# laoreja/HPLFlowNet

Hardware: AMD Instinct MI355X
Metric: point-pairs/sec + EPE3D, N=8192 FlyingThings3D, 1/2/4/8 MI355X (higher is better)
Workload: dtype f32 (wide layers: fp32 operands as scaled fp16 pairs, 3 partial products, fp32 accumulate); 1 GPU; full HPLFlowNet inference (7 levels, 19.3M params, random init), FT3D-like synthetic pair, N=8192, bs=1 per GPU; num_points=8192, step_includes_lattice_build=True, forward_streams=3, lattices_under_construction=3, exact_fallback_launches=0, lattice_launches_per_pair=34

## Files before the change

### hplflownet_amd/_lib.py

```python
import ctypes
import os

import torch

_HERE = os.path.dirname(os.path.abspath(__file__))
LIB_PATH = os.path.join(_HERE, 'libhplbcl.so')

c_i64, c_i32, c_f32, c_vp = ctypes.c_int64, ctypes.c_int32, ctypes.c_float, ctypes.c_void_p


class HplError(RuntimeError):
    pass


class RelayoutJob(ctypes.Structure):
    _fields_ = [('W', ctypes.c_void_p), ('base', ctypes.c_int64), ('sr', ctypes.c_int64), ('sq', ctypes.c_int64),
                ('sf', ctypes.c_int64), ('R', ctypes.c_int32), ('Q', ctypes.c_int32), ('F', ctypes.c_int32),
                ('mirror', ctypes.c_int32), ('ldw', ctypes.c_int64)]


class Split3Job(ctypes.Structure):
    _fields_ = [('Wt', ctypes.c_void_p), ('dst', ctypes.c_void_p), ('k_rows', ctypes.c_int64), ('ldw', ctypes.c_int64),
                ('plane_stride', ctypes.c_int64), ('amax', ctypes.c_void_p), ('planes', ctypes.c_int32), ('pad_', ctypes.c_int32)]

# ... 52 lines not shown
class Buf(ctypes.Structure):
    _fields_ = [('rows_sym', c_i32), ('cols', c_i32)]


class Weight(ctypes.Structure):
    _fields_ = [('Wt', c_vp), ('ldw', c_i64), ('rows', c_i64), ('Wt3', c_vp), ('wt3_plane_stride', c_i64),
                ('w_amax', c_vp), ('wt3_planes', c_i32), ('pad_', c_i32)]


class Op(ctypes.Structure):
    _fields_ = [('kind', c_i32), ('tag', c_i32), ('a', Ref), ('out', Ref), ('res', Ref), ('m_sym', c_i32),
                ('res_mod_sym', c_i32), ('level', c_i32), ('table', c_i32), ('order', c_i32), ('F', c_i32), ('C', c_i32),
                ('N', c_i32), ('weight', c_i32), ('bias', c_i32), ('act', c_i32), ('slope', c_f32), ('use_norm', c_i32),
                ('reg_stride_sym', c_i32), ('ext', c_i32), ('cond', c_i32), ('cond_level', c_i32), ('out2', Ref),
                ('rows2_sym', c_i32), ('b', Ref), ('flags', c_i32), ('aux', c_i32)]


class LevelTables(ctypes.Structure):
    _fields_ = [('n0', c_i64), ('n1', c_i64), ('H0', c_i64), ('H1', c_i64), ('emg_pair', c_vp),
                ('csr_ptr', c_vp), ('csr_pt', c_vp), ('csr_w', c_vp), ('csr_norm', c_vp), ('bary0', c_vp), ('off0', c_vp),
                ('blur', c_vp), ('blur_stride', c_i64), ('blur_perm', c_vp), ('up_perm', c_vp), ('n_up_groups', c_i32),
                ('up_group_cut', c_i32 * 5), ('up_group_perm', c_vp * 4), ('corr1', c_vp), ('corr1_stride', c_i64),
                ('corr1_perm', c_vp), ('corr2', c_vp), ('tile_bm', c_i32), ('group_tile_bm', c_i32),
                ('blur_perm_tidx', c_vp), ('blur_perm_tmask', c_vp), ('up_perm_tidx', c_vp), ('up_perm_tmask', c_vp),
                ('up_group_tidx', c_vp * 4), ('up_group_tmask', c_vp * 4), ('corr1_perm_tidx', c_vp),
                ('corr1_perm_tmask', c_vp), ('bary1', c_vp), ('off1', c_vp), ('up_tap_m', c_vp), ('up_tap_row', c_vp),
                ('up_tap_ptr', c_vp), ('up_tap_max', c_i64)]


class LatticeSpec(ctypes.Structure):
    _fields_ = [('n_levels', c_i32), ('scale', c_f32 * 8), ('bcn_radius', c_i32 * 8), ('corr_filter_radius', c_i32 * 8),
                ('corr_corr_radius', c_i32 * 8), ('next_divisor', c_f32 * 8), ('wide_up', c_i32 * 8), ('n_groups', c_i32),
                ('group_cut', c_i32 * 5), ('groups_min_sparsity', c_f32), ('perm_min_rows', c_i64), ('groups_min_rows', c_i64),
                ('group_tile_bm', c_i32),
                ('fused', c_i32)]


_SIGNATURES = {
    'hpl_version': (ctypes.c_int, []),
    'hpl_last_error': (ctypes.c_char_p, []),
    'hpl_device_info': (ctypes.c_int, [ctypes.c_int, ctypes.POINTER(ctypes.c_int), ctypes.POINTER(ctypes.c_int),
                                       ctypes.c_char_p, ctypes.c_int]),
    'hpl_index_narrow': (ctypes.c_int, [c_vp, c_vp, c_i64, c_vp]),
    'hpl_corr2_permute': (ctypes.c_int, [c_vp, c_vp, ctypes.c_int, ctypes.c_int, c_i64, c_vp]),
    'hpl_corr2_permute32': (ctypes.c_int, [c_vp, c_vp, ctypes.c_int, ctypes.c_int, c_i64, c_vp]),
    'hpl_csr_build': (ctypes.c_int, [c_vp, c_vp, c_i64, c_i64, c_i64, c_vp, c_vp, c_vp, c_vp, c_vp, c_vp]),
    'hpl_csr_build_pair': (ctypes.c_int, [c_vp, c_vp, c_i64, c_i64, c_vp, c_vp, c_i64, c_i64, c_vp, c_vp, c_vp, c_vp,
                                          c_vp, c_vp]),
    'hpl_splat': (ctypes.c_int, [c_vp, c_i64, ctypes.c_int, c_vp, c_vp, c_vp, c_vp, c_i64, c_vp, c_i64, c_vp]),
    'hpl_slice': (ctypes.c_int, [c_vp, c_i64, ctypes.c_int, c_vp, c_vp, c_i64, c_vp, c_vp, c_vp, c_i64, c_vp]),
    'hpl_splat_add': (ctypes.c_int, [c_vp, c_i64, ctypes.c_int, c_vp, c_vp, c_vp, c_vp, c_i64, c_vp, c_i64, c_vp]),
    'hpl_slice_add': (ctypes.c_int, [c_vp, c_i64, ctypes.c_int, c_vp, c_vp, c_i64, c_vp, c_vp, c_vp, c_i64, c_vp]),
    'hpl_weight_unlayout_batch': (ctypes.c_int, [c_vp, ctypes.c_int, c_vp, c_i64, c_vp, c_vp]),
    'hpl_psum': (ctypes.c_int, [c_vp, c_i64, c_i64, c_i64, ctypes.c_int, c_vp, c_i64, ctypes.c_int, c_vp]),
    'hpl_regroup': (ctypes.c_int, [c_vp, c_i64, c_i64, ctypes.c_int, ctypes.c_int, c_vp, c_i64, ctypes.c_int, c_vp]),
    'hpl_epe3d': (ctypes.c_int, [c_vp, c_vp, c_i64, c_vp, c_vp, c_vp]),
    'hpl_adam_flat': (ctypes.c_int, [c_vp, c_vp, c_vp, c_vp, c_i64, ctypes.c_double, ctypes.c_double, ctypes.c_double, ctypes.c_double,
                                     c_i64, c_vp]),
    'hpl_gather_sum': (ctypes.c_int, [c_vp, c_i64, c_vp, c_i64, c_i64, ctypes.c_int, ctypes.c_int, ctypes.c_int, c_vp, c_vp, c_i64, c_i64,
                                      ctypes.c_int, c_f32, c_vp, c_i64, c_vp]),
    'hpl_table_invert': (ctypes.c_int, [c_vp, c_i64, ctypes.c_int, c_i64, ctypes.c_int, c_i64, c_vp, c_vp]),
    'hpl_weight_relayout': (ctypes.c_int, [c_vp, c_i64, ctypes.c_int, ctypes.c_int, ctypes.c_int, c_i64, c_i64,
                                           c_i64, c_vp, c_vp, c_i64, c_i64, c_vp]),
    'hpl_weight_relayout_batch': (ctypes.c_int, [c_vp, ctypes.c_int, c_vp, c_i64, c_vp, c_vp]),
    'hpl_weight_fold': (ctypes.c_int, [c_vp, ctypes.c_int, ctypes.c_int, ctypes.c_int, ctypes.c_int, ctypes.c_int, c_vp, ctypes.c_int,
                                       c_vp, c_vp, ctypes.c_int, c_vp, c_i64, c_vp, c_vp, c_vp]),
    'hpl_weight_split3': (ctypes.c_int, [c_vp, c_i64, c_i64, c_vp, c_i64, c_vp]),
    'hpl_weight_split3_batch': (ctypes.c_int, [c_vp, ctypes.c_int, c_i64, ctypes.c_int, c_vp]),
    'hpl_weight_split2h': (ctypes.c_int, [c_vp, c_i64, c_i64, c_vp, c_i64, c_vp, c_vp]),
    'hpl_amax': (ctypes.c_int, [c_vp, c_i64, c_i64, c_i32, c_vp, c_vp]),
    'hpl_amax_rows': (ctypes.c_int, [c_vp, c_i64, c_i64, c_i32, c_vp, c_vp, c_vp]),
    'hpl_gconv_wgrad_scaled': (ctypes.c_int, [c_vp, c_i64, c_i64, c_vp, c_i64, c_i64, c_i64, ctypes.c_int, ctypes.c_int,
                                              c_vp, c_i64, ctypes.c_int, c_vp, c_i64, c_vp, c_vp, c_vp, c_i64, c_vp, c_vp, c_vp, c_vp]),
    'hpl_weight_unlayout': (ctypes.c_int, [c_vp, c_i64, ctypes.c_int, ctypes.c_int, ctypes.c_int, c_vp, c_i64,
                                           c_i64, c_i64, c_i64, ctypes.c_int, c_vp]),
    'hpl_tap_order_scratch_ints': (c_i64, [c_i64]),
    'hpl_tap_order': (ctypes.c_int, [c_vp, c_i64, ctypes.c_int, c_i64, c_vp, c_vp, c_vp]),
    'hpl_tile_index': (ctypes.c_int, [c_vp, c_i64, ctypes.c_int, c_i64, c_vp, ctypes.c_int, c_vp, c_vp, c_vp]),
    'hpl_gconv_forward': (ctypes.c_int, [ctypes.POINTER(GConvDesc), c_vp]),
    'hpl_gconv_forward_naive': (ctypes.c_int, [ctypes.POINTER(GConvDesc), c_vp]),
    'hpl_gconv_wgrad': (ctypes.c_int, [c_vp, c_i64, c_i64, c_vp, c_i64, c_i64, c_i64, ctypes.c_int, ctypes.c_int,
                                       c_vp, c_i64, ctypes.c_int, c_vp, c_i64, c_vp, c_vp, c_vp, c_i64, c_vp, c_vp]),
    'hpl_gconv_launch_info': (ctypes.c_int, [ctypes.POINTER(GConvDesc), ctypes.POINTER(GConvInfo)]),
    'hpl_wgrad_launch_info': (ctypes.c_int, [c_vp, c_i64, c_i64, c_vp, c_i64, c_i64, c_i64, ctypes.c_int, ctypes.c_int,
                                             c_vp, c_i64, ctypes.c_int, c_vp, c_i64, c_vp, c_vp, c_vp, c_i64, c_vp, c_vp, c_vp,
                                             ctypes.POINTER(WGradInfo)]),
    'hpl_tap_lists': (ctypes.c_int, [c_vp, c_i64, ctypes.c_int, c_i64, c_vp, c_vp, c_vp, c_vp, c_vp]),
    'hpl_colsum': (ctypes.c_int, [c_vp, c_i64, c_i64, ctypes.c_int, c_vp, c_vp]),
    'hpl_leaky_bwd': (ctypes.c_int, [c_vp, c_i64, c_vp, c_i64, c_f32, c_vp, c_i64, c_i64, ctypes.c_int, c_vp]),
    'hpl_leaky_bwd_amax': (ctypes.c_int, [c_vp, c_i64, c_vp, c_i64, c_f32, c_vp, c_i64, c_i64, ctypes.c_int, c_vp, c_vp]),
    'hpl_transpose': (ctypes.c_int, [c_vp, c_i64, c_vp, c_i64, c_i64, c_i64, c_vp]),
    'hpl_table_symmetric': (ctypes.c_int, [c_vp, c_i64, ctypes.c_int, c_i64, c_vp, c_vp]),
    'hpl_lattice_keys': (ctypes.c_int, [c_vp, c_i64, c_f32, c_vp, c_vp, c_vp, c_i64, c_vp]),
    'hpl_lattice_keys_pair': (ctypes.c_int, [c_vp, c_vp, c_vp, c_vp, c_i64, c_i64, c_f32, c_i64, c_i64, c_f32, c_vp, c_vp,
                                             c_vp, c_vp, c_vp, c_vp, c_i64, c_vp]),
    'hpl_lattice_workspace_bytes': (c_i64, [c_i64, c_i64]),
    'hpl_lattice_hash': (ctypes.c_int, [c_vp, c_i64, c_vp, c_i64, c_vp, c_vp, c_vp, c_vp, c_vp, c_vp, c_i64, c_vp]),
    'hpl_lattice_neighbors': (ctypes.c_int, [c_vp, c_i64, c_i64, c_vp, c_vp, c_i64, c_i64, ctypes.c_int,
                                             ctypes.c_int, ctypes.c_int, c_vp, c_vp, c_i64, c_i64, c_vp, c_vp, c_vp]),
    'hpl_lattice_next_points': (ctypes.c_int, [c_vp, c_i64, c_i64, c_f32, c_vp, c_vp]),
    'hpl_lattice_create': (c_vp, [ctypes.POINTER(LatticeSpec)]),
    'hpl_lattice_destroy': (None, [c_vp]),
    'hpl_lattice_arena_bytes': (c_i64, [c_vp, c_i64, c_i64]),
    'hpl_lattice_set_bounds': (ctypes.c_int, [c_vp, ctypes.POINTER(c_i64)]),
    'hpl_lattice_stats': (ctypes.c_int, [c_vp, ctypes.POINTER(c_i32)]),
    'hpl_lattice_begin': (ctypes.c_int, [c_vp, c_vp, c_vp, c_i64, c_i64, c_vp, c_i64, c_vp]),
    'hpl_lattice_begin_batch': (ctypes.c_int, [c_vp, c_vp, c_vp, c_i64, c_i64, c_i64, c_vp, c_i64, c_vp]),
    'hpl_lattice_arena_bytes_batch': (c_i64, [c_vp, c_i64, c_i64, c_i64]),
    'hpl_lattice_begin_ragged': (ctypes.c_int, [c_vp, c_vp, c_vp, c_i64, ctypes.POINTER(c_i64), ctypes.POINTER(c_i64), c_vp, c_i64,
                                                c_vp]),
    'hpl_lattice_arena_bytes_ragged': (c_i64, [c_vp, c_i64, ctypes.POINTER(c_i64), ctypes.POINTER(c_i64)]),
    'hpl_lattice_pair_counts': (ctypes.c_int, [c_vp, ctypes.POINTER(c_i64)]),
    'hpl_lattice_ready': (ctypes.c_int, [c_vp]),
    'hpl_lattice_advance': (ctypes.c_int, [c_vp, ctypes.POINTER(ctypes.c_int)]),
    'hpl_lattice_tables': (ctypes.POINTER(LevelTables), [c_vp]),
    'hpl_lattice_extras': (ctypes.c_int, [c_vp, ctypes.POINTER(c_vp), ctypes.POINTER(c_i64)]),
    'hpl_lattice_query_info': (ctypes.c_int, [c_vp, ctypes.POINTER(QueryInfo)]),
    'hpl_lattice_query': (ctypes.c_int, [ctypes.POINTER(QueryInfo), c_vp, c_i64, ctypes.POINTER(c_i64), ctypes.c_int, c_vp, c_vp, c_vp,
                                         c_vp]),
    'hpl_knn_interp': (ctypes.c_int, [c_vp, c_i64, c_vp, ctypes.c_int, c_vp, c_i64, ctypes.c_int, c_f32, ctypes.c_int,
                                      ctypes.POINTER(c_i64), ctypes.POINTER(c_i64), c_vp, c_vp, c_vp, c_vp, c_vp]),
    'hpl_rigid_fit_workspace_bytes': (c_i64, [ctypes.c_int, c_i64]),
    'hpl_rigid_fit': (ctypes.c_int, [c_vp, c_i64, c_vp, c_i64, c_i64, c_vp, ctypes.c_int, ctypes.POINTER(c_i64), ctypes.c_int,
                                     c_f32, c_vp, c_vp, c_vp, c_vp, c_vp, c_i64, c_vp]),
    'hpl_motion_segment_workspace_bytes': (c_i64, [ctypes.c_int, c_i64]),
    'hpl_motion_segment': (ctypes.c_int, [c_vp, c_i64, c_vp, c_i64, c_i64, c_vp, ctypes.c_int, ctypes.POINTER(c_i64), c_f32, c_f32,
                                          c_f32, ctypes.c_int, ctypes.c_int, c_vp, c_vp, c_vp, c_vp, c_vp, c_i64, c_vp]),
    'hpl_selfsup_loss_workspace_bytes': (c_i64, [ctypes.c_int, c_i64, c_i64, ctypes.c_int]),
    'hpl_selfsup_loss': (ctypes.c_int, [c_vp, c_i64, c_vp, c_i64, c_i64, c_vp, c_i64, ctypes.c_int, ctypes.POINTER(c_i64),
                                        ctypes.POINTER(c_i64), ctypes.c_int, c_f32, c_f32, c_vp, c_vp, c_vp, c_vp, c_vp, c_vp,
                                        c_i64, c_vp]),
    'hpl_ground_fit_workspace_bytes': (c_i64, [ctypes.c_int, c_i64, ctypes.c_int]),
    'hpl_ground_fit': (ctypes.c_int, [c_vp, c_i64, ctypes.c_int, ctypes.POINTER(c_i64), ctypes.POINTER(c_f32), c_f32, ctypes.c_int,
                                      c_f32, ctypes.c_int, c_f32, ctypes.c_uint64, ctypes.c_uint64, c_vp, c_vp, c_vp, c_vp, c_vp,
                                      c_vp, c_vp, c_i64, c_vp]),
    'hpl_voxel_downsample_workspace_bytes': (c_i64, [ctypes.c_int, c_i64, ctypes.c_int]),
    'hpl_voxel_downsample': (ctypes.c_int, [c_vp, c_i64, c_vp, c_i64, ctypes.c_int, ctypes.c_int, ctypes.POINTER(c_i64), c_f32,
                                            ctypes.POINTER(c_f32), ctypes.c_int, c_vp, c_i64, c_vp, c_i64, c_vp, c_vp, c_vp,
                                            c_vp, c_vp, c_i64, c_vp]),
    'hpl_frames_workspace_bytes': (c_i64, [ctypes.c_int, c_i64]),
    'hpl_frames_from_kitti': (ctypes.c_int, [c_vp, c_vp, c_vp, ctypes.c_int, ctypes.POINTER(ctypes.c_int32),
                                             ctypes.POINTER(ctypes.c_int32), ctypes.POINTER(c_i64), ctypes.POINTER(c_f32), c_f32,
                                             c_vp, c_i64, c_vp, c_i64, c_vp, c_vp, c_vp, c_i64, c_vp]),
    'hpl_frames_from_ft3d': (ctypes.c_int, [c_vp, c_vp, c_vp, c_vp, c_vp, ctypes.c_int, ctypes.POINTER(ctypes.c_int32),
                                            ctypes.POINTER(ctypes.c_int32), ctypes.POINTER(c_i64), c_f32, c_f32, c_f32,
                                            ctypes.c_int, c_f32, c_vp, c_i64, c_vp, c_i64, c_vp, c_vp, c_vp, c_i64, c_vp]),
    'hpl_png_unfilter': (ctypes.c_int, [c_vp, c_i64, c_i64, ctypes.c_int]),
    'hpl_icp_workspace_bytes': (c_i64, [ctypes.c_int, c_i64, c_i64]),
    'hpl_icp': (ctypes.c_int, [c_vp, c_i64, c_vp, c_i64, c_vp, c_vp, ctypes.c_int, ctypes.POINTER(c_i64), ctypes.POINTER(c_i64),
                               ctypes.c_int, c_f32, c_f32, c_f32, c_f32, c_vp, c_vp, c_vp, c_vp, c_vp, c_vp, c_i64, c_vp]),
    'hpl_plan_create': (c_vp, [ctypes.POINTER(Op), ctypes.c_int, ctypes.POINTER(Buf), ctypes.c_int,
                               ctypes.POINTER(Weight), ctypes.c_int, ctypes.POINTER(c_vp), ctypes.c_int]),
    'hpl_plan_destroy': (None, [c_vp]),
    'hpl_plan_workspace_bytes': (c_i64, [c_vp, ctypes.POINTER(LevelTables), ctypes.c_int]),
    'hpl_plan_run': (ctypes.c_int, [c_vp, ctypes.POINTER(LevelTables), ctypes.c_int, c_vp, c_vp, c_vp, c_vp, c_i64, c_vp]),
    'hpl_plan_run_range': (ctypes.c_int, [c_vp, ctypes.POINTER(LevelTables), ctypes.c_int, c_vp, c_vp, c_vp, c_vp, c_vp, c_vp, c_i64,
                                          c_vp, c_vp, ctypes.c_int, ctypes.c_int, ctypes.c_int]),
    'hpl_plan_run_range_loss': (ctypes.c_int, [c_vp, ctypes.POINTER(LevelTables), ctypes.c_int, c_vp, c_vp, c_vp, c_vp, c_vp, c_vp, c_i64,
                                               c_vp, c_vp, ctypes.c_int, ctypes.c_int, ctypes.c_int, ctypes.c_int, ctypes.c_int,
                                               ctypes.POINTER(c_i64), c_vp, ctypes.c_int, c_vp]),
    'hpl_plan_run_batch': (ctypes.c_int, [c_vp, ctypes.POINTER(LevelTables), ctypes.c_int, ctypes.c_int, c_vp, c_vp, c_vp, c_vp, c_i64,
                                          c_vp]),
    'hpl_plan_batch_extra_bytes': (c_i64, [ctypes.POINTER(LevelTables), ctypes.c_int]),
    'hpl_batch_stage': (ctypes.c_int, [ctypes.c_int, c_i64, c_i64, c_vp, c_vp, c_vp, c_vp, c_vp, c_vp, c_vp]),
    'hpl_ragged_stage': (ctypes.c_int, [ctypes.c_int, ctypes.POINTER(c_vp), ctypes.POINTER(c_i64), ctypes.POINTER(c_i64),
                                        ctypes.POINTER(c_vp), ctypes.POINTER(c_i64), ctypes.POINTER(c_i64), ctypes.POINTER(c_vp),
# ... 84 lines not shown
```

### hplflownet_amd/csrc/executor.hip

```cpp
#include "common.h"
#include "gconv_common.h"
#include <stdlib.h>

#include <algorithm>
#include <new>
#include <vector>

using namespace hpl;

namespace {

constexpr int64_t SPLITK_ELEMS = 8 << 20;
constexpr int64_t SPLITK_WS_BYTES = 64ll << 20;
constexpr int AMAX_SLOTS = 4096;
constexpr int64_t HEAD_BYTES = SPLITK_WS_BYTES + AMAX_SLOTS * 8;
constexpr int MAX_SYMS = HPL_SYM_LEVEL0 + 8 * HPL_MAX_LEVELS;

__global__ void k_copy_cols(const float *__restrict__ src, int64_t lds, float *__restrict__ dst, int64_t ldd,
                            int64_t rows, int cols) {
    const int64_t total = rows * cols;
    int64_t i = (int64_t)blockIdx.x * blockDim.x + threadIdx.x;
    const int64_t stride = (int64_t)gridDim.x * blockDim.x;
    for (; i < total; i += stride) {
        const int64_t r = i / cols;
        const int c = (int)(i - r * cols);
        dst[r * ldd + c] = src[r * lds + c];
    }
}

__global__ void k_copy_cols4(const float4 *__restrict__ src, int64_t lds4, float4 *__restrict__ dst, int64_t ldd4,
                             int64_t rows, int cols4) {
    const int64_t total = rows * cols4;
    int64_t i = (int64_t)blockIdx.x * blockDim.x + threadIdx.x;
    const int64_t stride = (int64_t)gridDim.x * blockDim.x;
    for (; i < total; i += stride) {
        const int64_t r = i / cols4;
        const int c = (int)(i - r * cols4);
        dst[r * ldd4 + c] = src[r * lds4 + c];
    }
}

constexpr int EMG_JOBS = 24;
struct EmgJobs {
    const float4 *src[EMG_JOBS];
    float *dst[EMG_JOBS];
    int64_t ldd[EMG_JOBS];
    int64_t rows[EMG_JOBS];
    int ones[EMG_JOBS];
    int n;
};
__global__ void k_copy_emg_batch(const EmgJobs j) {
    const int job = blockIdx.y;
    const float4 *src = j.src[job];
    float *dst = j.dst[job];
    const int64_t ldd = j.ldd[job], rows = j.rows[job];
    const bool ones = j.ones[job] != 0;
    const bool vec = (ldd % 4 == 0) && ((reinterpret_cast<uintptr_t>(dst) & 15) == 0);
    for (int64_t r = (int64_t)blockIdx.x * blockDim.x + threadIdx.x; r < rows; r += (int64_t)gridDim.x * blockDim.x) {
        const float4 v = src[r];
        float *d = dst + r * ldd;
        if (vec) *reinterpret_cast<float4 *>(d) = v;
        else { d[0] = v.x; d[1] = v.y; d[2] = v.z; d[3] = v.w; }
        if (!ones) continue;
        if (vec) *reinterpret_cast<float4 *>(d + 4) = make_float4(1.f, 0.f, 0.f, 0.f);
        else { d[4] = 1.f; d[5] = 0.f; d[6] = 0.f; d[7] = 0.f; }
    }
}

inline int range_guard_mode() {
    static const int m = [] { const char *e = getenv("HPL_RANGE_GUARD"); return e ? atoi(e) : 1; }();
    return m;
}
inline bool range_guard() { return range_guard_mode() != 0; }

struct View {
    float *p;
    int64_t ld;
    int64_t rows;
    int cols;
};

}

struct hpl_plan {
    std::vector<hpl_op> ops;
    std::vector<hpl_buf> bufs;
    std::vector<hpl_weight> weights;
    std::vector<const float *> biases;
    int profile_tag = -1;
    bool hoist_emg = true;
    int64_t *clock_probe = nullptr;
    std::vector<hipEvent_t> pool;
    size_t pool_used = 0;
    std::vector<float *> base;
    std::vector<int64_t> rows;
    const hpl_relayout_job *ul_jobs = nullptr;
    const int64_t *ul_prefix = nullptr;
    const float *ul_src = nullptr;
    std::vector<int32_t> ul_first;
    std::vector<int64_t> ul_offset;
    std::vector<hipEvent_t> fence;
    size_t fence_used = 0;
    struct AmaxEnt { int buf; int64_t row_off, rows; int col_off, cols; const float *slot; bool guarded; };
    std::vector<AmaxEnt> amax;
    int amax_used = 0;
    int32_t *guard_trips = nullptr;
    std::vector<int64_t> lay_sym, lay_off;
    int64_t lay_total = 0;
};

namespace {

int resolve_syms(const hpl_level_tables *lv, int n_levels, int64_t *sym) {
    HPL_REQUIRE(lv && n_levels >= 1 && n_levels <= HPL_MAX_LEVELS, "hpl_plan: 1 .. %d lattice levels expected, got %d",
                HPL_MAX_LEVELS, n_levels);
    for (int i = 0; i < MAX_SYMS; ++i) sym[i] = 0;
    sym[HPL_SYM_N0] = lv[0].n0;
    sym[HPL_SYM_N1] = lv[0].n1;
    sym[HPL_SYM_NP] = lv[0].n0 + lv[0].n1;
    for (int L = 0; L < n_levels; ++L) {
        int64_t *s = sym + HPL_SYM_LEVEL0 + 8 * L;
        HPL_REQUIRE(lv[L].n0 > 0 && lv[L].n1 > 0 && lv[L].H0 > 0 && lv[L].H1 > 0, "hpl_plan: empty lattice level %d", L);
        HPL_REQUIRE(L == 0 || (lv[L].n0 == lv[L - 1].H0 && lv[L].n1 == lv[L - 1].H1),
                    "hpl_plan: level %d has %lld / %lld input points, level %d has %lld / %lld vertices", L,
                    (long long)lv[L].n0, (long long)lv[L].n1, L - 1, (long long)lv[L - 1].H0, (long long)lv[L - 1].H1);
        s[HPL_SYM_H0] = lv[L].H0;
        s[HPL_SYM_H1] = lv[L].H1;
        s[HPL_SYM_HP] = lv[L].H0 + lv[L].H1;
        s[HPL_SYM_FH0] = 15 * lv[L].H0;
        s[HPL_SYM_IN0] = lv[L].n0;
        s[HPL_SYM_INP] = lv[L].n0 + lv[L].n1;
        s[HPL_SYM_FH1] = 15 * lv[L].H1;
    }
    return HPL_OK;
}

inline int64_t symv(const int64_t *sym, int id) { return id < 0 ? 0 : sym[id]; }

inline int64_t buf_bytes(int64_t rows, int cols) { return (rows * cols * 4 + 255) / 256 * 256; }

struct Runner {
    hpl_plan &pl;
    const hpl_level_tables *lv;
    int n_levels;
    const int64_t *sym;
    const float *pc[2];
    float *out;
    float *splitk;
    hipStream_t s;
    hplStream hs;
    const float *sf = nullptr;
    float *loss = nullptr;
    int loss_kind = HPL_LOSS_ROWS;
    int batch = 1, loss_stride = 1;
    const float *pair_loss = nullptr;
    const float *dflow = nullptr;
    hipStream_t main_s = nullptr, side_s = nullptr;
    bool side_busy = false;
    float *amax_base = nullptr;
    const float *cur_a_amax = nullptr, *cur_b_amax = nullptr;
    float *cur_y_amax = nullptr;
    bool cur_y_guarded = false;

    int amax_of(const hpl_ref &r, const View &v, int64_t rows, int cols, const float *&slot, bool guard) {
        const int64_t off = r.buf >= 0 ? symv(sym, r.row_off_sym) : 0;
        guard = guard && range_guard() && range_guard_mode() != 3;
        for (const auto &e : pl.amax)
            if (e.buf == r.buf && e.row_off == off && e.rows == rows && e.col_off == r.col_off && e.cols == cols && (e.guarded || !guard)) { slot = e.slot; return HPL_OK; }
        HPL_REQUIRE(pl.amax_used < AMAX_SLOTS, "hpl_plan_run: more than %d operand reductions in one run", AMAX_SLOTS);
        float *dst = amax_base + 2 * pl.amax_used++;
        const int rc = hpl_gc::amax_launch(v.p, v.ld, rows, cols, dst, main_s, guard ? reinterpret_cast<unsigned *>(dst + 1) : nullptr);
        if (rc) return rc;
        if (r.buf >= 0) pl.amax.push_back({r.buf, off, rows, r.col_off, cols, dst, guard});
        slot = dst;
        return HPL_OK;
    }
    void amax_forget(const hpl_ref &r) {
        if (r.buf < 0) return;
        for (size_t i = 0; i < pl.amax.size();) {
            const auto &e = pl.amax[i];
            if (e.buf == r.buf && e.col_off < r.col_off + r.cols && r.col_off < e.col_off + e.cols) { pl.amax[i] = pl.amax.back(); pl.amax.pop_back(); }
            else ++i;
        }
    }
    void amax_produced(const hpl_op &op) {
        if (!cur_y_amax || op.out.buf < 0) return;
        pl.amax.push_back({op.out.buf, symv(sym, op.out.row_off_sym), symv(sym, op.m_sym), op.out.col_off, op.N, cur_y_amax, cur_y_guarded});
        cur_y_amax = nullptr;
    }
    static bool guarded(const hpl_op &op) { return range_guard() && !(op.flags & HPL_FLAG_NOGUARD); }
    float *amax_slot() { return pl.amax_used < AMAX_SLOTS ? amax_base + 2 * pl.amax_used++ : nullptr; }
    int prepare_amax(const hpl_op &op, bool side) {
        cur_a_amax = cur_b_amax = nullptr;
        cur_y_amax = nullptr;
        cur_y_guarded = false;
        if (hpl_gc::split_planes() != 2) return HPL_OK;
        View A, B;
        int rc;
        if (op.kind == HPL_OP_LEAKY_BWD) {
            if (!side && op.out.buf >= 0 && op.N >= 128 && symv(sym, op.m_sym) >= 1024) cur_y_amax = amax_slot();
            return HPL_OK;
        }
        if (op.kind == HPL_OP_GCONV) {
            if (op.weight < 0 || op.weight >= (int)pl.weights.size() || pl.weights[op.weight].wt3_planes != 2 || !pl.weights[op.weight].Wt3) return HPL_OK;
            const int64_t M = symv(sym, op.m_sym);
            if ((op.flags & HPL_FLAG_SCATTER) || !hpl_gc::split3_maybe(M, op.C, op.F > 15 ? 15 : op.F, op.N)) return HPL_OK;
            if ((rc = view(op.a, A, "gconv input"))) return rc;
            if ((rc = amax_of(op.a, A, A.rows, op.C, cur_a_amax, guarded(op)))) return rc;
            if (!side && op.out.buf >= 0 && op.N >= 128 && !(op.flags & HPL_FLAG_NOYAMAX)) cur_y_amax = amax_slot();
            return HPL_OK;
        }
        if (op.kind == HPL_OP_WGRAD) {
            const int64_t M = symv(sym, op.m_sym);
            const bool taps = (op.flags & HPL_FLAG_TAPS) && op.table == HPL_TBL_BLUR0;
            if (!(op.N >= 256 && op.C >= 128 && M >= 8192 && (taps || (op.F == 1 && op.table == HPL_TBL_NONE)))) return HPL_OK;
            if ((rc = view(op.a, A, "wgrad input")) || (rc = view(op.b, B, "wgrad output gradient"))) return rc;
            if ((rc = amax_of(op.a, A, A.rows, op.C, cur_a_amax, false))) return rc;
            return amax_of(op.b, B, M, op.N, cur_b_amax, false);
        }
        return HPL_OK;
    }

    hipEvent_t fence_event() {
        if (pl.fence_used == pl.fence.size()) {
            hipEvent_t e;
            if (hipEventCreateWithFlags(&e, hipEventDisableTiming) != hipSuccess) return nullptr;
            pl.fence.push_back(e);
        }
        return pl.fence[pl.fence_used++];
    }
    int to_side() {
        hipEvent_t e = fence_event();
        HPL_REQUIRE(e, "hpl_plan_run_range: hipEventCreate failed");
        if (hipEventRecord(e, main_s) != hipSuccess || hipStreamWaitEvent(side_s, e, 0) != hipSuccess) { set_error("hpl_plan_run_range: fence"); return HPL_EHIP; }
        s = side_s; hs = reinterpret_cast<hplStream>(side_s);
        side_busy = true;
        return HPL_OK;
    }
    void to_main() { s = main_s; hs = reinterpret_cast<hplStream>(main_s); }
    int join() {
        if (!side_busy) return HPL_OK;
        hipEvent_t e = fence_event();
        HPL_REQUIRE(e, "hpl_plan_run_range: hipEventCreate failed");
        if (hipEventRecord(e, side_s) != hipSuccess || hipStreamWaitEvent(main_s, e, 0) != hipSuccess) { set_error("hpl_plan_run_range: join"); return HPL_EHIP; }
        side_busy = false;
        return HPL_OK;
    }

    int view(const hpl_ref &r, View &v, const char *what) const {
        if (r.buf == HPL_BUF_OUT) {
            v.p = out + r.col_off;
            v.ld = 3;
            v.rows = sym[HPL_SYM_N0];
            v.cols = r.cols;
            HPL_REQUIRE(r.col_off + r.cols <= 3, "hpl_plan_run: %s exceeds the [N][3] output", what);
            return HPL_OK;
        }
        HPL_REQUIRE(r.buf >= 0 && r.buf < (int)pl.bufs.size(), "hpl_plan_run: %s refers to buffer %d", what, r.buf);
        const int64_t off = symv(sym, r.row_off_sym);
        const int64_t have = pl.rows[r.buf] - off;
        v.rows = r.rows_sym < 0 ? have : sym[r.rows_sym];
        HPL_REQUIRE(off >= 0 && v.rows >= 0 && v.rows <= have && r.col_off >= 0 &&
                        r.col_off + r.cols <= pl.bufs[r.buf].cols,
                    "hpl_plan_run: %s outside buffer %d (%lld x %d): rows %lld + %lld, columns %d + %d", what, r.buf,
                    (long long)pl.rows[r.buf], pl.bufs[r.buf].cols, (long long)off, (long long)v.rows, r.col_off, r.cols);
        HPL_REQUIRE(pl.base[r.buf], "hpl_plan_run: %s refers to buffer %d, which no active op of the program uses", what, r.buf);
        v.ld = pl.bufs[r.buf].cols;
        v.p = pl.base[r.buf] + off * v.ld + r.col_off;
        v.cols = r.cols;
        return HPL_OK;
    }

    void bracket(bool on, bool stop) {
// ... 27 lines not shown
        }
        HPL_REQUIRE(op.weight >= 0 && op.weight < (int)pl.weights.size(), "hpl_plan_run: weight image %d", op.weight);
        HPL_REQUIRE(op.level >= 0 && op.level < n_levels, "hpl_plan_run: op uses lattice level %d of %d", op.level, n_levels);
        const hpl_level_tables &t = lv[op.level];
        const hpl_weight &w = pl.weights[op.weight];
        const int64_t M = symv(sym, op.m_sym);
        const int32_t *nbr = nullptr, *perm = nullptr, *tidx = nullptr, *tmask = nullptr;
        int64_t stride = 0, reg = 0;
        int ngroups = 0;
        switch (op.table) {
        case HPL_TBL_NONE: break;
        case HPL_TBL_BLUR_PAIR:
            nbr = t.blur; stride = t.blur_stride;
            if (op.order != HPL_ORD_NONE) { perm = t.blur_perm; tidx = t.blur_perm_tidx; tmask = t.blur_perm_tmask; }
            break;
        case HPL_TBL_BLUR0:
            nbr = t.blur; stride = t.blur_stride;
            if (op.order == HPL_ORD_GROUPS && t.n_up_groups >= 2) ngroups = t.n_up_groups;
            else if (op.order != HPL_ORD_NONE) { perm = t.up_perm; tidx = t.up_perm_tidx; tmask = t.up_perm_tmask; }
            break;
        case HPL_TBL_CORR1:
            nbr = t.corr1; stride = t.corr1_stride;
            if (op.order != HPL_ORD_NONE) { perm = t.corr1_perm; tidx = t.corr1_perm_tidx; tmask = t.corr1_perm_tmask; }
            break;
        case HPL_TBL_CORR2: nbr = t.corr2; stride = 15 * t.H0; break;
        case HPL_TBL_REGULAR: reg = symv(sym, op.reg_stride_sym); break;
        default: HPL_REQUIRE(false, "hpl_plan_run: gconv with table kind %d", op.table);
        }
        HPL_REQUIRE(op.table == HPL_TBL_NONE || op.table == HPL_TBL_REGULAR || nbr, "hpl_plan_run: level %d lacks table %d",
                    op.level, op.table);
        HPL_REQUIRE(op.table != HPL_TBL_REGULAR || (reg > 0 && (op.F - 1) * reg + M <= A.rows),
                    "hpl_plan_run: regular stride %lld x %d taps outside the %lld input rows", (long long)reg, op.F,
                    (long long)A.rows);
        const bool accum = (op.flags & HPL_FLAG_ACCUM) != 0, scatter = (op.flags & HPL_FLAG_SCATTER) != 0;
        HPL_REQUIRE(!(accum && has_res) && !(scatter && (has_out2 || ngroups >= 2 || !t.corr2 || op.aux <= 0 || op.N % op.aux)),
                    "hpl_plan_run: accumulate / scatter flags on an op they do not fit");
        HPL_REQUIRE(A.cols >= op.C && (scatter || (Y.cols >= op.N && Y.rows >= M)), "hpl_plan_run: gconv shapes (C=%d of %d, N=%d of %d)",
                    op.C, A.cols, op.N, Y.cols);
        HPL_REQUIRE(!scatter || (Y.cols >= op.aux && Y.rows >= t.H1), "hpl_plan_run: scatter target too small");
        const bool prof = pl.profile_tag >= 0 && op.tag == pl.profile_tag;
        auto pass = [&](int f0, int F, const int32_t *row_perm, bool first, bool last, const int32_t *ti,
                        const int32_t *tm) -> int {
            hpl_gconv_desc d = {};
            d.A = A.p + (reg ? (int64_t)f0 * reg * A.ld : 0);
            d.lda = A.ld;
            d.rows_a = A.rows - (reg ? (int64_t)f0 * reg : 0);
            d.nbr = nbr ? nbr + (int64_t)f0 * stride : nullptr;
            d.nbr_stride = stride;
            d.reg_stride = reg;
            d.M = M; d.C = op.C; d.F = F;
            const int64_t wrows = w.rows - (int64_t)f0 * op.C;
            d.Wt = w.Wt + (int64_t)f0 * op.C * w.ldw;
            d.ldw = w.ldw;
            d.N = op.N;
            d.w_rows = (int32_t)imin(wrows, cdiv((int64_t)F * op.C, 32) * 32);
            d.act = last ? op.act : HPL_ACT_NONE;
            d.slope = op.slope;
            d.bias = (first && op.bias >= 0) ? pl.biases[op.bias] : nullptr;
            if (first) {
                if (has_res) { d.res = R.p; d.ldres = R.ld; d.res_mod = op.res_mod_sym >= 0 ? sym[op.res_mod_sym] : R.rows; }
                else if (accum && !scatter) { d.res = Y.p; d.ldres = Y.ld; d.res_mod = M; }
            } else {
                d.res = Y.p; d.ldres = Y.ld; d.res_mod = M;
            }
            d.Y = Y.p; d.ldy = Y.ld;
            if (last && has_out2) { d.Y2 = Y2.p; d.ldy2 = Y2.ld; d.rows2 = rows2; }
            if (last && cur_y_amax && !scatter) {
                d.y_amax = cur_y_amax;
                if (guarded(op) && range_guard_mode() < 3) { d.y_guard = reinterpret_cast<uint32_t *>(cur_y_amax + 1); cur_y_guarded = true; }
            }
            d.row_perm = row_perm;
            if (row_perm && ti && tm) { d.tile_idx = ti; d.tile_mask = tm; d.tile_bm = ngroups >= 2 ? t.group_tile_bm : t.tile_bm; }
            if (w.Wt3 && ((int64_t)f0 * op.C) % 8 == 0 && (w.wt3_planes != 2 || cur_a_amax)) {
                d.Wt3 = static_cast<const char *>(w.Wt3) + (int64_t)f0 * op.C / 8 * w.ldw * 16;
                d.wt3_plane_stride = w.wt3_plane_stride;
                d.wt3_planes = w.wt3_planes;
                d.a_amax = cur_a_amax; d.w_amax = w.w_amax;
                if (cur_a_amax && guarded(op) && range_guard_mode() != 2) { d.a_guard = reinterpret_cast<const uint32_t *>(cur_a_amax + 1); d.guard_trips = pl.guard_trips; }
            }
            if (prof) d.clock_probe = pl.clock_probe;
            if (scatter) { d.scat = t.corr2; d.scat_stride = 15 * t.H0; d.scat_c = op.aux; }
            else
            if (M * op.N <= SPLITK_ELEMS) { d.ws = splitk; d.ws_bytes = SPLITK_WS_BYTES; }
            bracket(prof, false);
            const int r = hpl_gconv_forward(&d, hs);
            bracket(prof, true);
            return r;
        };
        if (ngroups >= 2) {
            for (int g = 0; g < ngroups; ++g) {
                rc = pass(t.up_group_cut[g], t.up_group_cut[g + 1] - t.up_group_cut[g], t.up_group_perm[g], g == 0,
                          g == ngroups - 1, t.up_group_tidx[g], t.up_group_tmask[g]);
                if (rc) return rc;
            }
            return HPL_OK;
        }
        if ((nbr || reg) && op.F > 15) {
            for (int f0 = 0; f0 < op.F; f0 += 15) {
                rc = pass(f0, (int)imin(15, op.F - f0), nullptr, f0 == 0, f0 + 15 >= op.F, nullptr, nullptr);
                if (rc) return rc;
            }
            return HPL_OK;
        }
        return pass(0, op.F, perm, true, true, tidx, tmask);
    }

    int run_op(const hpl_op &op) {
        const bool prof = pl.profile_tag >= 0 && op.tag == pl.profile_tag && op.kind != HPL_OP_GCONV;
        int rc = HPL_OK;
        View A, Y;
        switch (op.kind) {
        case HPL_OP_GCONV: return gconv(op);
        case HPL_OP_SPLAT: {
            if ((rc = view(op.a, A, "splat input")) || (rc = view(op.out, Y, "splat output"))) return rc;
            HPL_REQUIRE(op.level >= 0 && op.level < n_levels, "hpl_plan_run: splat at level %d", op.level);
            const hpl_level_tables &t = lv[op.level];
            const int64_t H = symv(sym, op.m_sym);
            HPL_REQUIRE(op.table == HPL_TBL_CSR_PAIR || op.table == HPL_TBL_CSR_C0, "hpl_plan_run: splat table kind %d", op.table);
            HPL_REQUIRE(H == (op.table == HPL_TBL_CSR_PAIR ? t.H0 + t.H1 : t.H0) && Y.rows >= H && Y.cols >= op.C &&
                            A.cols >= op.C && A.rows >= (op.table == HPL_TBL_CSR_PAIR ? t.n0 + t.n1 : t.n0),
                        "hpl_plan_run: splat shapes at level %d", op.level);
            bracket(prof, false);
            rc = ((op.flags & HPL_FLAG_ACCUM) ? hpl_splat_add : hpl_splat)(A.p, A.ld, op.C, t.csr_ptr, t.csr_pt, t.csr_w,
                                                                         op.use_norm ? t.csr_norm : nullptr, H, Y.p, Y.ld, hs);
            bracket(prof, true);
            return rc;
        }
        case HPL_OP_SLICE: {
            if ((rc = view(op.a, A, "slice input")) || (rc = view(op.out, Y, "slice output"))) return rc;
            HPL_REQUIRE(op.level >= 0 && op.level < n_levels && op.table == HPL_TBL_CLOUD0, "hpl_plan_run: slice at level %d", op.level);
            const hpl_level_tables &t = lv[op.level];
            const int64_t N = symv(sym, op.m_sym);
            HPL_REQUIRE(N == t.n0 && A.rows >= t.H0 && A.cols >= op.C && Y.cols >= op.C && Y.rows >= N,
                        "hpl_plan_run: slice shapes at level %d", op.level);
            bracket(prof, false);
            rc = hpl_slice(A.p, A.ld, op.C, t.bary0, t.off0, N, nullptr, op.bias >= 0 ? pl.biases[op.bias] : nullptr, Y.p,
                           Y.ld, hs);
            bracket(prof, true);
            return rc;
        }
        case HPL_OP_COPY: {
            if ((rc = view(op.out, Y, "copy output"))) return rc;
            const int64_t rows = symv(sym, op.m_sym);
            const float *src;
            int64_t lds;
            if (op.a.buf == -1) {
                HPL_REQUIRE(op.level >= 0 && op.level < n_levels && (op.C == 4 || op.C == 8), "hpl_plan_run: emg copy at level %d", op.level);
                src = lv[op.level].emg_pair;
                lds = 4;
                HPL_REQUIRE(rows <= lv[op.level].n0 + lv[op.level].n1, "hpl_plan_run: emg copy of %lld rows", (long long)rows);
                if (op.C == 8) {
                    HPL_REQUIRE(!(op.flags & HPL_FLAG_ACCUM) && Y.rows >= rows && Y.cols >= 8, "hpl_plan_run: emg copy output too small");
                    if (rows == 0) return HPL_OK;
                    EmgJobs jobs;
                    jobs.src[0] = reinterpret_cast<const float4 *>(src);
                    jobs.dst[0] = Y.p; jobs.ldd[0] = Y.ld; jobs.rows[0] = rows; jobs.ones[0] = 1;
                    jobs.n = 1;
                    k_copy_emg_batch<<<dim3((unsigned)imin(cdiv(rows, 256), 64), 1), 256, 0, s>>>(jobs);
                    HPL_CHECK_LAUNCH("hpl_plan_run (copy)");
                    return HPL_OK;
                }
            } else {
                if ((rc = view(op.a, A, "copy input"))) return rc;
                HPL_REQUIRE(A.rows >= rows && A.cols >= op.C, "hpl_plan_run: copy input too small");
                src = A.p;
                lds = A.ld;
            }
            HPL_REQUIRE(Y.rows >= rows && Y.cols >= op.C, "hpl_plan_run: copy output too small");
// ... 130 lines not shown
            return hpl_gather_sum(A.p, A.ld, t.corr2, 15 * t.H0, M, op.F, op.N, op.N, bias, has_res ? R.p : nullptr, has_res ? R.ld : 0,
                                  has_res ? (op.res_mod_sym >= 0 ? sym[op.res_mod_sym] : R.rows) : 0, op.act, op.slope, Y.p, Y.ld, hs);
        }
        case HPL_OP_INVERT: {
            if ((rc = view(op.out, Y, "inverse table"))) return rc;
            HPL_REQUIRE(op.level >= 0 && op.level < n_levels && lv[op.level].corr2, "hpl_plan_run: invert at level %d", op.level);
            const hpl_level_tables &t = lv[op.level];
            HPL_REQUIRE(Y.ld == Y.cols && Y.rows * Y.cols >= 225 * t.H1, "hpl_plan_run: inverse table buffer too small");
            return hpl_table_invert(t.corr2, 15 * t.H0, 15, t.H0, 15, t.H1, reinterpret_cast<int32_t *>(Y.p), hs);
        }
        default: HPL_REQUIRE(false, "hpl_plan_run: unknown op kind %d", op.kind);
        }
        return HPL_OK;
    }
};

}

extern "C" hpl_plan *hpl_plan_create(const hpl_op *ops, int n_ops, const hpl_buf *bufs, int n_bufs,
                                     const hpl_weight *weights, int n_weights, const float *const *biases,
                                     int n_biases) {
    if (!ops || n_ops <= 0 || !bufs || n_bufs <= 0 || n_weights < 0 || n_biases < 0) {
        set_error("hpl_plan_create: bad arguments");
        return nullptr;
    }
    hpl_plan *p = new (std::nothrow) hpl_plan();
    if (!p) return nullptr;
    p->ops.assign(ops, ops + n_ops);
    p->bufs.assign(bufs, bufs + n_bufs);
    if (n_weights) p->weights.assign(weights, weights + n_weights);
    if (n_biases) p->biases.assign(biases, biases + n_biases);
    auto overlaps = [](const hpl_ref &a, const hpl_ref &b) {
        return a.buf >= 0 && a.buf == b.buf && a.col_off < b.col_off + b.cols && b.col_off < a.col_off + a.cols;
    };
    for (int i = 0; i < n_ops && p->hoist_emg; ++i) {
        if (!(ops[i].kind == HPL_OP_COPY && ops[i].a.buf == -1)) continue;
        for (int j = 0; j < n_ops; ++j)
            if (j != i && (overlaps(ops[i].out, ops[j].out) || (ops[j].kind == HPL_OP_GCONV && overlaps(ops[i].out, ops[j].out2)))) {
                const bool exclusive = ops[i].cond != HPL_COND_ALWAYS && ops[j].cond != HPL_COND_ALWAYS &&
                                       ops[i].cond != ops[j].cond && ops[i].cond_level == ops[j].cond_level;
                if (!exclusive) p->hoist_emg = false;
            }
    }
    for (const hpl_buf &b : p->bufs)
        if (b.cols <= 0 || b.rows_sym < 0 || b.rows_sym >= MAX_SYMS) {
            set_error("hpl_plan_create: bad buffer (rows symbol %d, %d columns)", b.rows_sym, b.cols);
            delete p;
            return nullptr;
        }
    return p;
}

extern "C" void hpl_plan_destroy(hpl_plan *plan) {
    if (!plan) return;
    for (hipEvent_t e : plan->pool) (void)hipEventDestroy(e);
    for (hipEvent_t e : plan->fence) (void)hipEventDestroy(e);
    if (plan->guard_trips) (void)hipFree(plan->guard_trips);
    delete plan;
}

namespace {
int64_t plan_layout(hpl_plan &pl, const hpl_level_tables *lv, int n_levels, const int64_t *sym) {
    if (pl.lay_sym.size() == (size_t)MAX_SYMS && std::equal(pl.lay_sym.begin(), pl.lay_sym.end(), sym)) return pl.lay_total;
    const int nb = (int)pl.bufs.size(), nops = (int)pl.ops.size();
    std::vector<int> first(nb, nops + 1), last(nb, -1);
    auto touch = [&](const hpl_ref &r, int at, bool to_end) {
        if (r.buf < 0 || r.buf >= nb) return;
        first[r.buf] = std::min(first[r.buf], at);
        last[r.buf] = std::max(last[r.buf], to_end ? nops : at);
    };
    for (int i = 0; i < nops; ++i) {
        const hpl_op &op = pl.ops[i];
        if (op.cond != HPL_COND_ALWAYS) {
            if (op.cond_level < 0 || op.cond_level >= n_levels) continue;
            const bool shrink = lv[op.cond_level].n0 < lv[op.cond_level].H0;
            if ((op.cond == HPL_COND_SHRINK) != shrink) continue;
        }
        const bool emg = op.kind == HPL_OP_COPY && op.a.buf == -1 && pl.hoist_emg;
        const bool side = (op.flags & HPL_FLAG_SIDE) != 0;
        const int at = emg ? 0 : i;
        touch(op.a, at, side); touch(op.b, at, side); touch(op.res, at, side);
        touch(op.out, at, false); touch(op.out2, at, false);
    }
    std::vector<int> order;
    for (int b = 0; b < nb; ++b) if (last[b] >= 0) order.push_back(b);
    std::vector<int64_t> size(nb, 0);
    for (int b : order) size[b] = buf_bytes(sym[pl.bufs[b].rows_sym], pl.bufs[b].cols);
    std::stable_sort(order.begin(), order.end(), [&](int x, int y) { return first[x] != first[y] ? first[x] < first[y] : size[x] > size[y]; });
    pl.lay_off.assign(nb, -1);
    int64_t total = HEAD_BYTES;
    std::vector<std::pair<int64_t, int64_t>> busy;
    std::vector<int> placed;
    for (int b : order) {
        busy.clear();
        for (int q : placed)
            if (first[q] <= last[b] && first[b] <= last[q] && size[q] > 0) busy.emplace_back(pl.lay_off[q], pl.lay_off[q] + size[q]);
        std::sort(busy.begin(), busy.end());
        int64_t at = HEAD_BYTES;
        for (const auto &iv : busy) {
            if (iv.first - at >= size[b]) break;
            at = std::max(at, iv.second);
        }
        pl.lay_off[b] = at;
        total = std::max(total, at + size[b]);
        placed.push_back(b);
    }
    pl.lay_sym.assign(sym, sym + MAX_SYMS);
    pl.lay_total = total + 256;
    return pl.lay_total;
}
}

extern "C" int64_t hpl_plan_workspace_bytes(const hpl_plan *plan, const hpl_level_tables *levels, int n_levels) {
    int64_t sym[MAX_SYMS];
    if (!plan || resolve_syms(levels, n_levels, sym) != HPL_OK) return -1;
    return plan_layout(*const_cast<hpl_plan *>(plan), levels, n_levels, sym);
}

extern "C" int hpl_plan_run(hpl_plan *plan, const hpl_level_tables *levels, int n_levels, const float *pc1,
                            const float *pc2, float *out, void *workspace, int64_t workspace_bytes, hplStream stream) {
    HPL_REQUIRE(plan, "hpl_plan_run: null argument");
    return hpl_plan_run_range(plan, levels, n_levels, pc1, pc2, nullptr, out, nullptr, workspace, workspace_bytes, stream, nullptr, 0,
                              (int)plan->ops.size(), 1);
}

extern "C" int hpl_plan_set_unlayout(hpl_plan *plan, const hpl_relayout_job *jobs, const int64_t *prefix, const float *src,
                                     const int32_t *bucket_first, const int64_t *bucket_offset, int n_buckets) {
    HPL_REQUIRE(plan && jobs && prefix && src && bucket_first && bucket_offset && n_buckets > 0, "hpl_plan_set_unlayout: bad arguments");
    plan->ul_jobs = jobs; plan->ul_prefix = prefix; plan->ul_src = src;
    plan->ul_first.assign(bucket_first, bucket_first + n_buckets + 1);
    plan->ul_offset.assign(bucket_offset, bucket_offset + n_buckets + 1);
    return HPL_OK;
}

extern "C" int hpl_plan_run_range(hpl_plan *plan, const hpl_level_tables *levels, int n_levels, const float *pc1, const float *pc2,
                                  const float *sf, float *out, float *loss, void *workspace, int64_t workspace_bytes, hplStream stream,
                                  hplStream side_stream, int op_begin, int op_end, int join) {
    return hpl_plan_run_range_loss(plan, levels, n_levels, pc1, pc2, sf, out, loss, workspace, workspace_bytes, stream, side_stream,
                                   op_begin, op_end, join, HPL_LOSS_ROWS, 1, nullptr, nullptr, 1, nullptr);
}

extern "C" int hpl_plan_run_range_loss(hpl_plan *plan, const hpl_level_tables *levels, int n_levels, const float *pc1, const float *pc2,
                                       const float *sf, float *out, float *loss, void *workspace, int64_t workspace_bytes,
                                       hplStream stream, hplStream side_stream, int op_begin, int op_end, int join, int loss_kind,
                                       int batch, const int64_t *prefix, float *pair_loss, int loss_stride, const float *dflow) {
    HPL_REQUIRE(plan && pc1 && pc2 && out && workspace, "hpl_plan_run: null argument");
    HPL_REQUIRE(loss_kind == HPL_LOSS_ROWS || loss_kind == HPL_LOSS_GRAD,
                "hpl_plan_run_range_loss: loss kind %d", loss_kind);
    if (loss_kind != HPL_LOSS_ROWS) {
        HPL_REQUIRE(batch >= 1 && batch <= 64 && prefix && loss_stride >= 1,
                    "hpl_plan_run_range_loss: loss kind %d over %d pairs (1 .. 64) needs their prefix and a loss stride >= 1 (%d)", loss_kind,
                    batch, loss_stride);
        HPL_REQUIRE(levels && prefix[0] == 0 && prefix[batch] == levels[0].n0,
                    "hpl_plan_run_range_loss: the prefix runs from %lld to %lld, the lattice has %lld points", (long long)prefix[0],
                    (long long)prefix[batch], levels ? (long long)levels[0].n0 : -1ll);
    }
    HPL_REQUIRE(op_begin >= 0 && op_begin <= op_end && op_end <= (int)plan->ops.size(), "hpl_plan_run_range: ops [%d, %d) of %d", op_begin,
                op_end, (int)plan->ops.size());
    int64_t sym[MAX_SYMS];
    int rc = resolve_syms(levels, n_levels, sym);
    if (rc) return rc;
    char *w = reinterpret_cast<char *>((reinterpret_cast<uintptr_t>(workspace) + 255) / 256 * 256);
    char *const end = reinterpret_cast<char *>(workspace) + workspace_bytes;
    const int64_t need = plan_layout(*plan, levels, n_levels, sym);
    HPL_REQUIRE(w + need - 256 <= end, "hpl_plan_run: workspace of %lld bytes is too small (hpl_plan_workspace_bytes: %lld)",
                (long long)workspace_bytes, (long long)need);
    plan->base.resize(plan->bufs.size());
    plan->rows.resize(plan->bufs.size());
    for (size_t i = 0; i < plan->bufs.size(); ++i) {
        plan->rows[i] = sym[plan->bufs[i].rows_sym];
        plan->base[i] = plan->lay_off[i] >= 0 ? reinterpret_cast<float *>(w + plan->lay_off[i]) : nullptr;
    }
    float *splitk = reinterpret_cast<float *>(w);
    Runner r{*plan, levels, n_levels, sym, {pc1, pc2}, out, splitk, to_stream(stream), stream};
    r.sf = sf; r.loss = loss;
    r.loss_kind = loss_kind; r.batch = batch; r.loss_stride = loss_stride;
    r.pair_loss = pair_loss; r.dflow = dflow;
    r.main_s = to_stream(stream);
    r.side_s = side_stream ? to_stream(side_stream) : nullptr;
    r.amax_base = reinterpret_cast<float *>(w + SPLITK_WS_BYTES);
    plan->fence_used = 0;
    if (!plan->guard_trips && hpl_gc::split_planes() == 2) {
        if (hipMalloc(reinterpret_cast<void **>(&plan->guard_trips), 4) != hipSuccess || hipMemsetAsync(plan->guard_trips, 0, 4, r.main_s) != hipSuccess) {
            set_error("hpl_plan_run: allocating the range-guard counter failed");
            return HPL_EHIP;
        }
    }
    if (op_begin == 0) {
        plan->amax.clear();
        plan->amax_used = 0;
        if (hpl_gc::split_planes() == 2 && hipMemsetAsync(r.amax_base, 0, AMAX_SLOTS * 8, r.main_s) != hipSuccess) { set_error("hpl_plan_run: hipMemsetAsync failed"); return HPL_EHIP; }
    }
    auto active = [&](const hpl_op &op, bool &run) -> int {
        run = true;
        if (op.cond != HPL_COND_ALWAYS) {
            HPL_REQUIRE(op.cond_level >= 0 && op.cond_level < n_levels, "hpl_plan_run: condition on level %d", op.cond_level);
            const bool shrink = levels[op.cond_level].n0 < levels[op.cond_level].H0;
            run = (op.cond == HPL_COND_SHRINK) == shrink;
        }
        return HPL_OK;
    };
    auto is_emg = [](const hpl_op &op) { return op.kind == HPL_OP_COPY && op.a.buf == -1; };
    constexpr int batch_emg = 1;
    const bool hoist = batch_emg && plan->hoist_emg;
    if (hoist && op_begin == 0) {
        EmgJobs jobs;
        jobs.n = 0;
        int64_t most = 0;
        auto flush = [&]() {
            if (!jobs.n) return;
            dim3 grid((unsigned)imin(cdiv(most, 256), 64), (unsigned)jobs.n);
            k_copy_emg_batch<<<grid, 256, 0, r.s>>>(jobs);
            jobs.n = 0;
            most = 0;
        };
        for (const hpl_op &op : plan->ops) {
            if (!is_emg(op)) continue;
            bool run;
            if ((rc = active(op, run))) return rc;
            if (!run) continue;
            View Y;
            if ((rc = r.view(op.out, Y, "copy output"))) return rc;
            const int64_t rows = symv(sym, op.m_sym);
            HPL_REQUIRE(op.level >= 0 && op.level < n_levels && (op.C == 4 || op.C == 8) && Y.cols >= op.C && Y.rows >= rows &&
                            rows <= levels[op.level].n0 + levels[op.level].n1,
                        "hpl_plan_run: emg copy of %lld rows at level %d", (long long)rows, op.level);
            if (rows == 0) continue;
            jobs.src[jobs.n] = reinterpret_cast<const float4 *>(levels[op.level].emg_pair);
            jobs.dst[jobs.n] = Y.p;
            jobs.ldd[jobs.n] = Y.ld;
            jobs.rows[jobs.n] = rows;
            jobs.ones[jobs.n] = op.C == 8;
            most = most > rows ? most : rows;
            if (++jobs.n == EMG_JOBS) flush();
        }
        flush();
        HPL_CHECK_LAUNCH("hpl_plan_run (emg copies)");
    }
    for (int i = op_begin; i < op_end; ++i) {
        const hpl_op &op = plan->ops[i];
        if (hoist && is_emg(op)) continue;
        bool run;
        if ((rc = active(op, run))) return rc;
        if (!run) continue;
        const bool side = r.side_s && (op.flags & HPL_FLAG_SIDE);
        if ((rc = r.prepare_amax(op, side))) return rc;
        r.amax_forget(op.out);
        r.amax_forget(op.out2);
        if (side) { if ((rc = r.to_side())) return rc; }
        else if (op.kind == HPL_OP_UNLAYOUT && (rc = r.join())) return rc;
        rc = r.run_op(op);
        if (side) r.to_main();
        if (rc) return rc;
        r.amax_produced(op);
    }
    if (!join) return HPL_OK;
    r.side_busy = r.side_s != nullptr;
    return r.join();
}

extern "C" int hpl_plan_guard_trips(hpl_plan *plan, int64_t *count) {
    HPL_REQUIRE(plan && count, "hpl_plan_guard_trips: null argument");
    *count = 0;
    if (!plan->guard_trips) return HPL_OK;
    int32_t v = 0;
    if (hipMemcpy(&v, plan->guard_trips, 4, hipMemcpyDeviceToHost) != hipSuccess) { set_error("hpl_plan_guard_trips: read-back failed"); return HPL_EHIP; }
    *count = v;
    return HPL_OK;
}

extern "C" int hpl_plan_profile(hpl_plan *plan, int tag) {
    HPL_REQUIRE(plan, "hpl_plan_profile: null plan");
    plan->profile_tag = tag;
    return HPL_OK;
}

extern "C" int hpl_plan_clock_probe(hpl_plan *plan, int64_t *clock_probe) {
    HPL_REQUIRE(plan, "hpl_plan_clock_probe: null plan");
    plan->clock_probe = clock_probe;
    return HPL_OK;
}

extern "C" int hpl_plan_profile_read(hpl_plan *plan, int *launches, float *total_ms) {
    HPL_REQUIRE(plan && launches && total_ms, "hpl_plan_profile_read: null argument");
    *launches = 0;
    *total_ms = 0.f;
    for (size_t i = 0; i + 1 < plan->pool_used; i += 2) {
        if (hipEventSynchronize(plan->pool[i + 1]) != hipSuccess) { set_error("hpl_plan_profile_read: event wait failed"); return HPL_EHIP; }
        float ms = 0.f;
        if (hipEventElapsedTime(&ms, plan->pool[i], plan->pool[i + 1]) == hipSuccess) { *total_ms += ms; ++*launches; }
    }
    plan->pool_used = 0;
    return HPL_OK;
}
```

### hplflownet_amd/csrc/gconv.hip

```cpp
#include "common.h"
#include "gconv_common.h"
#include <cstdlib>
#include <cmath>
#include <cstring>
#include <string>

#include <stdlib.h>
#include <type_traits>

using namespace hpl;
using namespace hpl_gc;



namespace {

template <int BM, int BN, int WGM, int WGN, bool AVEC, int F_LDS, bool COMPACT = false>
__global__ void __launch_bounds__(64 * WGM * WGN, COMPACT ? 6 : 1) k_gconv(const GParams p) {
    constexpr int NT = 64 * WGM * WGN;
    constexpr int WTM = BM / WGM, WTN = BN / WGN;
    constexpr int TM = WTM / 32, TN = WTN / 32;
    constexpr int LDA_S = COMPACT ? BM + 1 : BM + 2;
    constexpr int LDB_S = BN;
    constexpr int A_ROWS_PER_PASS = NT / 8;
// ... 436 lines not shown
        if (p.act == HPL_ACT_LEAKY) {
            acc.x = acc.x > 0.f ? acc.x : p.slope * acc.x;
            acc.y = acc.y > 0.f ? acc.y : p.slope * acc.y;
            acc.z = acc.z > 0.f ? acc.z : p.slope * acc.z;
            acc.w = acc.w > 0.f ? acc.w : p.slope * acc.w;
        }
        *reinterpret_cast<float4 *>(p.Y + (int64_t)m * p.ldy + n) = acc;
        if (p.Y2 && m < (unsigned)p.rows2) *reinterpret_cast<float4 *>(p.Y2 + (int64_t)m * p.ldy2 + n) = acc;
    }
}

__global__ void k_gconv_naive(const GParams p) {
    const int64_t total = p.M * p.N;
    int64_t i = (int64_t)blockIdx.x * blockDim.x + threadIdx.x;
    const int64_t stride = (int64_t)gridDim.x * blockDim.x;
    for (; i < total; i += stride) {
        const int64_t m = i / p.N;
        const int n = (int)(i - m * p.N);
        float acc = 0.f;
        for (int f = 0; f < p.F; ++f) {
            const int64_t row = src_row(p, f, m);
            if (row < 0) continue;
            const float *a = p.A + row * p.lda;
            const float *w = p.Wt + (int64_t)f * p.C * p.ldw + n;
            for (int c = 0; c < p.C; ++c) acc = fmaf(a[c], w[(int64_t)c * p.ldw], acc);
        }
        float v = acc + (p.bias ? p.bias[n] : 0.f);
        if (p.res) v += p.res[(m % p.res_mod) * p.ldres + n];
        if (p.act == HPL_ACT_LEAKY) v = v > 0.f ? v : p.slope * v;
        if (p.scat) {
            const int k = n / p.scat_c, c = n - k * p.scat_c;
            const int32_t tgt = p.scat[(int64_t)k * p.scat_stride + m];
            if (tgt >= 0) atomicAdd(p.Y + (int64_t)tgt * p.ldy + c, v);
        } else {
            p.Y[m * p.ldy + n] = v;
            if (p.Y2 && m < p.rows2) p.Y2[m * p.ldy2 + n] = v;
        }
    }
}

}

int hpl_gc::fill_params(const hpl_gconv_desc *d, GParams &p, const char *who) {
    HPL_REQUIRE(d, "%s: null descriptor", who);
    HPL_REQUIRE(d->A && d->Wt && d->Y, "%s: null A / Wt / Y", who);
    HPL_REQUIRE(d->M >= 0 && d->C > 0 && d->F > 0 && d->N > 0, "%s: bad sizes M=%lld C=%d F=%d N=%d", who,
                (long long)d->M, d->C, d->F, d->N);
    HPL_REQUIRE(d->F <= 15, "%s: F=%d taps (radius > 1) not supported by the LDS-staged index table", who, d->F);
    HPL_REQUIRE(d->rows_a > 0 && d->rows_a < (int64_t)INT32_MAX, "%s: rows_a out of range", who);
    HPL_REQUIRE((int64_t)d->F * d->C <= 32768, "%s: contraction length F*C = %lld > 32768 (slice list in LDS)", who,
                (long long)d->F * d->C);
    HPL_REQUIRE(d->lda >= d->C, "%s: lda %lld < C %d", who, (long long)d->lda, d->C);
    HPL_REQUIRE(d->ldw >= d->N && d->ldw % 4 == 0 && aligned16(d->Wt), "%s: ldw must be a multiple of 4 >= N and Wt 16-byte aligned", who);
    HPL_REQUIRE(d->nbr || d->F == 1 || d->reg_stride > 0, "%s: F > 1 needs a neighbour table or reg_stride", who);
    HPL_REQUIRE(!d->res || (d->res_mod > 0 && d->ldres >= d->N), "%s: bad residual description", who);
    HPL_REQUIRE(!d->scat || d->scat_c > 0, "%s: bad scatter description", who);
    HPL_REQUIRE(d->scat || d->ldy >= d->N, "%s: ldy %lld < N %d", who, (long long)d->ldy, d->N);
    HPL_REQUIRE(d->act == HPL_ACT_NONE || d->act == HPL_ACT_LEAKY, "%s: unknown activation %d", who, d->act);
    p.A = d->A; p.lda = d->lda; p.rows_a = d->rows_a;
    p.nbr = d->nbr; p.nbr_stride = d->nbr_stride; p.reg_stride = d->reg_stride;
    p.M = d->M; p.C = d->C; p.F = d->F; p.K = d->F * d->C;
    p.Wt = d->Wt; p.ldw = d->ldw; p.N = d->N; p.act = d->act; p.slope = d->slope;
    p.bias = d->bias; p.res = d->res; p.ldres = d->ldres; p.res_mod = d->res_mod;
    p.Y = d->Y; p.ldy = d->ldy;
    p.Y2 = d->Y2; p.ldy2 = d->ldy2; p.rows2 = d->Y2 ? d->rows2 : 0;
    HPL_REQUIRE(!d->Y2 || (!d->scat && d->ldy2 >= d->N && d->rows2 >= 0), "%s: bad second destination", who);
    p.scat = d->scat; p.scat_stride = d->scat_stride; p.scat_c = d->scat_c;
    p.row_perm = d->row_perm;
    p.tile_idx = (d->tile_idx && d->tile_mask && d->row_perm) ? d->tile_idx : nullptr;
    p.tile_mask = d->tile_mask;
    p.tile_bm = d->tile_bm;
    p.clock_probe = reinterpret_cast<long long *>(d->clock_probe);
    p.perm_chunk = 4;
    p.ws = d->ws; p.ws_bytes = d->ws ? d->ws_bytes : 0; p.splits = 1; p.partial = nullptr;
    p.Wt3 = d->Wt3; p.w3_plane_stride = d->wt3_plane_stride;
    p.planes = d->wt3_planes == 2 ? 2 : 3; p.a_amax = d->a_amax; p.w_amax = d->w_amax;
    HPL_REQUIRE(!d->Wt3 || d->wt3_planes == 0 || d->wt3_planes == 2 || d->wt3_planes == 3, "%s: wt3_planes = %d", who, d->wt3_planes);
    if (p.planes == 2 && !(p.a_amax && p.w_amax)) p.Wt3 = nullptr;
    p.y_amax = d->y_amax; p.y_amax_done = 0;
    p.a_guard = d->a_guard; p.y_guard = d->y_guard; p.guard_trips = d->guard_trips; p.guard_partials = 0;
    HPL_REQUIRE(!(d->y_amax && d->scat), "%s: y_amax with a scatter epilogue", who);
    p.col_share = 0; p.col_rows = 0;
    p.tiles_m = p.tiles_n = 0;
    p.a_bytes = ((d->rows_a - 1) * d->lda + d->C) * 4;
    const int64_t w_rows = d->w_rows ? (int64_t)d->w_rows : cdiv(p.K, 32) * 32;
    HPL_REQUIRE(w_rows >= p.K, "%s: w_rows=%lld < F*C=%d", who, (long long)w_rows, p.K);
    p.w_bytes = imin(w_rows, cdiv(p.K, 32) * 32) * d->ldw * 4;
    HPL_REQUIRE(p.a_bytes < (int64_t)INT32_MAX && p.w_bytes < (int64_t)INT32_MAX,
                "%s: A or Wt spans >= 2 GiB (32-bit buffer offsets)", who);
    return HPL_OK;
}

namespace {
void plan_cfg(GParams &p, hpl_gconv_info &o, int BM, int BN, int WGM, int WGN) {
    const bool avec = o.avec != 0;
    o.family = HPL_FAMILY_FP32;
    o.bm = BM; o.bn = BN; o.threads = 64 * WGM * WGN;
    p.tiles_m = (int)cdiv(p.M, BM);
    p.tiles_n = (int)cdiv(p.N, BN);
    if (p.tile_bm != BM || p.F == 1) p.tile_idx = nullptr;
    p.splits = 1;
    const int tiles = p.tiles_m * p.tiles_n;
    const int nk = (p.K + BK - 1) / BK;
    if (p.ws && !p.scat && tiles <= 128 && nk >= 8) {
        int sp = (int)imin(imin(16, nk / 4), imax(1, 512 / tiles));
        while (sp > 1 && (int64_t)sp * p.M * p.N * 4 > p.ws_bytes) --sp;
        p.splits = sp;
        p.partial = p.ws;
    } else if (p.ws && !p.scat && nk >= 32) {
        constexpr int mid = 1;
        const int WG_PER_CU = 16 / (WGM * WGN);
        const double slots = 256.0 * WG_PER_CU;
        if (mid && tiles < 6 * slots) {
            double best = 0.0;
            int best_sp = 1;
            for (int sp = 1; sp <= 16 && sp * 8 <= nk; ++sp) {
                if (sp > 1 && (int64_t)sp * p.M * p.N * 4 > p.ws_bytes) break;
                const double rounds = tiles * sp / slots;
                const double eff = rounds / std::ceil(rounds);
                const double cost = sp == 1 ? 0.0 : 100.0 * sp / (double)p.K;
                const double score = eff * (1.0 - cost);
                if (score > best * 1.03) { best = score; best_sp = sp; }
            }
            if (best_sp > 1) { p.splits = best_sp; p.partial = p.ws; }
        }
    }
    int grid = tiles * p.splits;
    {
        const int64_t lim = (int64_t)0x7fffffff;
        static const int epi = getenv("HPL_GCONV_EPILOGUE") ? atoi(getenv("HPL_GCONV_EPILOGUE")) : 1;
        p.epi_fast = (epi && !p.scat && p.M < (1 << 24) && p.M * (p.splits > 1 ? p.N : p.ldy) * 4 < lim && p.ldy * 4 < (1 << 24) &&
                      (!p.res || (p.res_mod > 0 && p.res_mod < (1 << 24) && imin(p.res_mod, p.M) * p.ldres * 4 < lim && p.ldres * 4 < (1 << 24))) &&
                      (!p.Y2 || (p.rows2 * p.ldy2 * 4 < lim && p.ldy2 * 4 < (1 << 24)))) ? 1 : 0;
    }
    p.col_share = 0; p.col_rows = 0;
    constexpr int col_order = 1;
    if (col_order && p.row_perm && p.splits == 1) {
        int g = 8, b = p.tiles_n % 8;
        while (b) { const int t = g % b; g = b; b = t; }
        p.col_share = 8 / g;
        p.col_rows = p.col_share == 1 ? p.tiles_m : (int)cdiv(p.tiles_m, COL_CHUNK * p.col_share) * COL_CHUNK;
        grid = p.tiles_n * p.col_share * p.col_rows;
    }
    o.f_lds = p.F == 1 ? 1 : 15;
    o.compact = 0;
    if (BM == 64 && BN == 128 && WGM == 2 && WGN == 4) {
        if (avec && p.F > 1 && p.F <= 8 && nk <= 512 && p.splits == 1) {
            o.f_lds = 8;
            o.compact = 1;
        }
    }
    o.splits = p.splits;
    o.guard_sets = 1;
    o.col_share = p.col_share; o.col_rows = p.col_rows;
    o.tile_tables = p.tile_idx ? 1 : 0;
    o.epi_fast = p.epi_fast;
    o.tiles_m = p.tiles_m; o.tiles_n = p.tiles_n;
    o.grid = grid;
}

template <int BM, int BN, int WGM, int WGN>
void launch_cfg(const GParams &p, const hpl_gconv_info &o, hipStream_t s) {
    const int grid = (int)o.grid;
    if constexpr (BM == 64 && BN == 128 && WGM == 2 && WGN == 4) {
        if (o.compact) {
            k_gconv<BM, BN, WGM, WGN, true, 8, true><<<grid, 64 * WGM * WGN, 0, s>>>(p);
            return;
        }
    }
    if (o.f_lds == 1) {
        if (o.avec) k_gconv<BM, BN, WGM, WGN, true, 1><<<grid, 64 * WGM * WGN, 0, s>>>(p);
        else k_gconv<BM, BN, WGM, WGN, false, 1><<<grid, 64 * WGM * WGN, 0, s>>>(p);
    } else {
        if (o.avec) k_gconv<BM, BN, WGM, WGN, true, 15><<<grid, 64 * WGM * WGN, 0, s>>>(p);
        else k_gconv<BM, BN, WGM, WGN, false, 15><<<grid, 64 * WGM * WGN, 0, s>>>(p);
    }
}

int plan_finish(const GParams &p) {
    if (p.splits <= 1) return HPL_FINISH_NONE;
    const bool vec = p.N % 4 == 0 && p.ldy % 4 == 0 && aligned16(p.Y) && aligned16(p.partial) && (!p.bias || aligned16(p.bias)) &&
                     (!p.res || (p.ldres % 4 == 0 && aligned16(p.res))) && (!p.Y2 || (p.ldy2 % 4 == 0 && aligned16(p.Y2))) &&
                     p.M * p.N < (int64_t)0x7fffffff && p.res_mod < (int64_t)0x7fffffff;
    return vec ? HPL_FINISH_VEC4 : HPL_FINISH_SCALAR;
}

void launch_finish(const GParams &p, const hpl_gconv_info &o, hipStream_t s) {
    if (o.finish == HPL_FINISH_VEC4) {
        const int g = (int)imin(cdiv(p.M * (p.N / 4), 256), 2048);
        k_gconv_finish4<<<g, 256, 0, s>>>(p);
    } else {
        const int g = (int)imin(cdiv(p.M * p.N, 256), 2048);
        k_gconv_finish<<<g, 256, 0, s>>>(p);
    }
}

void plan_forward(GParams &p, hpl_gconv_info &o) {
    memset(&o, 0, sizeof(o));
    o.avec = ((p.C % 4 == 0) && (p.lda % 4 == 0) && aligned16(p.A)) ? 1 : 0;
    if (o.avec && p.Wt3 && plan_split3(p, o)) {
        o.finish = plan_finish(p);
        return;
    }
    const int64_t t128 = cdiv(p.M, 128), t64 = cdiv(p.M, 64);
    const int nsel = p.N;
    if (nsel > 64) {
        const int64_t tn = cdiv(p.N, 128);
        if (t64 * tn >= 512) plan_cfg(p, o, 64, 128, 2, 4);
        else plan_cfg(p, o, 64, 64, 2, 2);
    } else if (nsel > 32) {
        plan_cfg(p, o, 64, 64, 2, 2);
    } else {
        if (t128 >= 512) plan_cfg(p, o, 128, 32, 4, 1);
        else plan_cfg(p, o, 64, 32, 2, 1);
    }
    o.finish = plan_finish(p);
}
}

extern "C" int hpl_gconv_launch_info(const hpl_gconv_desc *d, hpl_gconv_info *info) {
    HPL_REQUIRE(info, "hpl_gconv_launch_info: null info");
    memset(info, 0, sizeof(*info));
    GParams p;
    int rc = fill_params(d, p, "hpl_gconv_forward");
    if (rc != HPL_OK) return rc;
    if (p.M == 0) return HPL_OK;
    plan_forward(p, *info);
    return HPL_OK;
}

extern "C" int hpl_gconv_forward(const hpl_gconv_desc *d, hplStream stream) {
    GParams p;
    int rc = fill_params(d, p, "hpl_gconv_forward");
    if (rc != HPL_OK) return rc;
    if (p.M == 0) return HPL_OK;
    hipStream_t s = to_stream(stream);
    hpl_gconv_info o;
    plan_forward(p, o);
    if (o.family != HPL_FAMILY_FP32) {
        launch_split3(p, o, s);
        if (o.finish != HPL_FINISH_NONE) launch_finish(p, o, s);
        HPL_CHECK_LAUNCH("hpl_gconv_forward");
        if (p.y_amax && !p.y_amax_done) return amax_launch(p.Y, p.ldy, p.M, p.N, p.y_amax, s, p.y_guard);
        return HPL_OK;
    }
    if (o.bm == 128) launch_cfg<128, 32, 4, 1>(p, o, s);
    else if (o.bn == 128) launch_cfg<64, 128, 2, 4>(p, o, s);
    else if (o.bn == 64) launch_cfg<64, 64, 2, 2>(p, o, s);
    else launch_cfg<64, 32, 2, 1>(p, o, s);
    if (o.finish != HPL_FINISH_NONE) launch_finish(p, o, s);
    HPL_CHECK_LAUNCH("hpl_gconv_forward");
    if (p.y_amax) return amax_launch(p.Y, p.ldy, p.M, p.N, p.y_amax, s, p.y_guard);
    return HPL_OK;
}

namespace {
__global__ void __launch_bounds__(256) k_tile_index(const int32_t *__restrict__ nbr, int64_t stride, int F, int64_t M,
                                                    const int32_t *__restrict__ perm, int BM, int32_t *__restrict__ tile_idx,
                                                    int32_t *__restrict__ tile_mask) {
    __shared__ int masks[8];
    const int t = threadIdx.x;
    if (t < 8) masks[t] = 0;
    __syncthreads();
    const int64_t tile = blockIdx.x, m0 = tile * BM;
    int32_t *out = tile_idx + tile * F * BM;
    const int r = t % BM;
    const int64_t m = m0 + r;
    const int v = (m < M) ? (perm ? perm[m] : (int)m) : -1;
    int mybits = 0;
    for (int f = t / BM; f < F; f += 256 / BM) {
        const int row = (v >= 0) ? nbr[(int64_t)f * stride + v] : -1;
        out[f * BM + r] = row;
        mybits |= (row >= 0) ? (1 << f) : 0;
    }
#pragma unroll
    for (int o = 16; o >= 1; o >>= 1) mybits |= __shfl_xor(mybits, o, 64);
    if ((t & 31) == 0 && mybits) {
        atomicOr(&masks[0], mybits);
        atomicOr(&masks[2 + (r >> 5)], mybits);
    }
    __syncthreads();
    if (t < 8) tile_mask[tile * 8 + t] = masks[t];
}
}

namespace {
__global__ void __launch_bounds__(1024) k_tile_rank(int32_t *__restrict__ tile_mask, int tiles) {
    __shared__ int hist[16], base[16], running[16], wcnt[16][16];
    const int t = threadIdx.x, lane = t & 63, wave = t >> 6;
    if (t < 16) { hist[t] = 0; running[t] = 0; }
    __syncthreads();
    for (int j = t; j < tiles; j += 1024) atomicAdd(&hist[__popc(tile_mask[(int64_t)j * 8] & 0x7fff)], 1);
    __syncthreads();
    if (t == 0) {
        int off = 0;
        for (int b = 15; b >= 0; --b) { base[b] = off; off += hist[b]; }
    }
    __syncthreads();
    for (int j0 = 0; j0 < tiles; j0 += 1024) {
        const int j = j0 + t;
        const int c = j < tiles ? __popc(tile_mask[(int64_t)j * 8] & 0x7fff) : -1;
        int mine = 0;
#pragma unroll
        for (int cls = 0; cls < 16; ++cls) {
            const unsigned long long bal = __ballot(c == cls);
            if (c == cls) mine = __popcll(bal & ((1ull << lane) - 1ull));
            if (lane == 0) wcnt[wave][cls] = __popcll(bal);
        }
        __syncthreads();
        if (c >= 0) {
            int before = 0;
            for (int w = 0; w < wave; ++w) before += wcnt[w][c];
            tile_mask[(int64_t)(base[c] + running[c] + before + mine) * 8 + 6] = j;
        }
        __syncthreads();
        if (t < 16) {
            int tot = 0;
            for (int w = 0; w < 16; ++w) tot += wcnt[w][t];
            running[t] += tot;
        }
        __syncthreads();
    }
}
}

extern "C" int hpl_tile_index(const int32_t *nbr, int64_t nbr_stride, int F, int64_t M, const int32_t *row_perm,
                              int BM, int32_t *tile_idx, int32_t *tile_mask, hplStream stream) {
    HPL_REQUIRE(nbr && tile_idx && tile_mask && F >= 1 && F <= 15 && M > 0 && (BM == 64 || BM == 128),
                "hpl_tile_index: bad arguments");
    k_tile_index<<<(int)cdiv(M, BM), 256, 0, to_stream(stream)>>>(nbr, nbr_stride, F, M, row_perm, BM, tile_idx, tile_mask);
    k_tile_rank<<<1, 1024, 0, to_stream(stream)>>>(tile_mask, (int)cdiv(M, BM));
    HPL_CHECK_LAUNCH("hpl_tile_index");
    return HPL_OK;
}

extern "C" int hpl_gconv_forward_naive(const hpl_gconv_desc *d, hplStream stream) {
// ... 706 lines not shown
```

### hplflownet_amd/csrc/gconv3.hip

```cpp
#include "common.h"
#include "gconv_common.h"

#include <stdlib.h>
#include <string>
#include <type_traits>

using namespace hpl;
using namespace hpl_gc;

typedef __bf16 bf16x8 __attribute__((ext_vector_type(8)));
typedef __bf16 bf16x2 __attribute__((ext_vector_type(2)));
typedef _Float16 f16x8 __attribute__((ext_vector_type(8)));
typedef _Float16 f16x2 __attribute__((ext_vector_type(2)));
typedef float float2_t __attribute__((ext_vector_type(2)));
typedef unsigned u32x4 __attribute__((ext_vector_type(4)));
typedef unsigned u32x2 __attribute__((ext_vector_type(2)));


namespace {

__device__ __forceinline__ void split2(float x0, float x1, unsigned &h, unsigned &m, unsigned &l) {
    const float2_t v = {x0, x1};
    h = __builtin_bit_cast(unsigned, __builtin_convertvector(v, bf16x2));
    const float r0 = x0 - __builtin_bit_cast(float, h << 16), r1 = x1 - __builtin_bit_cast(float, h & 0xffff0000u);
    const float2_t rv = {r0, r1};
    m = __builtin_bit_cast(unsigned, __builtin_convertvector(rv, bf16x2));
    const float s0 = r0 - __builtin_bit_cast(float, m << 16), s1 = r1 - __builtin_bit_cast(float, m & 0xffff0000u);
    const float2_t sv = {s0, s1};
    l = __builtin_bit_cast(unsigned, __builtin_convertvector(sv, bf16x2));
}

__device__ __forceinline__ void split2h(float x0, float x1, float s, unsigned &h, unsigned &l) {
    const float2_t v = {x0 * s, x1 * s};
    const f16x2 hh = __builtin_convertvector(v, f16x2);
    h = __builtin_bit_cast(unsigned, hh);
    const float2_t hf = __builtin_convertvector(hh, float2_t);
    const float2_t r = {v.x - hf.x, v.y - hf.y};
    l = __builtin_bit_cast(unsigned, __builtin_convertvector(r, f16x2));
}

__device__ __forceinline__ void split2h_resid(float x0, float x1, float s, unsigned &h, unsigned &l) {
    const float2_t v = {x0 * s, x1 * s};
    const f16x2 hh = __builtin_convertvector(v, f16x2);
    const float2_t hf = __builtin_convertvector(hh, float2_t);
    const float2_t r = {v.x - hf.x, v.y - hf.y};
    const f16x2 ll = __builtin_convertvector(r, f16x2);
    const float2_t lf = __builtin_convertvector(ll, float2_t);
    constexpr float K = (float)(1 << RESID_SHIFT);
    const float2_t r2 = {(r.x - lf.x) * K, (r.y - lf.y) * K};
    const f16x2 h2 = __builtin_convertvector(r2, f16x2);
    h = __builtin_bit_cast(unsigned, h2);
    const float2_t h2f = __builtin_convertvector(h2, float2_t);
    const float2_t q = {r2.x - h2f.x, r2.y - h2f.y};
    l = __builtin_bit_cast(unsigned, __builtin_convertvector(q, f16x2));
}

constexpr int BM3 = 128;

template <int WGN, int F_LDS, int NB, int PL, bool GUARD = false>
__device__ __forceinline__ void gconv3_body(const GParams &p, const unsigned block) {
    static_assert(PL == 2 || PL == 3, "operand planes: 2 (fp16 pairs) or 3 (bf16 triples)");
    static_assert(!GUARD || PL == 2, "the range guard belongs to the fp16-pair form");
    bool tripped = false;
    if constexpr (PL == 2) tripped = guard_tripped(p.a_amax, p.a_guard);
    if constexpr (GUARD) { if (!tripped) return; }
    constexpr int BM = BM3, BN = 64 * WGN, NT = 128 * WGN;
    constexpr int ROWS_PP = NT / 4;
    constexpr int A_PASSES = 2 * BM / ROWS_PP;
    constexpr int HALF_PASSES = A_PASSES / 2;
    constexpr int A_STAGE = PL * 2 * BM * 16;
    constexpr int B_STAGE = PL * 2 * BN * 16;
    constexpr int NA = 3;
    static_assert(NB == 3 || NB == 4, "weight ring of 3 or 4 stages");
    constexpr int ASETS = NB - 1;
    constexpr int B_BASE = NA * A_STAGE;
    constexpr int B_CHUNKS_PER_WAVE = PL;
    constexpr int KLIST = 1024;
    constexpr bool PP = WGN == 4;
    static_assert(A_PASSES == 2 || A_PASSES == 4, "two halves of a slice per thread");
    __shared__ __attribute__((aligned(16))) unsigned char smem[NA * A_STAGE + NB * B_STAGE + ((F_LDS + 1) * BM + BM + 8) * 4 + KLIST * 2];
    int *Is = reinterpret_cast<int *>(smem + NA * A_STAGE + NB * B_STAGE);
    int *Vs = Is + (F_LDS + 1) * BM;
    int *tapmask_s = Vs + BM;
    unsigned short *Ks = reinterpret_cast<unsigned short *>(tapmask_s + 8);

    int tile_m, tile_n;
    tile_coords(p, tile_m, tile_n, block);
    if (tile_m < 0) return;
    const int64_t m0 = (int64_t)tile_m * BM;
    const int n0 = tile_n * BN;
    const int t = threadIdx.x, lane = t & 63;
    const int wave = __builtin_amdgcn_readfirstlane(t >> 6);
    const int wm = wave / WGN, wn = wave % WGN;
    const int li = lane & 31, hi = lane >> 5;

    const bool probe = p.clock_probe && (block & 63) == 0 && t == 0;
    long long probe_c = 0, probe_w = 0;
    if (probe) { probe_c = (long long)__builtin_readcyclecounter(); probe_w = (long long)__builtin_amdgcn_s_memrealtime(); }

    if (p.tile_idx && p.tile_bm == BM) {
        const int32_t *ti = p.tile_idx + (int64_t)tile_m * p.F * BM;
        if (t < 8) tapmask_s[t] = p.tile_mask[(int64_t)tile_m * 8 + t];
        for (int r = t; r < BM; r += NT) {
            const int64_t m = m0 + r;
            Vs[r] = (m < p.M) ? (p.row_perm ? p.row_perm[m] : (int)m) : -1;
        }
        for (int i = t; i < (F_LDS + 1) * BM; i += NT) {
            const int row = (i < p.F * BM) ? ti[i] : -1;
            Is[i] = row >= 0 ? row * (int)(p.lda * 4) : (int)0x80000000;
        }
    } else {
        if (t < 8) tapmask_s[t] = 0;
        for (int r = t; r < BM; r += NT) {
            const int64_t m = m0 + r;
            Vs[r] = (m < p.M) ? (p.row_perm ? p.row_perm[m] : (int)m) : -1;
        }
        __syncthreads();
        int mybits = 0;
        for (int i = t; i < F_LDS * BM; i += NT) {
            const int f = i / BM, r = i - f * BM;
            const int v = Vs[r];
            int row = -1;
            if (v >= 0 && f < p.F) row = p.nbr ? p.nbr[(int64_t)f * p.nbr_stride + v] : (int)((int64_t)f * p.reg_stride + v);
            Is[i] = row >= 0 ? row * (int)(p.lda * 4) : (int)0x80000000;
            mybits |= (row >= 0) ? (1 << f) : 0;
        }
        for (int i = F_LDS * BM + t; i < (F_LDS + 1) * BM; i += NT) Is[i] = (int)0x80000000;
        if (mybits) {
            atomicOr(tapmask_s, mybits);
            atomicOr(tapmask_s + 2 + ((t % BM) >> 5), mybits);
        }
    }
    __syncthreads();
    const int tapmask = __builtin_amdgcn_readfirstlane(tapmask_s[0]);
    const bool blockskip = p.C >= BK;
    int bmask[2];
#pragma unroll
    for (int i = 0; i < 2; ++i) bmask[i] = __builtin_amdgcn_readfirstlane(tapmask_s[2 + wm * 2 + i]);
    const int nk = (p.K + BK - 1) / BK;
    if (wave == 0) {
        int count = 0;
        for (int base = 0; base < nk; base += 64) {
            const int kt = base + lane;
            bool need = false;
            int f_lo = 0;
            if (kt < nk) {
                f_lo = (kt * BK) / p.C;
                const int f_hi = min((kt * BK + BK - 1) / p.C, p.F - 1);
                int bits = 0;
                for (int f = f_lo; f <= f_hi; ++f) bits |= 1 << f;
                need = (tapmask & bits) != 0;
            }
            const unsigned long long bal = __ballot(need);
            if (need) {
                int e = kt;
                e |= (f_lo << 10) | ((blockskip && (kt * BK + BK - 1) / p.C > f_lo && f_lo + 1 < p.F) ? (1 << 14) : 0);
                Ks[count + __popcll(bal & ((1ull << lane) - 1ull))] = (unsigned short)e;
            }
            count += __popcll(bal);
        }
        if (lane == 0) tapmask_s[1] = count;
    }
    __syncthreads();
    int nsl = __builtin_amdgcn_readfirstlane(tapmask_s[1]);
    int split = 0;
    if (p.splits > 1) {
        const int ngrid = p.row_perm && p.col_share > 0 ? p.tiles_n * p.col_share * p.col_rows : p.tiles_m * p.tiles_n;
        split = (int)block / ngrid;
        const int k_lo = (int)((int64_t)nk * split / p.splits), k_hi = (int)((int64_t)nk * (split + 1) / p.splits);
        auto below = [&](int kt) {
            int a = 0, b = nsl;
            while (a < b) {
                const int mid = (a + b) >> 1;
                if ((int)(Ks[mid] & 1023) < kt) a = mid + 1; else b = mid;
            }
            return a;
        };
        const int lo = below(k_lo), hi_e = below(k_hi);
        __syncthreads();
        if (lo > 0) {
            unsigned short mine[KLIST / (128 * WGN) + 1];
            int cnt = 0;
            for (int i = t; i < hi_e - lo; i += NT) mine[cnt++] = Ks[lo + i];
            __syncthreads();
            cnt = 0;
            for (int i = t; i < hi_e - lo; i += NT) Ks[i] = mine[cnt++];
        }
        __syncthreads();
        nsl = hi_e - lo;
    }

    constexpr unsigned OOB = 0x80000000u;
    const int32x4_t rsrc_a = make_rsrc(p.A, (int)p.a_bytes);
    const int k4 = t & 3, arow0 = t >> 2;
    const unsigned w3_bytes = (unsigned)(p.w_bytes / 2);
    __amdgpu_buffer_rsrc_t rsrc_b[PL];
#pragma unroll
    for (int pl = 0; pl < PL; ++pl)
        rsrc_b[pl] = __builtin_amdgcn_make_buffer_rsrc(
            const_cast<unsigned char *>(reinterpret_cast<const unsigned char *>(p.Wt3) + (int64_t)pl * p.w3_plane_stride),
            (short)0, (int)w3_bytes, 0x00020000);
    const unsigned ldw16 = (unsigned)p.ldw * 16u;

    float4_t ra[ASETS][A_PASSES];
    int a_rows[A_PASSES], a_c[A_PASSES];
    auto load_a_rows = [&](int e) {
        const int f0 = (e >> 10) & 15;
        const int c0 = (e & 1023) * BK - f0 * p.C;
#pragma unroll
        for (int i = 0; i < A_PASSES; ++i) {
            int c = c0 + ((i & 1) * 4 + k4) * 4, f = f0;
            const bool wrap = c >= p.C;
            c = wrap ? c - p.C : c;
            f += wrap ? 1 : 0;
            a_rows[i] = Is[f * BM + arow0 + (i >> 1) * ROWS_PP];
            a_c[i] = c;
        }
    };
    auto load_a_issue = [&](auto set_tag) {
        constexpr int SET = decltype(set_tag)::value;
        const int32x4_t rs = rsrc_a;
#pragma unroll
        for (int i = 0; i < A_PASSES; ++i) {
            float4_t &dst = ra[SET][i];
            const unsigned o = (unsigned)a_rows[i] + (unsigned)a_c[i] * 4u;
            asm volatile("buffer_load_dwordx4 %0, %1, %2, 0 offen" : "=v"(dst) : "v"(o), "s"(rs) : "memory");
        }
    };
    auto load_a = [&](auto set_tag, int e) {
        load_a_rows(e);
        load_a_issue(set_tag);
    };
    auto pin = [&](auto set_tag) {
        constexpr int SET = decltype(set_tag)::value;
#pragma unroll
        for (int i = 0; i < A_PASSES; ++i) {
            float4_t &x = ra[SET][i];
            asm volatile("" : "+v"(x));
        }
    };
    auto a_slot = [](int row, int kb) { return row ^ ((((row >> 5) & 3) << 1) ^ (kb << 2)); };
    const int kb_w = (t >> 1) & 1;
    float s_a = 1.f, s_out = 1.f, s_out2 = 1.f;
    if constexpr (PL == 2) {
        s_a = split_scale(p.a_amax[0]);
        s_out = split_unscale(s_a);
        if constexpr (GUARD) s_out *= 1.0f / (float)(1 << RESID_SHIFT);
        s_out2 = split_unscale(split_scale(p.w_amax[0]));
    }
    auto store_a = [&](auto set_tag, int h, int st, int j) {
        constexpr int SET = decltype(set_tag)::value;
        const float4_t v = h ? ra[SET][2 * j + 1] : ra[SET][2 * j];
        const int row = arow0 + j * ROWS_PP;
        unsigned char *base = smem + st * A_STAGE + (kb_w * BM + a_slot(row, kb_w)) * 16 + (t & 1) * 8;
        if constexpr (PL == 2) {
            unsigned h0, l0, h1, l1;
            if constexpr (GUARD) {
                split2h_resid(v.x, v.y, s_a, h0, l0);
                split2h_resid(v.z, v.w, s_a, h1, l1);
            } else {
                split2h(v.x, v.y, s_a, h0, l0);
                split2h(v.z, v.w, s_a, h1, l1);
            }
            *reinterpret_cast<u32x2 *>(base) = u32x2{h0, h1};
            *reinterpret_cast<u32x2 *>(base + 2 * BM * 16) = u32x2{l0, l1};
        } else {
            unsigned h0, m0_, l0, h1, m1, l1;
            split2(v.x, v.y, h0, m0_, l0);
            split2(v.z, v.w, h1, m1, l1);
            *reinterpret_cast<u32x2 *>(base) = u32x2{h0, h1};
            *reinterpret_cast<u32x2 *>(base + 2 * BM * 16) = u32x2{m0_, m1};
            *reinterpret_cast<u32x2 *>(base + 4 * BM * 16) = u32x2{l0, l1};
        }
    };
    const unsigned b_colofs = ((unsigned)(n0 + wn * 64 + lane) < (unsigned)p.ldw) ? (unsigned)(n0 + wn * 64 + lane) * 16u : OOB;
    auto load_b = [&](int kt, int h, int st) {
        const unsigned kbg = (unsigned)(kt * (BK / 8) + h * 2 + wm);
        const unsigned off = kbg * ldw16 + b_colofs;
#pragma unroll
        for (int pl = 0; pl < PL; ++pl)
            __builtin_amdgcn_raw_ptr_buffer_load_lds(
                rsrc_b[pl],
                (__attribute__((address_space(3))) void *)(smem + B_BASE + st * B_STAGE + ((pl * 2 + wm) * BN + wn * 64) * 16),
                16, (int)off, 0, 0, 0);
    };

    floatx16 acc[2][2];
#pragma unroll
    for (int i = 0; i < 2; ++i)
#pragma unroll
        for (int j = 0; j < 2; ++j)
#pragma unroll
            for (int r = 0; r < 16; ++r) acc[i][j][r] = 0.f;

    unsigned a_rofs[2];
#pragma unroll
    for (int i = 0; i < 2; ++i) {
        const int row = wm * 64 + i * 32 + li;
        a_rofs[i] = (unsigned)((hi * BM + (row ^ ((((row >> 5) & 3) << 1) ^ (hi << 2)))) * 16);
    }
    const unsigned b_rofs = (unsigned)(B_BASE + (hi * BN + wn * 64 + li) * 16);

    using S0 = std::integral_constant<int, 0>;
    using S1 = std::integral_constant<int, 1>;
    using T = std::true_type;
    using Fl = std::false_type;
    auto wait_vm_lgkm0 = [](auto n_tag) {
        constexpr int N = decltype(n_tag)::value;
        __builtin_amdgcn_s_waitcnt((N & 0xF) | ((N >> 4) << 14) | (0x7 << 4) | (0x0 << 8));
    };

    using S2 = std::integral_constant<int, 2>;
    if (nsl > 0) {
        int ks_cb = 0;
        int ks_reg = (int)Ks[min(lane, KLIST - 1)];
        auto ks_at = [&](int x) { return __builtin_amdgcn_readlane(ks_reg, x - ks_cb); };
        auto ks_advance = [&](int sl) {
            if (sl - ks_cb >= 32) { ks_cb += 32; ks_reg = (int)Ks[min(ks_cb + lane, KLIST - 1)]; }
        };
        auto kt_at = [&](int sl) { return ks_at(sl) & 1023; };
#pragma unroll
        for (int g = 0; g < NB - 1; ++g)
            if (g / 2 < nsl) load_b(kt_at(g / 2), g & 1, g);
        load_a(S0{}, ks_at(0));
        wait_vm_lgkm0(S0{});
        pin(S0{});
#pragma unroll
        for (int j = 0; j < HALF_PASSES; ++j) { store_a(S0{}, 0, 0, j); store_a(S0{}, 1, 1, j); }
        if (nsl > 1) load_a(S1{}, ks_at(1));
        if constexpr (ASETS == 3) { if (nsl > 2) load_a(S2{}, ks_at(2)); }
        wait_vm_lgkm0(S0{});
        asm volatile("s_barrier" ::: "memory");

        if (PP && wm == 1) asm volatile("s_barrier" ::: "memory");

        int sta = 0, stb = 0;
        auto halfstep = [&](int e_cur, int h, auto b_tag, int kt_b, int hb_b, auto w_tag, auto setw_tag, auto l_tag, auto setl_tag,
                            int kt_l, auto inflight_tag) {
            constexpr bool B = decltype(b_tag)::value, W = decltype(w_tag)::value, L = decltype(l_tag)::value;
            const int sta2 = sta >= 1 ? sta - 1 : 2;
            const int stb2 = stb >= 1 ? stb - 1 : NB - 1;
            const unsigned char *sa = smem + sta * A_STAGE;
            const unsigned char *sb = smem + stb * B_STAGE;
            bool need[2];
            {
                const int f_lo = (e_cur >> 10) & 15, two = (e_cur >> 14) & 1;
#pragma unroll
                for (int i = 0; i < 2; ++i)
                    need[i] = !blockskip || (((bmask[i] >> f_lo) | (two ? (bmask[i] >> (f_lo + 1)) : 0)) & 1);
            }
            u32x4 af[PL][2], bf[PL][2];
            constexpr int NQ = PL == 3 ? 6 : 3;
            constexpr int PA[6] = {0, 0, 1, 0, PL == 3 ? 2 : 0, 1};
            constexpr int PB[6] = {0, 1, 0, PL == 3 ? 2 : 0, 0, 1};
            auto mfma = [&](const u32x4 &a, const u32x4 &b, floatx16 &c) {
                if constexpr (PL == 3)
                    c = __builtin_amdgcn_mfma_f32_32x32x16_bf16(__builtin_bit_cast(bf16x8, b), __builtin_bit_cast(bf16x8, a), c, 0, 0, 0);
                else
                    c = __builtin_amdgcn_mfma_f32_32x32x16_f16(__builtin_bit_cast(f16x8, b), __builtin_bit_cast(f16x8, a), c, 0, 0, 0);
            };
            if constexpr (PP) {
#pragma unroll
                for (int pl = 0; pl < PL; ++pl)
#pragma unroll
                    for (int i = 0; i < 2; ++i) {
                        af[pl][i] = *reinterpret_cast<const u32x4 *>(sa + a_rofs[i] + pl * 2 * BM * 16);
                        bf[pl][i] = *reinterpret_cast<const u32x4 *>(sb + b_rofs + pl * 2 * BN * 16 + i * 32 * 16);
                    }
                wait_vm_lgkm0(inflight_tag);
                __builtin_amdgcn_sched_barrier(0);
                asm volatile("s_barrier" ::: "memory");
                __builtin_amdgcn_sched_barrier(0);
                auto others = [&]() {
                    if constexpr (B) load_b(kt_b, hb_b, stb2);
                    if constexpr (L) { load_a_issue(setl_tag); load_a_rows(kt_l); }
                    if constexpr (W) {
                        if (h == 0) pin(setw_tag);
#pragma unroll
                        for (int j = 0; j < HALF_PASSES; ++j) store_a(setw_tag, h, sta2, j);
                    }
                };
                if (need[0] || need[1]) {
#pragma unroll
                    for (int q = 0; q < NQ; ++q)
#pragma unroll
                        for (int i = 0; i < 2; ++i)
#pragma unroll
                            for (int j = 0; j < 2; ++j) mfma(af[PA[q]][i], bf[PB[q]][j], acc[i][j]);
                    others();
#pragma unroll
                    for (int k = 0; k < 4 * NQ; ++k) {
                        __builtin_amdgcn_sched_group_barrier(0x008, 1, 0);
                        __builtin_amdgcn_sched_group_barrier(0x006, 4, 0);
                        if (k % 3 == 0) __builtin_amdgcn_sched_group_barrier(0x020, 1, 0);
                        if (k % 4 == 1) __builtin_amdgcn_sched_group_barrier(0x100, 1, 0);
                        if (k % 4 == 3) __builtin_amdgcn_sched_group_barrier(0x200, 1, 0);
                    }
                } else {
                    others();
                }
                __builtin_amdgcn_sched_barrier(0);
                asm volatile("s_barrier" ::: "memory");
                __builtin_amdgcn_sched_barrier(0);
                sta = sta == 2 ? 0 : sta + 1;
                stb = stb == NB - 1 ? 0 : stb + 1;
                return;
            }
            if (need[0] || need[1]) {
#pragma unroll
                for (int pl = 0; pl < PL; ++pl)
#pragma unroll
                    for (int i = 0; i < 2; ++i) {
                        af[pl][i] = *reinterpret_cast<const u32x4 *>(sa + a_rofs[i] + pl * 2 * BM * 16);
                        bf[pl][i] = *reinterpret_cast<const u32x4 *>(sb + b_rofs + pl * 2 * BN * 16 + i * 32 * 16);
                    }
            }
            if constexpr (B) load_b(kt_b, hb_b, stb2);
            if constexpr (L) load_a_rows(kt_l);
            if constexpr (W) { if (h == 0) pin(setw_tag); }
            auto rest = [&]() {
                if constexpr (L) load_a_issue(setl_tag);
                if constexpr (W) {
#pragma unroll
                    for (int j = 0; j < HALF_PASSES; ++j) store_a(setw_tag, h, sta2, j);
                }
            };
            if (need[0] || need[1]) {
#pragma unroll
                for (int q = 0; q < NQ; ++q)
#pragma unroll
                    for (int i = 0; i < 2; ++i)
#pragma unroll
                        for (int j = 0; j < 2; ++j) mfma(af[PA[q]][i], bf[PB[q]][j], acc[i][j]);
                rest();
#pragma unroll
                for (int k = 0; k < 4 * NQ; ++k) {
                    __builtin_amdgcn_sched_group_barrier(0x008, 1, 0);
                    __builtin_amdgcn_sched_group_barrier(0x006, 4, 0);
                    if (k % 4 == 0) __builtin_amdgcn_sched_group_barrier(0x020, 1, 0);
                    if (k % 4 == 3) __builtin_amdgcn_sched_group_barrier(0x200, 1, 0);
                }
            } else {
                rest();
            }
            wait_vm_lgkm0(inflight_tag);
            asm volatile("s_barrier" ::: "memory");
            sta = sta == 2 ? 0 : sta + 1;
            stb = stb == NB - 1 ? 0 : stb + 1;
        };
        constexpr int NLB = B_CHUNKS_PER_WAVE, NLA = A_PASSES;
        auto slice_steady = [&](int sl, auto u_tag) {
            constexpr int U = decltype(u_tag)::value;
            using SW = std::integral_constant<int, (U + 1) % ASETS>;
            using SL = std::integral_constant<int, U % ASETS>;
            ks_advance(sl);
            const int e = ks_at(sl);
            const int k1 = kt_at(sl + 1), kl = ks_at(sl + ASETS);
            if constexpr (PP) {
                halfstep(e, 0, T{}, k1, 1, T{}, SW{}, T{}, SL{}, ks_at(sl + ASETS + 1), std::integral_constant<int, NLB>{});
                halfstep(e, 1, T{}, kt_at(sl + 2), 0, T{}, SW{}, Fl{}, SL{}, 0, std::integral_constant<int, NLB + NLA>{});
            } else
            if constexpr (NB == 3) {
                halfstep(e, 0, T{}, k1, 0, T{}, SW{}, T{}, SL{}, kl, std::integral_constant<int, NLB + NLA>{});
                halfstep(e, 1, T{}, k1, 1, T{}, SW{}, Fl{}, SL{}, 0, std::integral_constant<int, NLB>{});
            } else {
                halfstep(e, 0, T{}, k1, 1, T{}, SW{}, T{}, SL{}, kl, std::integral_constant<int, 2 * NLB + NLA>{});
                halfstep(e, 1, T{}, kt_at(sl + 2), 0, T{}, SW{}, Fl{}, SL{}, 0, std::integral_constant<int, 2 * NLB + NLA>{});
            }
        };
        auto slice_tail = [&](int sl, auto u_tag) {
            constexpr int U = decltype(u_tag)::value;
            using SW = std::integral_constant<int, (U + 1) % ASETS>;
            using SL = std::integral_constant<int, U % ASETS>;
            using Z = std::integral_constant<int, 0>;
            ks_advance(sl);
            const int e = ks_at(sl);
            const bool w = sl + 1 < nsl, l = sl + ASETS < nsl;
            const int kl = l ? ks_at(sl + ASETS + (PP ? 1 : 0)) : 0;
            {
                const int gb = 2 * sl + NB - 1;
                const bool b = gb / 2 < nsl;
                const int kb = b ? kt_at(gb / 2) : 0;
                if (b && w && l) halfstep(e, 0, T{}, kb, gb & 1, T{}, SW{}, T{}, SL{}, kl, Z{});
                else if (b && w) halfstep(e, 0, T{}, kb, gb & 1, T{}, SW{}, Fl{}, SL{}, 0, Z{});
                else if (w) halfstep(e, 0, Fl{}, 0, 0, T{}, SW{}, Fl{}, SL{}, 0, Z{});
                else if (b) halfstep(e, 0, T{}, kb, gb & 1, Fl{}, SW{}, Fl{}, SL{}, 0, Z{});
                else halfstep(e, 0, Fl{}, 0, 0, Fl{}, SW{}, Fl{}, SL{}, 0, Z{});
            }
            {
                const int gb = 2 * sl + 1 + NB - 1;
                const bool b = gb / 2 < nsl;
                const int kb = b ? kt_at(gb / 2) : 0;
                if (b && w) halfstep(e, 1, T{}, kb, gb & 1, T{}, SW{}, Fl{}, SL{}, 0, Z{});
                else if (w) halfstep(e, 1, Fl{}, 0, 0, T{}, SW{}, Fl{}, SL{}, 0, Z{});
                else if (b) halfstep(e, 1, T{}, kb, gb & 1, Fl{}, SW{}, Fl{}, SL{}, 0, Z{});
                else halfstep(e, 1, Fl{}, 0, 0, Fl{}, SW{}, Fl{}, SL{}, 0, Z{});
            }
        };
        if constexpr (PP) load_a_rows(ks_at(ASETS));
        int sl = 0;
        for (; sl + 2 * ASETS < nsl; sl += ASETS) {
            slice_steady(sl, S0{});
            slice_steady(sl + 1, S1{});
            if constexpr (ASETS == 3) slice_steady(sl + 2, S2{});
        }
        for (; sl < nsl; sl += ASETS) {
            slice_tail(sl, S0{});
            if (sl + 1 < nsl) slice_tail(sl + 1, S1{});
            if constexpr (ASETS == 3) { if (sl + 2 < nsl) slice_tail(sl + 2, S2{}); }
        }
        if (PP && wm == 0) asm volatile("s_barrier" ::: "memory");
    }
    if constexpr (PL == 2) {
#pragma unroll
        for (int i = 0; i < 2; ++i)
#pragma unroll
            for (int j = 0; j < 2; ++j)
#pragma unroll
                for (int r = 0; r < 16; ++r) acc[i][j][r] = acc[i][j][r] * s_out * s_out2;
    }
    if constexpr (GUARD) {
        if (p.guard_trips && t == 0 && tile_m == 0 && tile_n == 0 && split == 0) atomicAdd(p.guard_trips, 1);
    }
    const bool defer = !GUARD && tripped;

    typedef int int32x4v __attribute__((ext_vector_type(4)));
    const bool fast_epi = p.epi_fast != 0;
    if (fast_epi) {
        const __amdgpu_buffer_rsrc_t rs_y = __builtin_amdgcn_make_buffer_rsrc(
            p.splits > 1 ? (void *)(p.partial + (int64_t)split * p.M * p.N) : (void *)p.Y, (short)0, 0x7fffffff, 0x00020000);
        const __amdgpu_buffer_rsrc_t rs_r = __builtin_amdgcn_make_buffer_rsrc(
            p.res ? (void *)const_cast<float *>(p.res) : (void *)p.Y, (short)0, p.res ? 0x7fffffff : 0, 0x00020000);
        const __amdgpu_buffer_rsrc_t rs_y2 = __builtin_amdgcn_make_buffer_rsrc(
            p.Y2 ? (void *)p.Y2 : (void *)p.Y, (short)0, (p.Y2 && p.splits <= 1) ? 0x7fffffff : 0, 0x00020000);
        const unsigned ldy_b = (unsigned)(p.splits > 1 ? p.N : p.ldy) * 4u, ldr_b = (unsigned)p.ldres * 4u, ldy2_b = (unsigned)p.ldy2 * 4u;
        const bool plain = p.splits <= 1;
        unsigned ymax = 0;
        unsigned gmin = 0xffffffffu;
        const bool want_guard = p.y_guard && p.y_amax && plain && !defer;
        const bool res_wrap = p.res && p.res_mod < p.M;
        const float res_inv = res_wrap ? 1.0f / (float)p.res_mod : 0.f;
        const bool has_res = p.res != nullptr && plain;
        const bool has_y2 = p.Y2 != nullptr && plain && !defer;
        int mrow[2];
        unsigned yrow[2], rrow[2], y2row[2];
#pragma unroll
        for (int i = 0; i < 2; ++i) {
            const int m = Vs[wm * 64 + i * 32 + li];
            mrow[i] = m;
            int rr = m;
            if (res_wrap) {
                const int q = (int)((float)rr * res_inv);
                rr -= (int)__umul24((unsigned)q, (unsigned)p.res_mod);
                rr = rr < 0 ? rr + (int)p.res_mod : (rr >= (int)p.res_mod ? rr - (int)p.res_mod : rr);
            }
            yrow[i] = __umul24((unsigned)m, ldy_b);
            rrow[i] = __umul24((unsigned)rr, ldr_b);
            y2row[i] = __umul24((unsigned)m, ldy2_b);
        }
        auto at = [&](int m, unsigned row_b, int n) { return (m >= 0 && n < p.N) ? row_b + (unsigned)n * 4u : OOB; };
        auto col_of = [&](int j, int q) { return n0 + wn * 64 + j * 32 + 8 * q + 4 * hi; };
        u32x4 rv[2][2][4];
        if (has_res) {
#pragma unroll
            for (int i = 0; i < 2; ++i)
#pragma unroll
                for (int j = 0; j < 2; ++j)
#pragma unroll
                    for (int q = 0; q < 4; ++q)
                        rv[i][j][q] = __builtin_amdgcn_raw_buffer_load_b128(rs_r, (int)at(mrow[i], rrow[i], col_of(j, q)), 0, 0);
        }
#pragma unroll
        for (int i = 0; i < 2; ++i) {
            unsigned rowmax = 0;
#pragma unroll
            for (int j = 0; j < 2; ++j)
#pragma unroll
                for (int q = 0; q < 4; ++q) {
                    const int n = col_of(j, q);
                    float4_t bs = {0.f, 0.f, 0.f, 0.f};
                    if (p.bias && plain && n < p.N) bs = *reinterpret_cast<const float4_t *>(p.bias + n);
                    float v[4] = {acc[i][j][4 * q + 0], acc[i][j][4 * q + 1], acc[i][j][4 * q + 2], acc[i][j][4 * q + 3]};
// ... 1 lines not shown
                    const unsigned rr4[4] = {rv[i][j][q].x, rv[i][j][q].y, rv[i][j][q].z, rv[i][j][q].w};
                    u32x4 o;
                    unsigned ob[4];
                    const bool live = mrow[i] >= 0 && n < p.N;
#pragma unroll
                    for (int c = 0; c < 4; ++c) {
                        float x = v[c];
                        if (plain) {
                            x = x + bb[c];
                            if (has_res) x += __builtin_bit_cast(float, rr4[c]);
                            if (p.act == HPL_ACT_LEAKY && !defer) x = x > 0.f ? x : p.slope * x;
                        }
                        ob[c] = __builtin_bit_cast(unsigned, x);
                        const unsigned av = live ? (ob[c] & 0x7fffffffu) : 0u;
                        ymax = max(ymax, av);
                        rowmax = max(rowmax, av);
                    }
                    o.x = ob[0]; o.y = ob[1]; o.z = ob[2]; o.w = ob[3];
                    __builtin_amdgcn_raw_buffer_store_b128(o, rs_y, (int)at(mrow[i], yrow[i], n), 0, 0);
                    if (has_y2) __builtin_amdgcn_raw_buffer_store_b128(o, rs_y2, (int)at(mrow[i] < (int)p.rows2 ? mrow[i] : -1, y2row[i], n), 0, 0);
                }
            if (want_guard) {
                rowmax = max(rowmax, (unsigned)__shfl_xor((int)rowmax, 32));
                gmin = rowmax ? min(gmin, rowmax) : gmin;
            }
        }
        if (p.y_amax && plain && !defer) {
#pragma unroll
            for (int o = 32; o > 0; o >>= 1) ymax = max(ymax, (unsigned)__shfl_xor((int)ymax, o));
            unsigned inv = 0u;
            if (want_guard) {
                inv = gmin == 0xffffffffu ? 0u : ~gmin;
#pragma unroll
                for (int o = 16; o > 0; o >>= 1) inv = max(inv, (unsigned)__shfl_xor((int)inv, o));
            }
            __syncthreads();
            unsigned *red = reinterpret_cast<unsigned *>(smem);
            if (lane == 0) { red[2 * wave] = ymax; red[2 * wave + 1] = inv; }
            __syncthreads();
            if (t == 0) {
#pragma unroll
                for (int w = 1; w < NT / 64; ++w) { ymax = max(ymax, red[2 * w]); inv = max(inv, red[2 * w + 1]); }
                amax_publish(reinterpret_cast<unsigned *>(p.y_amax), ymax);
                if (want_guard) amax_publish(p.y_guard, inv);
            }
        }
    } else
#pragma unroll
    for (int i = 0; i < 2; ++i)
#pragma unroll
        for (int j = 0; j < 2; ++j) {
            const int64_t m = Vs[wm * 64 + i * 32 + li];
            if (m < 0) continue;
            const int res_mod = (int)p.res_mod;
#pragma unroll
            for (int r = 0; r < 16; ++r) {
                const int n = n0 + wn * 64 + j * 32 + (r & 3) + 8 * (r >> 2) + 4 * hi;
                if (n >= p.N) continue;
                const float bsv = p.bias ? p.bias[n] : 0.f;
                if (p.splits > 1) {
                    p.partial[((int64_t)split * p.M + m) * p.N + n] = acc[i][j][r];
                    continue;
                }
                float v = acc[i][j][r] + bsv;
                if (p.res) v += p.res[(int64_t)((int)m < res_mod ? (int)m : (int)m % res_mod) * p.ldres + n];
                if (p.act == HPL_ACT_LEAKY && !defer) v = v > 0.f ? v : p.slope * v;
                p.Y[m * p.ldy + n] = v;
                if (p.Y2 && m < p.rows2 && !defer) p.Y2[m * p.ldy2 + n] = v;
            }
        }
    if (probe) {
        atomicAdd(reinterpret_cast<unsigned long long *>(p.clock_probe),
                  (unsigned long long)((long long)__builtin_readcyclecounter() - probe_c));
        atomicAdd(reinterpret_cast<unsigned long long *>(p.clock_probe) + 1,
                  (unsigned long long)((long long)__builtin_amdgcn_s_memrealtime() - probe_w));
    }
}

template <int WGN, int F_LDS, int PL, int NB = 3, bool GUARD = false>
__global__ void __launch_bounds__(128 * WGN, 2) k_gconv3(const GParams p) {
    gconv3_body<WGN, F_LDS, NB, PL, GUARD>(p, blockIdx.x);
}

template <int F_LDS, int NB, int PL, bool GUARD = false>
__global__ void __launch_bounds__(512, 2) k_gconv3w(const GParams p) {
    gconv3_body<4, F_LDS, NB, PL, GUARD>(p, blockIdx.x);
}

__global__ void __launch_bounds__(256) k_weight_split3(const float *__restrict__ Wt, int64_t k_rows, int64_t ldw,
                                                        unsigned char *__restrict__ dst, int64_t plane_stride) {
    const int64_t total = (k_rows / 8) * ldw;
    int64_t i = (int64_t)blockIdx.x * blockDim.x + threadIdx.x;
    const int64_t stride = (int64_t)gridDim.x * blockDim.x;
    for (; i < total; i += stride) {
        const int64_t kb = i / ldw, n = i - kb * ldw;
        float x[8];
#pragma unroll
        for (int j = 0; j < 8; ++j) x[j] = Wt[(kb * 8 + j) * ldw + n];
        u32x4 h, m, l;
        unsigned a, b, c;
        split2(x[0], x[1], a, b, c); h.x = a; m.x = b; l.x = c;
        split2(x[2], x[3], a, b, c); h.y = a; m.y = b; l.y = c;
        split2(x[4], x[5], a, b, c); h.z = a; m.z = b; l.z = c;
        split2(x[6], x[7], a, b, c); h.w = a; m.w = b; l.w = c;
        *reinterpret_cast<u32x4 *>(dst + i * 16) = h;
        *reinterpret_cast<u32x4 *>(dst + plane_stride + i * 16) = m;
        *reinterpret_cast<u32x4 *>(dst + 2 * plane_stride + i * 16) = l;
    }
}

__device__ __forceinline__ void amax_reduce(unsigned v, unsigned *slot) {
#pragma unroll
    for (int o = 32; o > 0; o >>= 1) v = max(v, (unsigned)__shfl_xor((int)v, o));
    __shared__ unsigned part[4];
    if ((threadIdx.x & 63) == 0) part[threadIdx.x >> 6] = v;
    __syncthreads();
    if (threadIdx.x == 0) {
        v = max(max(part[0], part[1]), max(part[2], part[3]));
        amax_publish(slot, v);
    }
}

template <typename V>
__global__ void __launch_bounds__(256) k_amax(const float *__restrict__ X, int64_t ld, int64_t rows, int colsv, int tpr_log, unsigned *__restrict__ slot) {
    constexpr int VW = sizeof(V) / 4;
    const int tpr = 1 << tpr_log, c0 = threadIdx.x & (tpr - 1), rpb = 256 >> tpr_log;
    unsigned v = 0;
    auto fold = [&](const V &x) {
        const unsigned *e = reinterpret_cast<const unsigned *>(&x);
#pragma unroll
        for (int u = 0; u < VW; ++u) v = max(v, e[u] & 0x7fffffffu);
    };
    const int64_t rstep = (int64_t)gridDim.x * rpb;
    int64_t r = (int64_t)blockIdx.x * rpb + (threadIdx.x >> tpr_log);
    for (; r + 3 * rstep < rows; r += 4 * rstep) {
        const float *p0 = X + r * ld, *p1 = p0 + rstep * ld, *p2 = p1 + rstep * ld, *p3 = p2 + rstep * ld;
        for (int c = c0; c < colsv; c += tpr) {
            const V a = *reinterpret_cast<const V *>(p0 + (int64_t)c * VW), b = *reinterpret_cast<const V *>(p1 + (int64_t)c * VW);
            const V d = *reinterpret_cast<const V *>(p2 + (int64_t)c * VW), f = *reinterpret_cast<const V *>(p3 + (int64_t)c * VW);
            fold(a); fold(b); fold(d); fold(f);
        }
    }
    for (; r < rows; r += rstep) {
        const float *p0 = X + r * ld;
        for (int c = c0; c < colsv; c += tpr) fold(*reinterpret_cast<const V *>(p0 + (int64_t)c * VW));
    }
    amax_reduce(v, slot);
}

template <typename V>
__global__ void __launch_bounds__(256) k_amax_rows(const float *__restrict__ X, int64_t ld, int64_t rows, int colsv, int tpr_log,
                                                   unsigned *__restrict__ slot, unsigned *__restrict__ guard) {
    constexpr int VW = sizeof(V) / 4;
    const int tpr = 1 << tpr_log, c0 = threadIdx.x & (tpr - 1), rpb = 256 >> tpr_log;
    unsigned v = 0, ginv = 0;
    auto fold = [&](unsigned &m, const V &x) {
        const unsigned *e = reinterpret_cast<const unsigned *>(&x);
#pragma unroll
        for (int u = 0; u < VW; ++u) m = max(m, e[u] & 0x7fffffffu);
    };
    auto row_done = [&](unsigned m) {
        for (int o = tpr >> 1; o > 0; o >>= 1) m = max(m, (unsigned)__shfl_xor((int)m, o));
        v = max(v, m);
        ginv = m ? max(ginv, ~m) : ginv;
    };
    const int64_t rstep = (int64_t)gridDim.x * rpb;
    for (int64_t r = (int64_t)blockIdx.x * rpb + (threadIdx.x >> tpr_log); r < rows; r += 4 * rstep) {
        const int64_t r1 = r + rstep < rows ? r + rstep : r, r2 = r + 2 * rstep < rows ? r + 2 * rstep : r, r3 = r + 3 * rstep < rows ? r + 3 * rstep : r;
        const float *p0 = X + r * ld, *p1 = X + r1 * ld, *p2 = X + r2 * ld, *p3 = X + r3 * ld;
        unsigned m0 = 0, m1 = 0, m2 = 0, m3 = 0;
        for (int c = c0; c < colsv; c += tpr) {
            const V a = *reinterpret_cast<const V *>(p0 + (int64_t)c * VW), b = *reinterpret_cast<const V *>(p1 + (int64_t)c * VW);
            const V d = *reinterpret_cast<const V *>(p2 + (int64_t)c * VW), f = *reinterpret_cast<const V *>(p3 + (int64_t)c * VW);
            fold(m0, a); fold(m1, b); fold(m2, d); fold(m3, f);
        }
        row_done(m0); row_done(m1); row_done(m2); row_done(m3);
    }
#pragma unroll
    for (int o = 32; o > 0; o >>= 1) ginv = max(ginv, (unsigned)__shfl_xor((int)ginv, o));
    __shared__ unsigned gpart[4];
    if ((threadIdx.x & 63) == 0) gpart[threadIdx.x >> 6] = ginv;
    amax_reduce(v, slot);
    if (threadIdx.x == 0) amax_publish(guard, max(max(gpart[0], gpart[1]), max(gpart[2], gpart[3])));
}

__global__ void k_amax_clear(const hpl_split3_job *__restrict__ jobs, int njobs) {
    for (int j = threadIdx.x; j < njobs; j += blockDim.x)
        if (jobs[j].planes == 2 && jobs[j].amax) *jobs[j].amax = 0.f;
}

__global__ void __launch_bounds__(256) k_amax_batch(const hpl_split3_job *__restrict__ jobs) {
    const hpl_split3_job jb = jobs[blockIdx.y];
    unsigned v = 0;
    if (jb.planes == 2) {
        const int64_t total4 = jb.k_rows * jb.ldw / 4;
        const uint4 *X = reinterpret_cast<const uint4 *>(jb.Wt);
        for (int64_t i = (int64_t)blockIdx.x * 256 + threadIdx.x; i < total4; i += (int64_t)gridDim.x * 256) {
            const uint4 x = X[i];
            v = max(max(v, x.x & 0x7fffffffu), max(max(x.y & 0x7fffffffu, x.z & 0x7fffffffu), x.w & 0x7fffffffu));
        }
    }
    amax_reduce(v, reinterpret_cast<unsigned *>(jb.amax ? jb.amax : const_cast<float *>(jb.Wt)));
}

__device__ __forceinline__ void split2h_store(const float *x, float sc, unsigned char *dst, int64_t plane_stride, int64_t i) {
    u32x4 h, l;
    unsigned a, b;
    split2h(x[0], x[1], sc, a, b); h.x = a; l.x = b;
    split2h(x[2], x[3], sc, a, b); h.y = a; l.y = b;
    split2h(x[4], x[5], sc, a, b); h.z = a; l.z = b;
    split2h(x[6], x[7], sc, a, b); h.w = a; l.w = b;
    *reinterpret_cast<u32x4 *>(dst + i * 16) = h;
    *reinterpret_cast<u32x4 *>(dst + plane_stride + i * 16) = l;
}

__global__ void __launch_bounds__(256) k_weight_split2h(const float *__restrict__ Wt, int64_t k_rows, int64_t ldw,
                                                         unsigned char *__restrict__ dst, int64_t plane_stride,
                                                         const float *__restrict__ amax) {
    const float sc = split_scale(amax[0]);
    const int64_t total = (k_rows / 8) * ldw;
    for (int64_t i = (int64_t)blockIdx.x * 256 + threadIdx.x; i < total; i += (int64_t)gridDim.x * 256) {
        const int64_t kb = i / ldw, n = i - kb * ldw;
        float x[8];
#pragma unroll
        for (int j = 0; j < 8; ++j) x[j] = Wt[(kb * 8 + j) * ldw + n];
        split2h_store(x, sc, dst, plane_stride, i);
    }
}

}

__global__ void __launch_bounds__(256) k_weight_split3_batch(const hpl_split3_job *__restrict__ jobs) {
    const hpl_split3_job jb = jobs[blockIdx.y];
    const float *Wt = jb.Wt;
    unsigned char *dst = reinterpret_cast<unsigned char *>(jb.dst);
    const int64_t ldw = jb.ldw, total = (jb.k_rows / 8) * ldw;
    const float sc = jb.planes == 2 ? split_scale(jb.amax[0]) : 1.f;
    for (int64_t i = (int64_t)blockIdx.x * 256 + threadIdx.x; i < total; i += (int64_t)gridDim.x * 256) {
        const int64_t kb = i / ldw, n = i - kb * ldw;
        float x[8];
#pragma unroll
        for (int j = 0; j < 8; ++j) x[j] = Wt[(kb * 8 + j) * ldw + n];
        if (jb.planes == 2) { split2h_store(x, sc, dst, jb.plane_stride, i); continue; }
        u32x4 h, m, l;
        unsigned a, b, c;
        split2(x[0], x[1], a, b, c); h.x = a; m.x = b; l.x = c;
        split2(x[2], x[3], a, b, c); h.y = a; m.y = b; l.y = c;
        split2(x[4], x[5], a, b, c); h.z = a; m.z = b; l.z = c;
        split2(x[6], x[7], a, b, c); h.w = a; m.w = b; l.w = c;
        *reinterpret_cast<u32x4 *>(dst + i * 16) = h;
        *reinterpret_cast<u32x4 *>(dst + jb.plane_stride + i * 16) = m;
        *reinterpret_cast<u32x4 *>(dst + 2 * jb.plane_stride + i * 16) = l;
    }
}

extern "C" int hpl_weight_split3_batch(const hpl_split3_job *jobs, int njobs, int64_t max_elems, int any_pairs, hplStream stream) {
    HPL_REQUIRE(jobs && njobs > 0 && njobs <= 65535 && max_elems > 0, "hpl_weight_split3_batch: bad arguments");
    if (any_pairs) {
        k_amax_clear<<<1, 256, 0, to_stream(stream)>>>(jobs, njobs);
        dim3 ga((unsigned)imin(cdiv(max_elems / 4, 256), 256), (unsigned)njobs);
        k_amax_batch<<<ga, 256, 0, to_stream(stream)>>>(jobs);
    }
    dim3 grid((unsigned)imin(cdiv(max_elems / 8, 256), 2048), (unsigned)njobs);
    k_weight_split3_batch<<<grid, 256, 0, to_stream(stream)>>>(jobs);
    HPL_CHECK_LAUNCH("hpl_weight_split3_batch");
    return HPL_OK;
}

int hpl_gc::amax_launch(const float *X, int64_t ld, int64_t rows, int cols, float *slot, hipStream_t s, unsigned *guard) {
    if (rows <= 0) return HPL_OK;
    const bool vec = cols % 4 == 0 && ld % 4 == 0 && aligned16(X);
    int cv = vec ? cols / 4 : cols;
    int64_t nrows = rows;
    if (guard) {
        int tl = 0;
        while ((1 << tl) < cv && tl < 6) ++tl;
        const int rpb = 256 >> tl;
        const int grid = (int)imax(1, imin(cdiv(nrows, (int64_t)rpb * 4), 1024));
        if (vec) k_amax_rows<float4><<<grid, 256, 0, s>>>(X, ld, nrows, cv, tl, reinterpret_cast<unsigned *>(slot), guard);
        else k_amax_rows<float><<<grid, 256, 0, s>>>(X, ld, nrows, cv, tl, reinterpret_cast<unsigned *>(slot), guard);
        HPL_CHECK_LAUNCH("hpl_amax_rows");
        return HPL_OK;
    }
    if (ld == cols && (int64_t)rows * cv >= 256) {
        const int64_t total = rows * cv;
        int w = 256;
        while (total % w) w >>= 1;
        if (w >= 64) { cv = w; nrows = total / w; ld = (int64_t)w * (vec ? 4 : 1); }
    }
    int tpr_log = 0;
    while ((1 << tpr_log) < cv && tpr_log < 8) ++tpr_log;
    const int rpb = 256 >> tpr_log;
    const int grid = (int)imax(1, imin(cdiv(nrows, (int64_t)rpb * 4), 1024));
    if (vec) k_amax<float4><<<grid, 256, 0, s>>>(X, ld, nrows, cv, tpr_log, reinterpret_cast<unsigned *>(slot));
    else k_amax<float><<<grid, 256, 0, s>>>(X, ld, nrows, cv, tpr_log, reinterpret_cast<unsigned *>(slot));
    HPL_CHECK_LAUNCH("hpl_amax");
    return HPL_OK;
}

extern "C" int hpl_amax(const float *X, int64_t ld, int64_t rows, int32_t cols, float *slot, hplStream stream) {
    HPL_REQUIRE(X && slot && rows >= 0 && cols > 0 && ld >= cols, "hpl_amax: bad arguments (rows=%lld cols=%d ld=%lld)", (long long)rows, cols, (long long)ld);
    hipStream_t s = to_stream(stream);
    if (hipMemsetAsync(slot, 0, 4, s) != hipSuccess) { set_error("hpl_amax: hipMemsetAsync failed"); return HPL_EHIP; }
    return amax_launch(X, ld, rows, cols, slot, s);
}

extern "C" int hpl_amax_rows(const float *X, int64_t ld, int64_t rows, int32_t cols, float *slot, uint32_t *guard, hplStream stream) {
    HPL_REQUIRE(X && slot && guard && rows >= 0 && cols > 0 && ld >= cols, "hpl_amax_rows: bad arguments (rows=%lld cols=%d ld=%lld)", (long long)rows, cols, (long long)ld);
    hipStream_t s = to_stream(stream);
    if (hipMemsetAsync(slot, 0, 4, s) != hipSuccess || hipMemsetAsync(guard, 0, 4, s) != hipSuccess) { set_error("hpl_amax_rows: hipMemsetAsync failed"); return HPL_EHIP; }
    return amax_launch(X, ld, rows, cols, slot, s, guard);
}

extern "C" int hpl_weight_split2h(const float *Wt, int64_t k_rows, int64_t ldw, void *dst, int64_t plane_stride, float *amax,
                                  hplStream stream) {
    HPL_REQUIRE(Wt && dst && amax && k_rows > 0 && k_rows % 8 == 0 && ldw > 0 && plane_stride >= k_rows * ldw * 2 &&
                    plane_stride % 16 == 0 && aligned16(dst),
                "hpl_weight_split2h: bad arguments (k_rows=%lld ldw=%lld)", (long long)k_rows, (long long)ldw);
    const int rc = hpl_amax(Wt, ldw, k_rows, (int32_t)ldw, amax, stream);
    if (rc) return rc;
    const int grid = (int)imin(cdiv(k_rows / 8 * ldw, 256), 16384);
    k_weight_split2h<<<grid, 256, 0, to_stream(stream)>>>(Wt, k_rows, ldw, reinterpret_cast<unsigned char *>(dst), plane_stride, amax);
    HPL_CHECK_LAUNCH("hpl_weight_split2h");
    return HPL_OK;
}

extern "C" int hpl_weight_split3(const float *Wt, int64_t k_rows, int64_t ldw, void *dst, int64_t plane_stride,
                                 hplStream stream) {
    HPL_REQUIRE(Wt && dst && k_rows > 0 && k_rows % 8 == 0 && ldw > 0 && plane_stride >= k_rows * ldw * 2 &&
                    plane_stride % 16 == 0 && aligned16(dst),
                "hpl_weight_split3: bad arguments (k_rows=%lld ldw=%lld)", (long long)k_rows, (long long)ldw);
    const int grid = (int)imin(cdiv(k_rows / 8 * ldw, 256), 16384);
    k_weight_split3<<<grid, 256, 0, to_stream(stream)>>>(Wt, k_rows, ldw, reinterpret_cast<unsigned char *>(dst), plane_stride);
    HPL_CHECK_LAUNCH("hpl_weight_split3");
    return HPL_OK;
}

bool hpl_gc::split3_enabled() { return split_planes() != 0; }

int hpl_gc::split_planes() {
    static const int planes = [] {
        const char *m = getenv("HPL_MATH");
        if (m && std::string(m) == "f32") return 0;
        if (m && std::string(m) == "bf16x3") return 3;
        return 2;
    }();
    return planes;
}

bool hpl_gc::plan_split3(GParams &p, hpl_gconv_info &o) {
    if (!split3_enabled() || p.scat || p.C < 32 || p.K > 32768) return false;
    if (p.F > 15 || (p.w_bytes / (p.ldw * 4)) % 8 != 0) return false;
    constexpr int min_rows = 8192;
    constexpr int min_rows_stencil = 16384;
    constexpr int fill_tiles = 128;
    constexpr int floor_rows = 1024;
    if (p.N < 256 || p.M < floor_rows) return false;
    const int64_t tiles256 = cdiv(p.M, BM3) * cdiv(p.N, 256);
    const bool fills = tiles256 >= fill_tiles;
    if (p.F == 1 && p.M < min_rows && !fills) return false;
    int splitk = 1;
    if (p.F > 1 && p.M < min_rows_stencil && !fills) {
        constexpr int mid_split = 1;
        constexpr int mid_min_rows = 1024;
        if (p.M < mid_min_rows) return false;
        const int64_t tiles = tiles256;
        const int nk_all = (p.K + BK - 1) / BK;
        splitk = (int)imin(imin(8, 256 / imax(1, tiles)), nk_all / 16);
        const int sets = (p.planes == 2 && p.a_guard) ? 2 : 1;
        if (!mid_split || !p.ws || p.scat || splitk < 2 || (int64_t)sets * splitk * p.M * p.N * 4 > p.ws_bytes || p.N % 256 > 0) return false;
    }
    p.tiles_m = (int)cdiv(p.M, BM3);
    constexpr int wide = 256;
    constexpr int pct = 108;
    const bool bn256 = splitk > 1 || (wide == 256 && cdiv(p.N, 256) * 256 * 100 <= cdiv(p.N, 128) * 128 * pct);
    const int BN = bn256 ? 256 : 128;
    p.tiles_n = (int)cdiv(p.N, BN);
    if (p.tile_bm != BM3) p.tile_idx = nullptr;
    p.splits = 1; p.partial = nullptr;
    int grid = p.tiles_m * p.tiles_n;
    p.col_share = 0; p.col_rows = 0;
    if (splitk > 1) {
        p.splits = splitk;
        p.partial = p.ws;
    }
    if (p.row_perm) {
        int g = 8, b = p.tiles_n % 8;
        while (b) { const int tt = g % b; g = b; b = tt; }
        p.col_share = 8 / g;
        p.col_rows = p.col_share == 1 ? p.tiles_m : (int)cdiv(p.tiles_m, COL_CHUNK * p.col_share) * COL_CHUNK;
        grid = p.tiles_n * p.col_share * p.col_rows;
        constexpr int xcd_row_major = 1;
        if (xcd_row_major && p.splits <= 1 && p.tiles_n > 1 && p.tiles_n <= 8) {
            p.col_share = -1;
            p.col_rows = (int)cdiv(p.tiles_m, 8);
            grid = 8 * p.col_rows * p.tiles_n;
        }
    }
    grid *= p.splits;
    {
        const int64_t lim = (int64_t)0x7fffffff;
        const int64_t rows_y = p.M;
        p.epi_fast = (rows_y < (1 << 24) && rows_y * (p.splits > 1 ? p.N : p.ldy) * 4 < lim && p.ldy * 4 < (1 << 24) &&
                      (!p.res || (p.res_mod > 0 && p.res_mod < (1 << 24) && imin(p.res_mod, rows_y) * p.ldres * 4 < lim && p.ldres * 4 < (1 << 24))) &&
                      (!p.Y2 || (p.rows2 * p.ldy2 * 4 < lim && p.ldy2 * 4 < (1 << 24))) &&
                      p.N % 4 == 0 && (p.splits > 1 ? aligned16(p.partial) : (p.ldy % 4 == 0 && aligned16(p.Y))) && (!p.bias || aligned16(p.bias)) &&
                      (!p.res || (p.ldres % 4 == 0 && aligned16(p.res))) && (!p.Y2 || (p.ldy2 % 4 == 0 && aligned16(p.Y2)))) ? 1 : 0;
        static const int epi = getenv("HPL_SPLIT3_EPILOGUE") ? atoi(getenv("HPL_SPLIT3_EPILOGUE")) : 1;
        if (!epi) p.epi_fast = 0;
    }
    p.y_amax_done = (p.y_amax && p.epi_fast && p.splits <= 1) ? 1 : 0;
    o.family = p.planes == 2 ? HPL_FAMILY_PAIRS : HPL_FAMILY_TRIPLES;
    o.bm = BM3; o.bn = BN; o.threads = bn256 ? 512 : 256;
    o.f_lds = p.F == 1 ? 1 : (p.F <= 8 ? 8 : 15);
    o.compact = 0;
    o.splits = p.splits;
    o.guard_sets = (p.planes == 2 && p.a_guard) ? 2 : 1;
    p.guard_partials = (o.guard_sets == 2 && p.splits > 1) ? 1 : 0;
    o.col_share = p.col_share; o.col_rows = p.col_rows;
    o.tile_tables = p.tile_idx ? 1 : 0;
    o.epi_fast = p.epi_fast;
    o.tiles_m = p.tiles_m; o.tiles_n = p.tiles_n;
    o.grid = grid;
    return true;
}

void hpl_gc::launch_split3(const GParams &p, const hpl_gconv_info &o, hipStream_t s) {
    const int grid = (int)o.grid;
    const bool bn256 = o.bn == 256;
    const int fl = o.f_lds;
    if (o.family == HPL_FAMILY_PAIRS) {
        if (bn256) {
            if (fl == 1) k_gconv3w<1, 4, 2><<<grid, 512, 0, s>>>(p);
            else if (fl == 8) k_gconv3w<8, 4, 2><<<grid, 512, 0, s>>>(p);
            else k_gconv3w<15, 4, 2><<<grid, 512, 0, s>>>(p);
        } else {
            if (fl == 1) k_gconv3<2, 1, 2><<<grid, 256, 0, s>>>(p);
            else if (fl == 8) k_gconv3<2, 8, 2><<<grid, 256, 0, s>>>(p);
            else k_gconv3<2, 15, 2><<<grid, 256, 0, s>>>(p);
        }
        if (o.guard_sets == 2) {
            GParams q = p;
            const int ggrid = grid;
            if (o.splits > 1) q.partial = p.partial + (int64_t)o.splits * p.M * p.N;
            else { q.res = p.Y; q.ldres = p.ldy; q.res_mod = p.M; q.bias = nullptr; }
            if (bn256) {
                if (fl == 1) k_gconv3w<1, 4, 2, true><<<ggrid, 512, 0, s>>>(q);
                else if (fl == 8) k_gconv3w<8, 4, 2, true><<<ggrid, 512, 0, s>>>(q);
                else k_gconv3w<15, 4, 2, true><<<ggrid, 512, 0, s>>>(q);
            } else {
                if (fl == 1) k_gconv3<2, 1, 2, 3, true><<<ggrid, 256, 0, s>>>(q);
                else if (fl == 8) k_gconv3<2, 8, 2, 3, true><<<ggrid, 256, 0, s>>>(q);
                else k_gconv3<2, 15, 2, 3, true><<<ggrid, 256, 0, s>>>(q);
            }
        }
    } else if (bn256) {
        if (fl == 1) k_gconv3w<1, 4, 3><<<grid, 512, 0, s>>>(p);
        else if (fl == 8) k_gconv3w<8, 4, 3><<<grid, 512, 0, s>>>(p);
        else k_gconv3w<15, 4, 3><<<grid, 512, 0, s>>>(p);
    } else {
        if (fl == 1) k_gconv3<2, 1, 3><<<grid, 256, 0, s>>>(p);
        else if (fl == 8) k_gconv3<2, 8, 3><<<grid, 256, 0, s>>>(p);
        else k_gconv3<2, 15, 3><<<grid, 256, 0, s>>>(p);
    }
}
```

### hplflownet_amd/csrc/gconv_common.h

```cpp
#pragma once
#include "common.h"

namespace hpl_gc {

typedef float floatx16 __attribute__((ext_vector_type(16)));
typedef int int32x4_t __attribute__((ext_vector_type(4)));
typedef float float4_t __attribute__((ext_vector_type(4)));

__device__ float4_t buffer_load_f32x4(int32x4_t srsrc, int voffset, int soffset, int aux)
    __asm("llvm.amdgcn.raw.buffer.load.v4f32");


__device__ __forceinline__ int32x4_t make_rsrc(const void *base, int bytes) {
    union {
        int32x4_t v;
        struct { const void *p; int range; int cfg; } s;
    } u;
    u.s.p = base;
    u.s.range = bytes;
    u.s.cfg = 0x00020000;
    return u.v;
}

__host__ __device__ __forceinline__ float split_scale(float amax) {
    unsigned bits;
    __builtin_memcpy(&bits, &amax, 4);
    const int e = (int)((bits >> 23) & 0xffu);
    int sb = 268 - e;
    sb = sb < 2 ? 2 : (sb > 252 ? 252 : sb);
    const unsigned sbits = e == 0 ? 0x3f800000u : ((unsigned)sb << 23);
    float s;
    __builtin_memcpy(&s, &sbits, 4);
    return s;
}
__host__ __device__ __forceinline__ float split_unscale(float s) {
    unsigned bits;
    __builtin_memcpy(&bits, &s, 4);
    const unsigned ibits = (254u - ((bits >> 23) & 0xffu)) << 23;
    float r;
    __builtin_memcpy(&r, &ibits, 4);
    return r;
}

constexpr int COL_CHUNK = 4;
constexpr int BK = 32;

struct GParams {
    const float *A; int64_t lda; int64_t rows_a;
    const int32_t *nbr; int64_t nbr_stride; int64_t reg_stride;
    int64_t M; int C; int F; int K;
    const float *Wt; int64_t ldw; int N; int act; float slope;
    const float *bias; const float *res; int64_t ldres; int64_t res_mod;
    float *Y; int64_t ldy;
    const int32_t *scat; int64_t scat_stride; int scat_c;
    int tiles_m; int tiles_n;
    int64_t a_bytes; int64_t w_bytes;
    const int32_t *row_perm;
    const int32_t *tile_idx;
    const int32_t *tile_mask;
    int tile_bm;
    long long *clock_probe;
    int perm_chunk;
    int col_share;
    int col_rows;
    int splits; float *partial;
    float *Y2; int64_t ldy2; int64_t rows2;
    float *ws; int64_t ws_bytes;
    const void *Wt3; int64_t w3_plane_stride;
    int planes;
    const float *a_amax; const float *w_amax;
    float *y_amax; int y_amax_done;
    const unsigned *a_guard; unsigned *y_guard; int *guard_trips;
    int guard_partials;
    int epi_fast;
};

__device__ __forceinline__ int64_t src_row(const GParams &p, int f, int64_t m) {
    if (f >= p.F || m >= p.M) return -1;
    if (p.nbr) return (int64_t)p.nbr[(int64_t)f * p.nbr_stride + m];
    return (int64_t)f * p.reg_stride + m;
}

__device__ __forceinline__ void tile_coords(const GParams &p, int &tm, int &tn, const unsigned block) {
    const int nwg = p.tiles_m * p.tiles_n;
    const int bid = (int)block % nwg;
    const int q = nwg / 8, r = nwg % 8;
    const int xcd = bid % 8, pos = bid / 8;
    const int id = (xcd < r ? xcd * (q + 1) : r * (q + 1) + (xcd - r) * q) + pos;
    if (p.row_perm && p.col_share < 0) {
        const int x2 = (int)block % 8, pos2 = (int)block / 8;
        const int j = pos2 / p.tiles_n;
        tn = pos2 - j * p.tiles_n;
        const int row = j * 8 + x2;
        tm = row < p.tiles_m ? (p.tile_idx ? p.tile_mask[(int64_t)row * 8 + 6] : p.tiles_m - 1 - row) : -1;
        return;
    }
    if (p.row_perm && p.col_share > 0) {
        const int gsz = p.tiles_n * p.col_share * p.col_rows;
        const int q2 = gsz / 8, r2 = gsz % 8;
        const int b2 = p.splits > 1 ? (int)block % gsz : (int)block;
        const int x2 = b2 % 8, pos2 = b2 / 8;
        const int id2 = (x2 < r2 ? x2 * (q2 + 1) : r2 * (q2 + 1) + (x2 - r2) * q2) + pos2;
        const int v = id2 / p.col_rows, pos = id2 - v * p.col_rows;
        tn = v / p.col_share;
        const int sh = v - tn * p.col_share;
        const int row = p.col_share == 1 ? pos : (pos / COL_CHUNK) * COL_CHUNK * p.col_share + sh * COL_CHUNK + pos % COL_CHUNK;
        tm = row < p.tiles_m ? (p.tile_idx ? p.tile_mask[(int64_t)row * 8 + 6] : p.tiles_m - 1 - row) : -1;
        return;
    }
    if (p.row_perm) {
        const int G = p.perm_chunk;
        const int T = p.tiles_m;
        const int nchunks = (T + G - 1) / G;
        auto chunk_rows = [&](int c) { return min(G, T - c * G); };
        auto chunk_of = [&](int x, int r) { return r * 8 + ((r & 1) ? 7 - x : x); };
        int sq = id / p.tiles_n;
        tn = id - sq * p.tiles_n;
        int x = 0;
        for (; x < 8; ++x) {
            int rows_x = 0;
            for (int r = 0; r * 8 < nchunks; ++r) {
                const int c = chunk_of(x, r);
                if (c < nchunks) rows_x += chunk_rows(c);
            }
            if (sq < rows_x) break;
            sq -= rows_x;
        }
        int row = 0;
        for (int r = 0;; ++r) {
            const int c = chunk_of(x, r);
            if (c >= nchunks) continue;
            const int n = chunk_rows(c);
            if (sq < n) { row = c * G + sq; break; }
            sq -= n;
        }
        tm = T - 1 - row;
        return;
    }
    constexpr int BAND = 8;
    const int band_sz = BAND * p.tiles_n;
    const int band = id / band_sz;
    const int in_band = id - band * band_sz;
    const int rows_in_band = min(BAND, p.tiles_m - band * BAND);
    tm = band * BAND + in_band % rows_in_band;
    tn = in_band / rows_in_band;
}
__device__ __forceinline__ void tile_coords(const GParams &p, int &tm, int &tn) { tile_coords(p, tm, tn, blockIdx.x); }


int fill_params(const hpl_gconv_desc *d, GParams &p, const char *who);
bool plan_split3(GParams &p, hpl_gconv_info &o);
void launch_split3(const GParams &p, const hpl_gconv_info &o, hipStream_t s);
bool split3_enabled();
int split_planes();
int amax_launch(const float *X, int64_t ld, int64_t rows, int cols, float *slot, hipStream_t s, unsigned *guard = nullptr);
constexpr int GUARD_GAP = 18;
__device__ __forceinline__ bool guard_tripped(const float *a_amax, const unsigned *a_guard) {
    if (!a_guard || !a_amax) return false;
    unsigned am;
    const float amf = a_amax[0];
    __builtin_memcpy(&am, &amf, 4);
    const unsigned g = a_guard[0];
    const unsigned rmin = g ? ~g : am;
    return (am >> 23) >= (rmin >> 23) + (unsigned)GUARD_GAP && (am >> 23) < 255u;
}
constexpr int RESID_SHIFT = 24;
inline bool split3_maybe(int64_t M, int C, int F, int N) {
    if (!(C >= 32 && N >= 256 && M >= 1024 && F <= 15)) return false;
    const int64_t tiles256 = ((M + 127) / 128) * ((N + 255) / 256);
    if (tiles256 >= 128) return true;
    if (F == 1) return M >= 8192;
    if (M >= 16384) return true;
    const int64_t nk = ((int64_t)F * C + BK - 1) / BK;
    const int64_t by_tiles = 256 / tiles256, by_k = nk / 16;
    return N % 256 == 0 && (by_tiles < by_k ? by_tiles : by_k) >= 2;
}

struct WParams {
    const float *A; int64_t lda; const int32_t *nbr; int64_t nbr_stride; int64_t reg_stride;
    int64_t M; int C; int F; int K;
    const float *dY; int64_t lddy; int N;
    float *dWt; int64_t ldw;
    int tiles_n; int64_t m_per_split;
    const int32_t *tap_m; const int32_t *tap_row; const int32_t *tap_ptr; int c_tiles;
    float *dbias;
    int64_t rows_a;
    const float *a_amax; const float *dy_amax;
};
bool plan_wgrad3(WParams &p, bool tap, int64_t m_len, hpl_wgrad_info &o);
void launch_wgrad3(const WParams &p, const hpl_wgrad_info &o, hipStream_t s);

}
```

### hplflownet_amd/ops.py

```python
import collections
import ctypes
import os

import torch

from . import _lib
from ._lib import GConvDesc, RelayoutJob, check, ptr, stream

ACT_NONE, ACT_LEAKY = 0, 1
LEAKY_RATE = 0.1


def _cl(x, what='activation'):
    if x.dim() != 2 or x.dtype != torch.float32 or not x.is_cuda or (x.shape[1] > 1 and x.stride(1) != 1):
        raise _lib.HplError('%s must be a channel-last 2-D float32 device tensor with unit channel stride, '
                            'got shape %s strides %s dtype %s device %s'
                            % (what, tuple(x.shape), x.stride(), x.dtype, x.device))
    return x


def _ld(x):
    return x.stride(0) if x.shape[0] > 1 else max(x.shape[1], x.stride(0))


# ... 1011 lines not shown

    def __init__(self, W, F, up0, up_w, Wb, bias_a, bias_b, ones_col, own_bias, dense_bias):
        self.src = (W, Wb, bias_a, bias_b, own_bias)
        self.args = (F, up0, up_w, ones_col, dense_bias)
        self.ptrs = self._ptrs()
        self._keep = [None if p is None else p.detach() for p in self.src]
        O = W.shape[0]
        Cout = W.numel() // (O * F) - up_w + Wb.numel() // up_w + (4 if ones_col >= 0 else 0)
        self.weight = torch.empty((O, Cout) + tuple(W.shape[2:]), dtype=torch.float32, device=W.device)
        self.bias = torch.empty((O,), dtype=torch.float32, device=W.device) if dense_bias else None
        self._sig = None
        self._ev = self._stream = None

    def _ptrs(self):
        return tuple(None if p is None else p.data_ptr() for p in self.src)

    def made_of(self, src, args):
        return args == self.args and all(a is b for a, b in zip(src, self.src)) and self._ptrs() == self.ptrs

    def ensure(self):
        sig = (weight_epoch(),) + tuple(None if p is None else p._version for p in self.src)
        if sig != self._sig:
            F, up0, up_w, ones_col, dense_bias = self.args
            W, Wb, ba, bb, own = [None if p is None else p.detach() for p in self.src]
            with torch.no_grad():
                self.weight, self.bias = weight_fold(W, F, up0, up_w, Wb, ba, bb, ones_col, own, dense_bias, out=self.weight,
                                                     out_bias=self.bias)
            if self._sig is not None:
                torch.autograd.graph.increment_version(self.weight)
                if self.bias is not None:
                    torch.autograd.graph.increment_version(self.bias)
            self._sig = sig
            self._ev = torch.cuda.Event()
            self._ev.record()
            self._stream = stream()
        elif self._ev is not None and stream() != self._stream:
            if self._ev.query():
                self._ev = None
            else:
                torch.cuda.current_stream().wait_event(self._ev)
        return self


class SplitW(object):
    __slots__ = ('planes', 'amax', 'P')

    def __init__(self, planes, amax, P):
        self.planes, self.amax, self.P = planes, amax, P

    def rows_from(self, k0, ldw):
        return SplitW(self.planes[:, (k0 // 8) * ldw * 16:], self.amax, self.P)


def weight_split3(Wt, out=None, planes=None):
    k_rows, ldw = Wt.shape
    if k_rows % 8 or not Wt.is_contiguous():
        raise _lib.HplError('weight_split3: image must be contiguous with a multiple of 8 rows, got %s' % (tuple(Wt.shape),))
    P = out.P if out is not None else (planes or SPLIT_PLANES)
    if out is None:
        out = SplitW(torch.empty((P, k_rows // 8 * ldw * 16), dtype=torch.uint8, device=Wt.device),
                     torch.zeros(1, dtype=torch.float32, device=Wt.device) if P == 2 else None, P)
    if P == 2:
        check(_lib.load().hpl_weight_split2h(ptr(Wt), k_rows, ldw, ptr(out.planes), out.planes.stride(0), ptr(out.amax), stream()),
              'hpl_weight_split2h')
    else:
        check(_lib.load().hpl_weight_split3(ptr(Wt), k_rows, ldw, ptr(out.planes), out.planes.stride(0), stream()), 'hpl_weight_split3')
    return out


def amax(X, rows=None, cols=None):
    p_, ld, r, c = _mat(X, 'amax input')
    out = torch.empty(1, dtype=torch.float32, device=X.device)
    check(_lib.load().hpl_amax(p_, ld, r if rows is None else rows, c if cols is None else cols, ptr(out), stream()), 'hpl_amax')
    return out


def amax_rows(X, rows=None, cols=None):
    p_, ld, r, c = _mat(X, 'amax input')
    out = torch.empty(1, dtype=torch.float32, device=X.device)
    guard = torch.empty(1, dtype=torch.int32, device=X.device)
    check(_lib.load().hpl_amax_rows(p_, ld, r if rows is None else rows, c if cols is None else cols, ptr(out), ptr(guard), stream()),
          'hpl_amax_rows')
    return out, guard


def _mat(x, what, dev=True):
    st, sh = x.stride(), x.shape
    if len(st) != 2 or x.dtype is not torch.float32 or (dev and not x.is_cuda) or (st[1] != 1 and sh[1] > 1):
        raise _lib.HplError('%s must be a channel-last 2-D float32 device tensor with unit channel stride, '
                            'got shape %s strides %s dtype %s device %s' % (what, tuple(sh), st, x.dtype, x.device))
    return x.data_ptr(), (st[0] if sh[0] > 1 else max(sh[1], st[0])), sh[0], sh[1]


def _gconv_desc(A, nbr, M, C, F, Wt, N, bias, act, res, res_mod, out, scat, scat_c, slope, row_perm, split_k, reg_stride, tiles,
                out2, rows2, Wt3, y_amax, guard, y_guard, guard_trips, query=False):
    dev = not query
    ptr = _addr if query else _lib.ptr
    keep = None
    d = GConvDesc()
    d.A, d.lda, d.rows_a, a_cols = _mat(A, 'activation', dev)
    if nbr is not None:
        nst, nsh = nbr.stride(), nbr.shape
        if nbr.dtype is not torch.int32 or len(nsh) != 2 or nsh[0] != F or nsh[1] != M or nst[1] != 1:
            raise _lib.HplError('neighbour table must be int32 [F=%d, M=%d] with unit column stride, got %s %s'
                                % (F, M, tuple(nsh), nbr.dtype))
        d.nbr, d.nbr_stride = ptr(nbr), nst[0]
    elif F != 1:
        if reg_stride <= 0 or (F - 1) * reg_stride + M > d.rows_a:
            raise _lib.HplError('F > 1 needs a neighbour table or a regular stride inside A (F=%d stride=%d M=%d '
                                'rows=%d)' % (F, reg_stride, M, d.rows_a))
        d.reg_stride = reg_stride
    d.M, d.C, d.F = M, C, F
    if C > a_cols:
        raise _lib.HplError('C=%d exceeds the %d channels of A' % (C, a_cols))
    wsh = Wt.shape
    if wsh[0] < F * C or wsh[1] < N or not Wt.is_contiguous():
        raise _lib.HplError('Wt %s too small for K=%d N=%d' % (tuple(wsh), F * C, N))
    d.Wt, d.ldw, d.N = ptr(Wt), wsh[1], N
    d.w_rows = min(wsh[0], round_up(F * C, 32))
    d.act, d.slope = act, slope
    if Wt3 is not None:
        if Wt3.P == 3:
            d.Wt3, d.wt3_plane_stride, d.wt3_planes = ptr(Wt3.planes), Wt3.planes.stride(0), 3
        elif scat is None and split3_maybe(M, C, F, N):
            if query:
                d.a_amax = _QUERY_PTR
                if guard:
                    d.a_guard = _QUERY_PTR
            elif guard:
                keep = amax_rows(A, cols=C)
                d.a_amax, d.a_guard = ptr(keep[0]), ptr(keep[1])
                if guard_trips is not None:
                    d.guard_trips = ptr(guard_trips)
            else:
                keep = amax(A, cols=C)
                d.a_amax = ptr(keep)
            d.Wt3, d.wt3_plane_stride, d.wt3_planes = ptr(Wt3.planes), Wt3.planes.stride(0), 2
            d.w_amax = ptr(Wt3.amax)
    if bias is not None:
        d.bias = ptr(bias)
    if res is not None:
        d.res, d.ldres, rrows, _ = _mat(res, 'res', dev)
        d.res_mod = res_mod or rrows
    if scat is not None:
        if out is None:
            raise _lib.HplError('scatter epilogue needs a zero-initialised `out`')
        d.scat, d.scat_stride, d.scat_c = ptr(scat), scat.stride(0), scat_c
    elif out is None and not query:
        out = torch.empty((M, N), dtype=torch.float32, device=A.device)
    if out is None:
        d.Y, d.ldy = _QUERY_PTR, N
    else:
        d.Y, d.ldy, _, _ = _mat(out, 'out', dev)
    if out2 is not None:
        d.Y2, d.ldy2, r2, c2 = _mat(out2, 'out2', dev)
        if scat is not None or rows2 > r2 or c2 < N:
            raise _lib.HplError('second destination: %d rows x %d columns for rows2=%d N=%d' % (r2, c2, rows2, N))
        d.rows2 = rows2
    if y_amax is not None:
        d.y_amax = ptr(y_amax)
        if y_guard is not None:
            d.y_guard = ptr(y_guard)
    if row_perm is not None:
        if row_perm.dtype is not torch.int32 or row_perm.numel() != M or not row_perm.is_contiguous():
            raise _lib.HplError('row_perm must be a contiguous int32 tensor of M=%d entries' % M)
        d.row_perm = ptr(row_perm)
        if tiles is not None:
            d.tile_idx, d.tile_mask, d.tile_bm = ptr(tiles[0]), ptr(tiles[1]), tiles[0].shape[2]
        if CLOCK_PROBE is not None and N > 64 and M >= 16384:
            d.clock_probe = CLOCK_PROBE.data_ptr()
    st = None if query else stream()
    if split_k and scat is None and M * N <= _SPLITK_MAX_ELEMS:
        if query:
            d.ws, d.ws_bytes = _QUERY_PTR, _SPLITK_WS_FLOATS * 4
        else:
            ws = _splitk_workspace(A.device, st)
            d.ws, d.ws_bytes = ws.data_ptr(), ws.numel() * 4
    return d, out, st, keep


def gconv_raw(A, nbr, M, C, F, Wt, N, bias=None, act=ACT_NONE, res=None, res_mod=0, out=None,
              scat=None, scat_c=0, naive=False, slope=LEAKY_RATE, row_perm=None, split_k=True, reg_stride=0, tiles=None,
              out2=None, rows2=0, Wt3=None, y_amax=None, guard=True, y_guard=None, guard_trips=None):
    d, out, st, _keep = _gconv_desc(A, nbr, M, C, F, Wt, N, bias, act, res, res_mod, out, scat, scat_c, slope, row_perm, split_k,
                                    reg_stride, tiles, out2, rows2, Wt3, y_amax, guard, y_guard, guard_trips)
    lib = _lib.load()
    rc = (lib.hpl_gconv_forward_naive if naive else lib.hpl_gconv_forward)(ctypes.byref(d), st)
    if rc != 0:
        check(rc, 'hpl_gconv_forward')
    return out


def _info_dict(info):
    return {name: getattr(info, name) for name, _ in info._fields_ if name != 'pad_'}


def gconv_launch_info(A, nbr, M, C, F, Wt, N, bias=None, act=ACT_NONE, res=None, res_mod=0, out=None,
                      scat=None, scat_c=0, slope=LEAKY_RATE, row_perm=None, split_k=True, reg_stride=0, tiles=None,
                      out2=None, rows2=0, Wt3=None, y_amax=None, guard=True, y_guard=None, guard_trips=None):
    d = _gconv_desc(A, nbr, M, C, F, Wt, N, bias, act, res, res_mod, out, scat, scat_c, slope, row_perm, split_k,
                    reg_stride, tiles, out2, rows2, Wt3, y_amax, guard, y_guard, guard_trips, query=True)[0]
    info = _lib.GConvInfo()
    check(_lib.load().hpl_gconv_launch_info(ctypes.byref(d), ctypes.byref(info)), 'hpl_gconv_launch_info')
    return _info_dict(info)


def _addr(t):
    return None if t is None else t.data_ptr()


_QUERY_PTR = 256

CLOCK_PROBE = None

_SPLITK_MAX_ELEMS = 8 << 20
_SPLITK_WS = {}
_SPLITK_WS_FLOATS = 16 << 20


def _splitk_workspace(device, st):
    key = (device, st)
    ws = _SPLITK_WS.get(key)
    if ws is None:
        ws = _SPLITK_WS[key] = torch.empty(_SPLITK_WS_FLOATS, dtype=torch.float32, device=device)
    return ws


def _wgrad_args(A, nbr, M, C, F, dY, N, taps, want_bias, reg_stride, query=False):
    ptr = _addr if query else _lib.ptr
    if not query:
        A, dY = _cl(A), _cl(dY, 'dY')
    kp, ldw = round_up(F * C, 32), round_up(N, 4)
    if query:
        dWt, gb = None, None
        p_dWt, p_gb = _QUERY_PTR, (_QUERY_PTR + kp * ldw * 4 if want_bias else None)
    else:
        buf = torch.zeros(kp * ldw + (ldw if want_bias else 0), dtype=torch.float32, device=A.device)
        dWt = buf[:kp * ldw].view(kp, ldw)
        gb = buf[kp * ldw:kp * ldw + N] if want_bias else None
        p_dWt, p_gb = ptr(dWt), ptr(gb)
    tl, tr, tp = taps if (taps is not None and nbr is not None) else (None, None, None)
    sa = sd = keep = None
    if SPLIT_PLANES == 2 and SPLIT3 and N >= 256 and C >= 128 and M >= 8192 and (tl is not None or (F == 1 and nbr is None)):
        if query:
            sa = sd = _QUERY_PTR
        else:
            keep = (amax(A, cols=C), amax(dY, rows=M, cols=N))
            sa, sd = ptr(keep[0]), ptr(keep[1])
    return (ptr(A), _ld(A), A.shape[0], ptr(nbr), nbr.stride(0) if nbr is not None else 0,
            reg_stride if nbr is None else 0, M, C, F, ptr(dY), _ld(dY), N, p_dWt, ldw,
            ptr(tl), ptr(tr), ptr(tp), M if tl is not None else 0, p_gb, sa, sd), dWt, gb, keep


def wgrad_raw(A, nbr, M, C, F, dY, N, taps=None, want_bias=False, reg_stride=0):
    args, dWt, gb, _keep = _wgrad_args(A, nbr, M, C, F, dY, N, taps, want_bias, reg_stride)
    check(_lib.load().hpl_gconv_wgrad_scaled(*(args + (stream(),))), 'hpl_gconv_wgrad')
    return (dWt, gb) if want_bias else dWt


def wgrad_launch_info(A, nbr, M, C, F, dY, N, taps=None, want_bias=False, reg_stride=0):
    args = _wgrad_args(A, nbr, M, C, F, dY, N, taps, want_bias, reg_stride, query=True)[0]
    info = _lib.WGradInfo()
    check(_lib.load().hpl_wgrad_launch_info(*(args + (ctypes.byref(info),))), 'hpl_wgrad_launch_info')
    return _info_dict(info)


def colsum(X):
    X = _cl(X)
    out = torch.empty(X.shape[1], dtype=torch.float32, device=X.device)
    check(_lib.load().hpl_colsum(ptr(X), _ld(X), X.shape[0], X.shape[1], ptr(out), stream()), 'hpl_colsum')
    return out


def leaky_bwd(dY, Y, slope=LEAKY_RATE, amax=None):
    dY, Y = _cl(dY, 'dY'), _cl(Y, 'Y')
    dX = torch.empty(tuple(Y.shape), dtype=torch.float32, device=Y.device)
    check(_lib.load().hpl_leaky_bwd_amax(ptr(dY), _ld(dY), ptr(Y), _ld(Y), slope, ptr(dX), _ld(dX), Y.shape[0],
                                         Y.shape[1], ptr(amax), stream()), 'hpl_leaky_bwd')
    return dX


class SplatFn(torch.autograd.Function):

    @staticmethod
    def forward(ctx, feat, cloud, use_norm):
        ctx.cloud, ctx.use_norm = cloud, use_norm
# ... 377 lines not shown
```

### include/hpl_bcl.h

```cpp
#ifndef HPL_BCL_H
#define HPL_BCL_H

#include <stdint.h>

#ifdef __cplusplus
extern "C" {
#endif

#define HPL_OK 0
#define HPL_EINVAL (-1)
#define HPL_EHIP (-2)
#define HPL_ENODEV (-3)

#define HPL_ACT_NONE 0
#define HPL_ACT_LEAKY 1

typedef void *hplStream;

int hpl_version(void);
const char *hpl_last_error(void);
int hpl_device_info(int device, int *cu_count, int *wave_size, char *arch, int arch_len);

int hpl_index_narrow(const int64_t *src, int32_t *dst, int64_t n, hplStream stream);

// ... 54 lines not shown
    int64_t k_rows, ldw, plane_stride;
    float *amax;
    int32_t planes;
    int32_t pad_;
} hpl_split3_job;
int hpl_weight_split3_batch(const hpl_split3_job *jobs , int njobs, int64_t max_elems, int any_pairs,
                            hplStream stream);

int hpl_weight_unlayout(const float *Wt, int64_t ldw, int R, int Q, int F, float *W, int64_t base,
                        int64_t sr, int64_t sq, int64_t sf, int accumulate, hplStream stream);

typedef struct hpl_gconv_desc {
    const float *A;
    int64_t lda;
    int64_t rows_a;
    const int32_t *nbr;
    int64_t nbr_stride;
    int64_t reg_stride;
    int64_t M;
    int32_t C;
    int32_t F;
    const float *Wt;
    int64_t ldw;
    int32_t N;
    int32_t act;
    float slope;
    const float *bias;
    const float *res;
    int64_t ldres;
    int64_t res_mod;
    float *Y;
    int64_t ldy;
    const int32_t *scat;
    int64_t scat_stride;
    int32_t scat_c;
    int32_t w_rows;
    const int32_t *row_perm;
    float *ws;
    int64_t ws_bytes;
    const int32_t *tile_idx;
    const int32_t *tile_mask;
    int32_t tile_bm;
    int64_t *clock_probe;
    float *Y2;
    int64_t ldy2;
    int64_t rows2;
    const void *Wt3;
    int64_t wt3_plane_stride;
    int32_t wt3_planes;
    const float *a_amax;
    const float *w_amax;
    float *y_amax;
    const uint32_t *a_guard;
    uint32_t *y_guard;
    int32_t *guard_trips;
} hpl_gconv_desc;

int hpl_amax(const float *X, int64_t ld, int64_t rows, int32_t cols, float *slot, hplStream stream);
int hpl_amax_rows(const float *X, int64_t ld, int64_t rows, int32_t cols, float *slot, uint32_t *guard, hplStream stream);

int64_t hpl_tap_order_scratch_ints(int64_t M);
int hpl_tap_order(const int32_t *nbr, int64_t nbr_stride, int F, int64_t M, int32_t *perm,
                  int32_t *scratch, hplStream stream);
int hpl_tile_index(const int32_t *nbr, int64_t nbr_stride, int F, int64_t M, const int32_t *row_perm, int BM,
                   int32_t *tile_idx, int32_t *tile_mask, hplStream stream);

int hpl_gconv_forward(const hpl_gconv_desc *desc , hplStream stream);
int hpl_gconv_forward_naive(const hpl_gconv_desc *desc , hplStream stream);

int hpl_gconv_wgrad(const float *A, int64_t lda, int64_t rows_a, const int32_t *nbr,
                    int64_t nbr_stride, int64_t reg_stride, int64_t M, int C, int F,
                    const float *dY, int64_t lddy, int N, float *dWt, int64_t ldw,
                    const int32_t *tap_m, const int32_t *tap_row, const int32_t *tap_ptr,
                    int64_t tap_max, float *dbias, hplStream stream);
int hpl_gconv_wgrad_scaled(const float *A, int64_t lda, int64_t rows_a, const int32_t *nbr,
                           int64_t nbr_stride, int64_t reg_stride, int64_t M, int C, int F,
                           const float *dY, int64_t lddy, int N, float *dWt, int64_t ldw,
                           const int32_t *tap_m, const int32_t *tap_row, const int32_t *tap_ptr,
                           int64_t tap_max, float *dbias, const float *a_amax, const float *dy_amax, hplStream stream);

#define HPL_FAMILY_FP32 0
#define HPL_FAMILY_PAIRS 2
#define HPL_FAMILY_TRIPLES 3
#define HPL_FINISH_NONE 0
#define HPL_FINISH_SCALAR 1
#define HPL_FINISH_VEC4 2
typedef struct hpl_gconv_info {
    int32_t family;
    int32_t bm, bn;
    int32_t threads;
    int32_t avec;
    int32_t f_lds;
    int32_t compact;
    int32_t splits;
    int32_t guard_sets;
    int32_t col_share;
    int32_t col_rows;
    int32_t tile_tables;
    int32_t epi_fast;
    int32_t finish;
    int32_t tiles_m, tiles_n;
    int64_t grid;
} hpl_gconv_info;
int hpl_gconv_launch_info(const hpl_gconv_desc *desc , hpl_gconv_info *info );

#define HPL_WBIAS_NONE 0
#define HPL_WBIAS_KERNEL 1
#define HPL_WBIAS_COLSUM 2
typedef struct hpl_wgrad_info {
    int32_t family;
    int32_t bn;
    int32_t vec;
    int32_t tap;
    int32_t threads;
    int32_t deep;
    int32_t tiles_k, tiles_n;
    int32_t bias;
    int32_t pad_;
    int64_t tiles;
    int64_t splits;
    int64_t m_per_split;
} hpl_wgrad_info;
int hpl_wgrad_launch_info(const float *A, int64_t lda, int64_t rows_a, const int32_t *nbr,
                          int64_t nbr_stride, int64_t reg_stride, int64_t M, int C, int F,
                          const float *dY, int64_t lddy, int N, float *dWt, int64_t ldw,
                          const int32_t *tap_m, const int32_t *tap_row, const int32_t *tap_ptr,
                          int64_t tap_max, float *dbias, const float *a_amax, const float *dy_amax,
                          hpl_wgrad_info *info );

int hpl_colsum(const float *X, int64_t ld, int64_t M, int N, float *out, hplStream stream);
int hpl_leaky_bwd(const float *dY, int64_t lddy, const float *Y, int64_t ldy, float slope,
                  float *dX, int64_t lddx, int64_t M, int N, hplStream stream);
int hpl_leaky_bwd_amax(const float *dY, int64_t lddy, const float *Y, int64_t ldy, float slope,
                       float *dX, int64_t lddx, int64_t M, int N, float *amax, hplStream stream);
int hpl_psum(const float *X, int64_t ldx, int64_t rows, int64_t mod, int N, float *out, int64_t ldo, int accumulate,
             hplStream stream);
int hpl_regroup(const float *G, int64_t ldg, int64_t M, int F, int C, float *out, int64_t ldo, int accumulate,
                hplStream stream);
int hpl_epe3d(const float *pred, const float *sf, int64_t N, float *grad, float *loss, hplStream stream);
int hpl_epe3d_pairs(const float *pred, const float *sf, int batch, int64_t n, float *pair_loss, hplStream stream);
int hpl_pair_grad(const float *dflow, int64_t rows, int batch, const float *pair_loss, int loss_stride, float *grad, float *loss,
                  hplStream stream);
typedef struct hpl_metrics_pair {
    const float *pred;
    const float *gt;
    const float *pc1;
    int64_t n;
    int64_t pred_sc, pred_sp, gt_sc, gt_sp, pc1_sc, pc1_sp;
    float camera[6];
    int32_t has_camera;
    int32_t pad_;
} hpl_metrics_pair;
int hpl_flow_metrics(const hpl_metrics_pair *pairs , int batch, hpl_metrics_pair *stage, double *out,
                     hplStream stream);
typedef struct hpl_transform_params {
    float m[9];
    float shift[3];
    float m2[9];
    float shift2[3];
    double jitter_sigma1, jitter_clip1, jitter_sigma2, jitter_clip2;
    float depth_threshold;
    int32_t no_corr;
    int32_t num_points;
    int32_t allow_less_points;
    int32_t augment;
    int32_t pad_;
    uint64_t seed;
    uint64_t counter;
} hpl_transform_params;
int hpl_transform_pair(const float *pc1, const float *pc2, int64_t M, const hpl_transform_params *params ,
                       const float *jitter1, const float *jitter2, const int32_t *sel1, const int32_t *sel2, int64_t n_sel,
                       float *out_pc1, float *out_pc2, float *out_sf, int64_t capacity, int32_t *counts, void *workspace,
                       int64_t workspace_bytes, hplStream stream);
int64_t hpl_transform_workspace_bytes(int64_t M);
int hpl_transform_capacity(int64_t M, int num_points, int64_t *capacity );
int hpl_philox4x32_10(const uint32_t *counter, const uint32_t *key, uint32_t *out);
int hpl_adam_flat(float *p, const float *g, float *m, float *v, int64_t n, double lr, double beta1, double beta2, double eps,
                  int64_t step, hplStream stream);

int hpl_tap_lists(const int32_t *nbr, int64_t nbr_stride, int F, int64_t M, int32_t *list_m,
                  int32_t *list_row, int32_t *tap_ptr, int32_t *scratch, hplStream stream);

int hpl_table_symmetric(const int32_t *nbr, int64_t nbr_stride, int F, int64_t M, int32_t *flag,
                        hplStream stream);

int hpl_transpose(const float *src, int64_t lds, float *dst, int64_t ldd, int64_t rows_src,
                  int64_t cols_src, hplStream stream);
// ... 320 lines not shown
```

Baseline: 500.8 point-pairs/s.

## Pre-split gconv activations into fp16 pair planes once and reuse across convs

```diff
diff --git a/hplflownet_amd/_lib.py b/hplflownet_amd/_lib.py
--- a/hplflownet_amd/_lib.py
+++ b/hplflownet_amd/_lib.py
@@ -158,6 +158,11 @@
     'hpl_gconv_wgrad': (ctypes.c_int, [c_vp, c_i64, c_i64, c_vp, c_i64, c_i64, c_i64, ctypes.c_int, ctypes.c_int,
                                        c_vp, c_i64, ctypes.c_int, c_vp, c_i64, c_vp, c_vp, c_vp, c_i64, c_vp, c_vp]),
     'hpl_gconv_launch_info': (ctypes.c_int, [ctypes.POINTER(GConvDesc), ctypes.POINTER(GConvInfo)]),
+    'hpl_presplit_ld': (c_i64, [c_i32]),
+    'hpl_presplit_bytes': (c_i64, [c_i64, c_i32]),
+    'hpl_presplit2h': (ctypes.c_int, [c_vp, c_i64, c_i64, c_i32, c_vp, c_vp, c_vp]),
+    'hpl_gconv_forward_presplit': (ctypes.c_int, [ctypes.POINTER(GConvDesc), c_vp, c_i64, c_i64, c_vp]),
+    'hpl_gconv_launch_info_presplit': (ctypes.c_int, [ctypes.POINTER(GConvDesc), c_vp, c_i64, c_i64, ctypes.POINTER(GConvInfo)]),
     'hpl_wgrad_launch_info': (ctypes.c_int, [c_vp, c_i64, c_i64, c_vp, c_i64, c_i64, c_i64, ctypes.c_int, ctypes.c_int,
                                              c_vp, c_i64, ctypes.c_int, c_vp, c_i64, c_vp, c_vp, c_vp, c_i64, c_vp, c_vp, c_vp,
                                              ctypes.POINTER(WGradInfo)]),
diff --git a/hplflownet_amd/csrc/executor.hip b/hplflownet_amd/csrc/executor.hip
--- a/hplflownet_amd/csrc/executor.hip
+++ b/hplflownet_amd/csrc/executor.hip
@@ -104,6 +104,10 @@
     struct AmaxEnt { int buf; int64_t row_off, rows; int col_off, cols; const float *slot; bool guarded; };
     std::vector<AmaxEnt> amax;
     int amax_used = 0;
+    struct PlaneKey { int buf, row_off_sym, rows_sym, col_off, cols; int first, last; };
+    struct PlaneLive { int key; const float *slot; };
+    std::vector<PlaneKey> plane_keys;
+    std::vector<PlaneLive> planes;
     int32_t *guard_trips = nullptr;
     std::vector<int64_t> lay_sym, lay_off;
     int64_t lay_total = 0;
@@ -139,6 +143,18 @@
 
 inline int64_t buf_bytes(int64_t rows, int cols) { return (rows * cols * 4 + 255) / 256 * 256; }
 
+bool planes_candidate(const hpl_plan &pl, const hpl_op &op, const int64_t *sym) {
+    if (hpl_gc::split_planes() != 2 || hpl_gc::presplit_mode() == 0) return false;
+    if (op.kind != HPL_OP_GCONV || op.a.buf < 0 || (op.flags & (HPL_FLAG_SCATTER | HPL_FLAG_NOGUARD | HPL_FLAG_SIDE))) return false;
+    if (op.weight < 0 || op.weight >= (int)pl.weights.size() || pl.weights[op.weight].wt3_planes != 2 || !pl.weights[op.weight].Wt3) return false;
+    const int64_t M = symv(sym, op.m_sym);
+    const int F = op.F > 15 ? 15 : op.F;
+    return hpl_gc::split3_maybe(M, op.C, F, op.N) && hpl_gc::presplit_maybe(M, op.C, F, op.N);
+}
+inline bool same_view(const hpl_plan::PlaneKey &k, const hpl_op &op) {
+    return k.buf == op.a.buf && k.row_off_sym == op.a.row_off_sym && k.rows_sym == op.a.rows_sym && k.col_off == op.a.col_off && k.cols == op.C;
+}
+
 struct Runner {
     hpl_plan &pl;
     const hpl_level_tables *lv;
@@ -157,6 +173,7 @@
     const float *dflow = nullptr;
     hipStream_t main_s = nullptr, side_s = nullptr;
     bool side_busy = false;
+    char *ws_base = nullptr;
     float *amax_base = nullptr;
     const float *cur_a_amax = nullptr, *cur_b_amax = nullptr;
     float *cur_y_amax = nullptr;
@@ -189,6 +206,31 @@
         cur_y_amax = nullptr;
     }
     static bool guarded(const hpl_op &op) { return range_guard() && !(op.flags & HPL_FLAG_NOGUARD); }
+    int planes_of(const hpl_op &op, const View &A, const float *slot, const void *&planes) {
+        planes = nullptr;
+        const int nb = (int)pl.bufs.size();
+        for (int k = 0; k < (int)pl.plane_keys.size(); ++k) {
+            if (!same_view(pl.plane_keys[k], op) || pl.lay_off[nb + k] < 0) continue;
+            planes = ws_base + pl.lay_off[nb + k];
+            for (const auto &e : pl.planes)
+                if (e.key == k && e.slot == slot) return HPL_OK;
+            const int rc = hpl_presplit2h(A.p, A.ld, A.rows, op.C, slot, const_cast<void *>(planes), hs);
+            if (rc) return rc;
+            for (size_t i = 0; i < pl.planes.size();)
+                if (pl.planes[i].key == k) { pl.planes[i] = pl.planes.back(); pl.planes.pop_back(); } else ++i;
+            pl.planes.push_back({k, slot});
+            return HPL_OK;
+        }
+        return HPL_OK;
+    }
+    void planes_forget(const hpl_ref &r) {
+        if (r.buf < 0) return;
+        for (size_t i = 0; i < pl.planes.size();) {
+            const auto &k = pl.plane_keys[pl.planes[i].key];
+            if (k.buf == r.buf && k.col_off < r.col_off + r.cols && r.col_off < k.col_off + k.cols) { pl.planes[i] = pl.planes.back(); pl.planes.pop_back(); }
+            else ++i;
+        }
+    }
     float *amax_slot() { return pl.amax_used < AMAX_SLOTS ? amax_base + 2 * pl.amax_used++ : nullptr; }
     int prepare_amax(const hpl_op &op, bool side) {
         cur_a_amax = cur_b_amax = nullptr;
@@ -382,8 +424,17 @@
             if (scatter) { d.scat = t.corr2; d.scat_stride = 15 * t.H0; d.scat_c = op.aux; }
             else
             if (M * op.N <= SPLITK_ELEMS) { d.ws = splitk; d.ws_bytes = SPLITK_WS_BYTES; }
+            const void *planes = nullptr;
+            const int64_t pld = hpl_presplit_ld(op.C), prow0 = reg ? (int64_t)f0 * reg : 0;
+            if (d.Wt3 && d.wt3_planes == 2 && d.a_amax && s == main_s && (A.rows + 1) * pld < (int64_t)INT32_MAX && planes_candidate(pl, op, sym)) {
+                hpl_gconv_info info;
+                int rp = hpl_gconv_launch_info_presplit(&d, ws_base, pld, A.rows - prow0, &info);
+                if (rp) return rp;
+                if (info.family == HPL_FAMILY_PAIRS_PRESPLIT && (rp = planes_of(op, A, d.a_amax, planes))) return rp;
+            }
             bracket(prof, false);
-            const int r = hpl_gconv_forward(&d, hs);
+            const int r = planes ? hpl_gconv_forward_presplit(&d, static_cast<const char *>(planes) + prow0 * pld, pld, A.rows - prow0, hs)
+                                 : hpl_gconv_forward(&d, hs);
             bracket(prof, true);
             return r;
         };
@@ -680,12 +731,35 @@
         touch(op.a, at, side); touch(op.b, at, side); touch(op.res, at, side);
         touch(op.out, at, false); touch(op.out2, at, false);
     }
+    pl.plane_keys.clear();
+    for (int i = 0; i < nops; ++i) {
+        const hpl_op &op = pl.ops[i];
+        if (op.cond != HPL_COND_ALWAYS) {
+            if (op.cond_level < 0 || op.cond_level >= n_levels) continue;
+            const bool shrink = lv[op.cond_level].n0 < lv[op.cond_level].H0;
+            if ((op.cond == HPL_COND_SHRINK) != shrink) continue;
+        }
+        if (op.a.buf >= nb || !planes_candidate(pl, op, sym)) continue;
+        bool found = false;
+        for (auto &k : pl.plane_keys)
+            if (same_view(k, op)) { k.last = i; found = true; break; }
+        if (!found) pl.plane_keys.push_back({op.a.buf, op.a.row_off_sym, op.a.rows_sym, op.a.col_off, op.C, i, i});
+    }
+    const int np = (int)pl.plane_keys.size();
+    first.resize(nb + np); last.resize(nb + np);
     std::vector<int> order;
     for (int b = 0; b < nb; ++b) if (last[b] >= 0) order.push_back(b);
-    std::vector<int64_t> size(nb, 0);
+    std::vector<int64_t> size(nb + np, 0);
     for (int b : order) size[b] = buf_bytes(sym[pl.bufs[b].rows_sym], pl.bufs[b].cols);
+    for (int k = 0; k < np; ++k) {
+        const auto &key = pl.plane_keys[k];
+        const int64_t rows = key.rows_sym < 0 ? sym[pl.bufs[key.buf].rows_sym] - symv(sym, key.row_off_sym) : sym[key.rows_sym];
+        first[nb + k] = key.first; last[nb + k] = key.last;
+        size[nb + k] = rows > 0 ? (hpl_presplit_bytes(rows, key.cols) + 255) / 256 * 256 : 0;
+        order.push_back(nb + k);
+    }
     std::stable_sort(order.begin(), order.end(), [&](int x, int y) { return first[x] != first[y] ? first[x] < first[y] : size[x] > size[y]; });
-    pl.lay_off.assign(nb, -1);
+    pl.lay_off.assign(nb + np, -1);
     int64_t total = HEAD_BYTES;
     std::vector<std::pair<int64_t, int64_t>> busy;
     std::vector<int> placed;
@@ -777,6 +851,7 @@
     r.main_s = to_stream(stream);
     r.side_s = side_stream ? to_stream(side_stream) : nullptr;
     r.amax_base = reinterpret_cast<float *>(w + SPLITK_WS_BYTES);
+    r.ws_base = w;
     plan->fence_used = 0;
     if (!plan->guard_trips && hpl_gc::split_planes() == 2) {
         if (hipMalloc(reinterpret_cast<void **>(&plan->guard_trips), 4) != hipSuccess || hipMemsetAsync(plan->guard_trips, 0, 4, r.main_s) != hipSuccess) {
@@ -787,6 +862,7 @@
     if (op_begin == 0) {
         plan->amax.clear();
         plan->amax_used = 0;
+        plan->planes.clear();
         if (hpl_gc::split_planes() == 2 && hipMemsetAsync(r.amax_base, 0, AMAX_SLOTS * 8, r.main_s) != hipSuccess) { set_error("hpl_plan_run: hipMemsetAsync failed"); return HPL_EHIP; }
     }
     auto active = [&](const hpl_op &op, bool &run) -> int {
@@ -845,11 +921,15 @@
         if ((rc = r.prepare_amax(op, side))) return rc;
         r.amax_forget(op.out);
         r.amax_forget(op.out2);
+        r.planes_forget(op.out);
+        r.planes_forget(op.out2);
         if (side) { if ((rc = r.to_side())) return rc; }
         else if (op.kind == HPL_OP_UNLAYOUT && (rc = r.join())) return rc;
         rc = r.run_op(op);
         if (side) r.to_main();
         if (rc) return rc;
+        r.planes_forget(op.out);
+        r.planes_forget(op.out2);
         r.amax_produced(op);
     }
     if (!join) return HPL_OK;
diff --git a/hplflownet_amd/csrc/gconv.hip b/hplflownet_amd/csrc/gconv.hip
--- a/hplflownet_amd/csrc/gconv.hip
+++ b/hplflownet_amd/csrc/gconv.hip
@@ -542,6 +542,7 @@
     HPL_REQUIRE(!(d->y_amax && d->scat), "%s: y_amax with a scatter epilogue", who);
     p.col_share = 0; p.col_rows = 0;
     p.tiles_m = p.tiles_n = 0;
+    p.a_planes = nullptr; p.a_pl_ld = 0; p.a_pl_rows = 0; p.presplit = 0;
     p.a_bytes = ((d->rows_a - 1) * d->lda + d->C) * 4;
     const int64_t w_rows = d->w_rows ? (int64_t)d->w_rows : cdiv(p.K, 32) * 32;
     HPL_REQUIRE(w_rows >= p.K, "%s: w_rows=%lld < F*C=%d", who, (long long)w_rows, p.K);
@@ -678,21 +679,32 @@
 }
 }
 
-extern "C" int hpl_gconv_launch_info(const hpl_gconv_desc *d, hpl_gconv_info *info) {
-    HPL_REQUIRE(info, "hpl_gconv_launch_info: null info");
+int hpl_gc::fill_planes(GParams &p, const void *a_planes, int64_t ld_bytes, int64_t rows, const char *who) {
+    if (!a_planes) return HPL_OK;
+    HPL_REQUIRE((reinterpret_cast<uintptr_t>(a_planes) & 127) == 0 && ld_bytes >= presplit_ld(p.C) && ld_bytes % PRESPLIT_UNIT == 0 &&
+                    rows >= p.rows_a && (rows + 1) * ld_bytes < (int64_t)INT32_MAX,
+                "%s: pre-split planes (%lld rows of %lld bytes for %lld x %d of A; 128-byte aligned, below 2 GiB)", who,
+                (long long)rows, (long long)ld_bytes, (long long)p.rows_a, p.C);
+    p.a_planes = a_planes; p.a_pl_ld = ld_bytes; p.a_pl_rows = rows;
+    return HPL_OK;
+}
+
+namespace {
+int gconv_info(const hpl_gconv_desc *d, const void *planes, int64_t ld_bytes, int64_t rows, hpl_gconv_info *info, const char *who) {
+    HPL_REQUIRE(info, "%s: null info", who);
     memset(info, 0, sizeof(*info));
     GParams p;
     int rc = fill_params(d, p, "hpl_gconv_forward");
-    if (rc != HPL_OK) return rc;
+    if (rc != HPL_OK || (rc = fill_planes(p, planes, ld_bytes, rows, who)) != HPL_OK) return rc;
     if (p.M == 0) return HPL_OK;
     plan_forward(p, *info);
     return HPL_OK;
 }
 
-extern "C" int hpl_gconv_forward(const hpl_gconv_desc *d, hplStream stream) {
+int gconv_forward(const hpl_gconv_desc *d, const void *planes, int64_t ld_bytes, int64_t rows, hplStream stream) {
     GParams p;
     int rc = fill_params(d, p, "hpl_gconv_forward");
-    if (rc != HPL_OK) return rc;
+    if (rc != HPL_OK || (rc = fill_planes(p, planes, ld_bytes, rows, "hpl_gconv_forward_presplit")) != HPL_OK) return rc;
     if (p.M == 0) return HPL_OK;
     hipStream_t s = to_stream(stream);
     hpl_gconv_info o;
@@ -712,6 +724,23 @@
     HPL_CHECK_LAUNCH("hpl_gconv_forward");
     if (p.y_amax) return amax_launch(p.Y, p.ldy, p.M, p.N, p.y_amax, s, p.y_guard);
     return HPL_OK;
+}
+}
+
+extern "C" int hpl_gconv_launch_info(const hpl_gconv_desc *d, hpl_gconv_info *info) {
+    return gconv_info(d, nullptr, 0, 0, info, "hpl_gconv_launch_info");
+}
+
+extern "C" int hpl_gconv_launch_info_presplit(const hpl_gconv_desc *d, const void *planes, int64_t ld_bytes, int64_t rows,
+                                              hpl_gconv_info *info) {
+    return gconv_info(d, planes, ld_bytes, rows, info, "hpl_gconv_launch_info_presplit");
+}
+
+extern "C" int hpl_gconv_forward(const hpl_gconv_desc *d, hplStream stream) { return gconv_forward(d, nullptr, 0, 0, stream); }
+
+extern "C" int hpl_gconv_forward_presplit(const hpl_gconv_desc *d, const void *planes, int64_t ld_bytes, int64_t rows,
+                                          hplStream stream) {
+    return gconv_forward(d, planes, ld_bytes, rows, stream);
 }
 
 namespace {
diff --git a/hplflownet_amd/csrc/gconv3.hip b/hplflownet_amd/csrc/gconv3.hip
--- a/hplflownet_amd/csrc/gconv3.hip
+++ b/hplflownet_amd/csrc/gconv3.hip
@@ -57,10 +57,11 @@
 
 constexpr int BM3 = 128;
 
-template <int WGN, int F_LDS, int NB, int PL, bool GUARD = false>
+template <int WGN, int F_LDS, int NB, int PL, bool GUARD = false, int PRE = 0>
 __device__ __forceinline__ void gconv3_body(const GParams &p, const unsigned block) {
     static_assert(PL == 2 || PL == 3, "operand planes: 2 (fp16 pairs) or 3 (bf16 triples)");
     static_assert(!GUARD || PL == 2, "the range guard belongs to the fp16-pair form");
+    static_assert(!PRE || (PL == 2 && !GUARD && WGN == 4 && NB == 4), "pre-split planes: the first launch of the pair form's 8-wave tile");
     bool tripped = false;
     if constexpr (PL == 2) tripped = guard_tripped(p.a_amax, p.a_guard);
     if constexpr (GUARD) { if (!tripped) return; }
@@ -70,7 +71,7 @@
     constexpr int HALF_PASSES = A_PASSES / 2;
     constexpr int A_STAGE = PL * 2 * BM * 16;
     constexpr int B_STAGE = PL * 2 * BN * 16;
-    constexpr int NA = 3;
+    constexpr int NA = PRE ? 4 : 3;
     static_assert(NB == 3 || NB == 4, "weight ring of 3 or 4 stages");
     constexpr int ASETS = NB - 1;
     constexpr int B_BASE = NA * A_STAGE;
@@ -94,6 +95,8 @@
     const int wm = wave / WGN, wn = wave % WGN;
     const int li = lane & 31, hi = lane >> 5;
 
+    const int row_b = PRE ? (int)p.a_pl_ld : (int)(p.lda * 4);
+    const int absent_b = PRE ? (int)(p.a_pl_rows * p.a_pl_ld) : (int)0x80000000;
     const bool probe = p.clock_probe && (block & 63) == 0 && t == 0;
     long long probe_c = 0, probe_w = 0;
     if (probe) { probe_c = (long long)__builtin_readcyclecounter(); probe_w = (long long)__builtin_amdgcn_s_memrealtime(); }
@@ -107,7 +110,7 @@
         }
         for (int i = t; i < (F_LDS + 1) * BM; i += NT) {
             const int row = (i < p.F * BM) ? ti[i] : -1;
-            Is[i] = row >= 0 ? row * (int)(p.lda * 4) : (int)0x80000000;
+            Is[i] = row >= 0 ? row * row_b : absent_b;
         }
     } else {
         if (t < 8) tapmask_s[t] = 0;
@@ -122,10 +125,10 @@
             const int v = Vs[r];
             int row = -1;
             if (v >= 0 && f < p.F) row = p.nbr ? p.nbr[(int64_t)f * p.nbr_stride + v] : (int)((int64_t)f * p.reg_stride + v);
-            Is[i] = row >= 0 ? row * (int)(p.lda * 4) : (int)0x80000000;
+            Is[i] = row >= 0 ? row * row_b : absent_b;
             mybits |= (row >= 0) ? (1 << f) : 0;
         }
-        for (int i = F_LDS * BM + t; i < (F_LDS + 1) * BM; i += NT) Is[i] = (int)0x80000000;
+        for (int i = F_LDS * BM + t; i < (F_LDS + 1) * BM; i += NT) Is[i] = absent_b;
         if (mybits) {
             atomicOr(tapmask_s, mybits);
             atomicOr(tapmask_s + 2 + ((t % BM) >> 5), mybits);
@@ -285,6 +288,47 @@
                 16, (int)off, 0, 0, 0);
     };
 
+    __amdgpu_buffer_rsrc_t rsrc_ap = rsrc_b[0];
+    if constexpr (PRE)
+        rsrc_ap = __builtin_amdgcn_make_buffer_rsrc(const_cast<void *>(p.a_planes), (short)0, (int)((p.a_pl_rows + 1) * p.a_pl_ld), 0x00020000);
+    const int pre_pl = wave & 1, pre_kb = (wave >> 1) & 1;
+    constexpr int PRE_N = PRE == 2 ? 4 : 1;
+    int pre_row[PRE_N];
+#pragma unroll
+    for (int i = 0; i < PRE_N; ++i) {
+        const int slot = wm * 64 + (PRE == 2 ? i * 16 + (lane >> 2) : lane);
+        pre_row[i] = slot ^ ((((slot >> 5) & 3) << 1) ^ (pre_kb << 2));
+    }
+    int pre_off[PRE_N] = {};
+    auto pre_col = [&](int e, int h, int &f) {
+        const int f0 = (e >> 10) & 15;
+        int c = (e & 1023) * BK - f0 * p.C + h * 16 + pre_kb * 8 + (PRE == 2 ? (lane & 3) * 2 : 0);
+        const bool wrap = c >= p.C;
+        f = f0 + (wrap ? 1 : 0);
+        return wrap ? c - p.C : c;
+    };
+    auto pre_index = [&](int e, int h) {
+        int f;
+        (void)pre_col(e, h, f);
+#pragma unroll
+        for (int i = 0; i < PRE_N; ++i) pre_off[i] = Is[f * BM + pre_row[i]];
+    };
+    auto pre_issue = [&](int e, int h, int st) {
+        int f;
+        const int c = pre_col(e, h, f);
+        const unsigned colb = (unsigned)presplit_col_offset(0, 0, c & ~7, pre_pl) + (unsigned)(c & 7) * 2u;
+        unsigned char *dst = smem + st * A_STAGE + ((pre_pl * 2 + pre_kb) * BM + wm * 64) * 16;
+        if constexpr (PRE == 2) {
+#pragma unroll
+            for (int i = 0; i < PRE_N; ++i)
+                __builtin_amdgcn_raw_ptr_buffer_load_lds(rsrc_ap, (__attribute__((address_space(3))) void *)(dst + i * 256), 4,
+                                                         (int)((unsigned)pre_off[i] + colb), 0, 0, 0);
+        } else {
+            __builtin_amdgcn_raw_ptr_buffer_load_lds(rsrc_ap, (__attribute__((address_space(3))) void *)dst, 16,
+                                                     (int)((unsigned)pre_off[0] + colb), 0, 0, 0);
+        }
+    };
+
     floatx16 acc[2][2];
 #pragma unroll
     for (int i = 0; i < 2; ++i)
@@ -322,23 +366,31 @@
 #pragma unroll
         for (int g = 0; g < NB - 1; ++g)
             if (g / 2 < nsl) load_b(kt_at(g / 2), g & 1, g);
-        load_a(S0{}, ks_at(0));
-        wait_vm_lgkm0(S0{});
-        pin(S0{});
-#pragma unroll
-        for (int j = 0; j < HALF_PASSES; ++j) { store_a(S0{}, 0, 0, j); store_a(S0{}, 1, 1, j); }
-        if (nsl > 1) load_a(S1{}, ks_at(1));
-        if constexpr (ASETS == 3) { if (nsl > 2) load_a(S2{}, ks_at(2)); }
+        if constexpr (PRE) {
+#pragma unroll
+            for (int g = 0; g < NB - 1; ++g)
+                if (g / 2 < nsl) { pre_index(ks_at(g / 2), g & 1); pre_issue(ks_at(g / 2), g & 1, g); }
+            if ((NB - 1) / 2 < nsl) pre_index(ks_at((NB - 1) / 2), (NB - 1) & 1);
+        } else {
+            load_a(S0{}, ks_at(0));
+            wait_vm_lgkm0(S0{});
+            pin(S0{});
+#pragma unroll
+            for (int j = 0; j < HALF_PASSES; ++j) { store_a(S0{}, 0, 0, j); store_a(S0{}, 1, 1, j); }
+            if (nsl > 1) load_a(S1{}, ks_at(1));
+            if constexpr (ASETS == 3) { if (nsl > 2) load_a(S2{}, ks_at(2)); }
+        }
         wait_vm_lgkm0(S0{});
         asm volatile("s_barrier" ::: "memory");
 
         if (PP && wm == 1) asm volatile("s_barrier" ::: "memory");
 
         int sta = 0, stb = 0;
-        auto halfstep = [&](int e_cur, int h, auto b_tag, int kt_b, int hb_b, auto w_tag, auto setw_tag, auto l_tag, auto setl_tag,
+        auto halfstep = [&](int e_cur, int h, auto b_tag, int e_b, int hb_b, auto w_tag, auto setw_tag, auto l_tag, auto setl_tag,
                             int kt_l, auto inflight_tag) {
-            constexpr bool B = decltype(b_tag)::value, W = decltype(w_tag)::value, L = decltype(l_tag)::value;
-            const int sta2 = sta >= 1 ? sta - 1 : 2;
+            constexpr bool B = decltype(b_tag)::value, W = decltype(w_tag)::value && !PRE, L = decltype(l_tag)::value && !PRE;
+            const int kt_b = e_b & 1023;
+            const int sta2 = sta >= 1 ? sta - 1 : NA - 1;
             const int stb2 = stb >= 1 ? stb - 1 : NB - 1;
             const unsigned char *sa = smem + sta * A_STAGE;
             const unsigned char *sb = smem + stb * B_STAGE;
@@ -373,6 +425,7 @@
                 __builtin_amdgcn_sched_barrier(0);
                 auto others = [&]() {
                     if constexpr (B) load_b(kt_b, hb_b, stb2);
+                    if constexpr (B && PRE) { pre_issue(e_b, hb_b, sta2); pre_index(kt_l, h); }
                     if constexpr (L) { load_a_issue(setl_tag); load_a_rows(kt_l); }
                     if constexpr (W) {
                         if (h == 0) pin(setw_tag);
@@ -402,7 +455,7 @@
                 __builtin_amdgcn_sched_barrier(0);
                 asm volatile("s_barrier" ::: "memory");
                 __builtin_amdgcn_sched_barrier(0);
-                sta = sta == 2 ? 0 : sta + 1;
+                sta = sta == NA - 1 ? 0 : sta + 1;
                 stb = stb == NB - 1 ? 0 : stb + 1;
                 return;
             }
@@ -455,17 +508,17 @@
             using SL = std::integral_constant<int, U % ASETS>;
             ks_advance(sl);
             const int e = ks_at(sl);
-            const int k1 = kt_at(sl + 1), kl = ks_at(sl + ASETS);
+            const int k1 = ks_at(sl + 1), k2 = ks_at(sl + 2), kl = ks_at(sl + ASETS);
             if constexpr (PP) {
-                halfstep(e, 0, T{}, k1, 1, T{}, SW{}, T{}, SL{}, ks_at(sl + ASETS + 1), std::integral_constant<int, NLB>{});
-                halfstep(e, 1, T{}, kt_at(sl + 2), 0, T{}, SW{}, Fl{}, SL{}, 0, std::integral_constant<int, NLB + NLA>{});
+                halfstep(e, 0, T{}, k1, 1, T{}, SW{}, T{}, SL{}, PRE ? k2 : ks_at(sl + ASETS + 1), std::integral_constant<int, PRE ? NLB + PRE_N : NLB>{});
+                halfstep(e, 1, T{}, k2, 0, T{}, SW{}, Fl{}, SL{}, PRE ? k2 : 0, std::integral_constant<int, PRE ? NLB + PRE_N : NLB + NLA>{});
             } else
             if constexpr (NB == 3) {
                 halfstep(e, 0, T{}, k1, 0, T{}, SW{}, T{}, SL{}, kl, std::integral_constant<int, NLB + NLA>{});
                 halfstep(e, 1, T{}, k1, 1, T{}, SW{}, Fl{}, SL{}, 0, std::integral_constant<int, NLB>{});
             } else {
                 halfstep(e, 0, T{}, k1, 1, T{}, SW{}, T{}, SL{}, kl, std::integral_constant<int, 2 * NLB + NLA>{});
-                halfstep(e, 1, T{}, kt_at(sl + 2), 0, T{}, SW{}, Fl{}, SL{}, 0, std::integral_constant<int, 2 * NLB + NLA>{});
+                halfstep(e, 1, T{}, k2, 0, T{}, SW{}, Fl{}, SL{}, 0, std::integral_constant<int, 2 * NLB + NLA>{});
             }
         };
         auto slice_tail = [&](int sl, auto u_tag) {
@@ -476,28 +529,36 @@
             ks_advance(sl);
             const int e = ks_at(sl);
             const bool w = sl + 1 < nsl, l = sl + ASETS < nsl;
-            const int kl = l ? ks_at(sl + ASETS + (PP ? 1 : 0)) : 0;
+            const int kl = PRE ? (sl + 2 < nsl ? ks_at(sl + 2) : 0) : (l ? ks_at(sl + ASETS + (PP ? 1 : 0)) : 0);
             {
                 const int gb = 2 * sl + NB - 1;
                 const bool b = gb / 2 < nsl;
-                const int kb = b ? kt_at(gb / 2) : 0;
+                const int kb = b ? ks_at(gb / 2) : 0;
+                if constexpr (PRE) {
+                    if (b) halfstep(e, 0, T{}, kb, gb & 1, Fl{}, SW{}, Fl{}, SL{}, kl, Z{});
+                    else halfstep(e, 0, Fl{}, 0, 0, Fl{}, SW{}, Fl{}, SL{}, 0, Z{});
+                } else
                 if (b && w && l) halfstep(e, 0, T{}, kb, gb & 1, T{}, SW{}, T{}, SL{}, kl, Z{});
-                else if (b && w) halfstep(e, 0, T{}, kb, gb & 1, T{}, SW{}, Fl{}, SL{}, 0, Z{});
+                else if (b && w) halfstep(e, 0, T{}, kb, gb & 1, T{}, SW{}, Fl{}, SL{}, kl, Z{});
                 else if (w) halfstep(e, 0, Fl{}, 0, 0, T{}, SW{}, Fl{}, SL{}, 0, Z{});
-                else if (b) halfstep(e, 0, T{}, kb, gb & 1, Fl{}, SW{}, Fl{}, SL{}, 0, Z{});
+                else if (b) halfstep(e, 0, T{}, kb, gb & 1, Fl{}, SW{}, Fl{}, SL{}, kl, Z{});
                 else halfstep(e, 0, Fl{}, 0, 0, Fl{}, SW{}, Fl{}, SL{}, 0, Z{});
             }
             {
                 const int gb = 2 * sl + 1 + NB - 1;
                 const bool b = gb / 2 < nsl;
-                const int kb = b ? kt_at(gb / 2) : 0;
-                if (b && w) halfstep(e, 1, T{}, kb, gb & 1, T{}, SW{}, Fl{}, SL{}, 0, Z{});
+                const int kb = b ? ks_at(gb / 2) : 0;
+                if constexpr (PRE) {
+                    if (b) halfstep(e, 1, T{}, kb, gb & 1, Fl{}, SW{}, Fl{}, SL{}, kl, Z{});
+                    else halfstep(e, 1, Fl{}, 0, 0, Fl{}, SW{}, Fl{}, SL{}, 0, Z{});
+                } else
+                if (b && w) halfstep(e, 1, T{}, kb, gb & 1, T{}, SW{}, Fl{}, SL{}, kl, Z{});
                 else if (w) halfstep(e, 1, Fl{}, 0, 0, T{}, SW{}, Fl{}, SL{}, 0, Z{});
-                else if (b) halfstep(e, 1, T{}, kb, gb & 1, Fl{}, SW{}, Fl{}, SL{}, 0, Z{});
+                else if (b) halfstep(e, 1, T{}, kb, gb & 1, Fl{}, SW{}, Fl{}, SL{}, kl, Z{});
                 else halfstep(e, 1, Fl{}, 0, 0, Fl{}, SW{}, Fl{}, SL{}, 0, Z{});
             }
         };
-        if constexpr (PP) load_a_rows(ks_at(ASETS));
+        if constexpr (PP && !PRE) load_a_rows(ks_at(ASETS));
         int sl = 0;
         for (; sl + 2 * ASETS < nsl; sl += ASETS) {
             slice_steady(sl, S0{});
@@ -665,9 +726,9 @@
     gconv3_body<WGN, F_LDS, NB, PL, GUARD>(p, blockIdx.x);
 }
 
-template <int F_LDS, int NB, int PL, bool GUARD = false>
+template <int F_LDS, int NB, int PL, bool GUARD = false, int PRE = 0>
 __global__ void __launch_bounds__(512, 2) k_gconv3w(const GParams p) {
-    gconv3_body<4, F_LDS, NB, PL, GUARD>(p, blockIdx.x);
+    gconv3_body<4, F_LDS, NB, PL, GUARD, PRE>(p, blockIdx.x);
 }
 
 __global__ void __launch_bounds__(256) k_weight_split3(const float *__restrict__ Wt, int64_t k_rows, int64_t ldw,
@@ -811,6 +872,45 @@
     }
 }
 
+__global__ void __launch_bounds__(256) k_presplit2h(const float *__restrict__ X, int64_t ld, int64_t rows, int c4, int64_t pld,
+                                                    const float *__restrict__ amax, unsigned char *__restrict__ dst) {
+    const float sc = split_scale(amax[0]);
+    const int64_t total = rows * c4;
+    const int64_t step = (int64_t)gridDim.x * 256;
+    for (int64_t i = (int64_t)blockIdx.x * 256 + threadIdx.x; i < total; i += step) {
+        const int64_t r = total < ((int64_t)1 << 32) ? (int64_t)((unsigned)i / (unsigned)c4) : i / c4;
+        const int c = (int)(i - r * c4) * 4;
+        const float4_t v = *reinterpret_cast<const float4_t *>(X + r * ld + c);
+        unsigned h0, l0, h1, l1;
+        split2h(v.x, v.y, sc, h0, l0);
+        split2h(v.z, v.w, sc, h1, l1);
+        unsigned char *d = dst + presplit_col_offset(pld, r, c & ~7, 0) + (c & 4) * 2;
+        *reinterpret_cast<u32x2 *>(d) = u32x2{h0, h1};
+        *reinterpret_cast<u32x2 *>(d + 64) = u32x2{l0, l1};
+    }
+    for (int64_t i = (int64_t)blockIdx.x * 256 + threadIdx.x; i < pld / 16; i += step)
+        *reinterpret_cast<u32x4 *>(dst + rows * pld + i * 16) = u32x4{0u, 0u, 0u, 0u};
+}
+
+}
+
+extern "C" int64_t hpl_presplit_ld(int32_t C) { return C > 0 ? presplit_ld(C) : 0; }
+extern "C" int64_t hpl_presplit_bytes(int64_t rows, int32_t C) { return (rows >= 0 && C > 0) ? presplit_bytes(rows, C) : 0; }
+
+extern "C" int hpl_presplit2h(const float *X, int64_t ld, int64_t rows, int32_t C, const float *amax, void *planes, hplStream stream) {
+    HPL_REQUIRE(X && amax && planes && rows >= 0 && C > 0 && C % 4 == 0 && ld >= C && ld % 4 == 0 && aligned16(X) &&
+                    (reinterpret_cast<uintptr_t>(planes) & 127) == 0,
+                "hpl_presplit2h: bad arguments (rows=%lld C=%d ld=%lld; C and ld multiples of 4, X 16-byte and the planes 128-byte aligned)",
+                (long long)rows, C, (long long)ld);
+    const int grid = (int)imax(1, imin(cdiv(rows * (C / 4), 256 * 4), 1024));
+    k_presplit2h<<<grid, 256, 0, to_stream(stream)>>>(X, ld, rows, C / 4, presplit_ld(C), amax, reinterpret_cast<unsigned char *>(planes));
+    HPL_CHECK_LAUNCH("hpl_presplit2h");
+    return HPL_OK;
+}
+
+int hpl_gc::presplit_mode() {
+    static const int mode = [] { const char *e = getenv("HPL_PRESPLIT"); return e ? (atoi(e) != 0 ? 1 : 0) : -1; }();
+    return mode;
 }
 
 __global__ void __launch_bounds__(256) k_weight_split3_batch(const hpl_split3_job *__restrict__ jobs) {
@@ -929,6 +1029,10 @@
         return 2;
     }();
     return planes;
+}
+
+static bool presplit_class_default(int f_lds, int splits) {
+    return f_lds == 8 && splits <= 1;
 }
 
 bool hpl_gc::plan_split3(GParams &p, hpl_gconv_info &o) {
@@ -998,6 +1102,12 @@
     o.f_lds = p.F == 1 ? 1 : (p.F <= 8 ? 8 : 15);
     o.compact = 0;
     o.splits = p.splits;
+    p.presplit = 0;
+    if (p.planes == 2 && p.a_planes && bn256 && presplit_maybe(p.M, p.C, p.F, p.N) && presplit_mode() != 0 &&
+        (presplit_mode() == 1 || presplit_class_default(o.f_lds, p.splits))) {
+        p.presplit = 1;
+        o.family = HPL_FAMILY_PAIRS_PRESPLIT;
+    }
     o.guard_sets = (p.planes == 2 && p.a_guard) ? 2 : 1;
     p.guard_partials = (o.guard_sets == 2 && p.splits > 1) ? 1 : 0;
     o.col_share = p.col_share; o.col_rows = p.col_rows;
@@ -1012,7 +1122,16 @@
     const int grid = (int)o.grid;
     const bool bn256 = o.bn == 256;
     const int fl = o.f_lds;
-    if (o.family == HPL_FAMILY_PAIRS) {
+    if (o.family == HPL_FAMILY_PAIRS || o.family == HPL_FAMILY_PAIRS_PRESPLIT) {
+        if (o.family == HPL_FAMILY_PAIRS_PRESPLIT && p.C % 8 == 0) {
+            if (fl == 1) k_gconv3w<1, 4, 2, false, 1><<<grid, 512, 0, s>>>(p);
+            else if (fl == 8) k_gconv3w<8, 4, 2, false, 1><<<grid, 512, 0, s>>>(p);
+            else k_gconv3w<15, 4, 2, false, 1><<<grid, 512, 0, s>>>(p);
+        } else if (o.family == HPL_FAMILY_PAIRS_PRESPLIT) {
+            if (fl == 1) k_gconv3w<1, 4, 2, false, 2><<<grid, 512, 0, s>>>(p);
+            else if (fl == 8) k_gconv3w<8, 4, 2, false, 2><<<grid, 512, 0, s>>>(p);
+            else k_gconv3w<15, 4, 2, false, 2><<<grid, 512, 0, s>>>(p);
+        } else
         if (bn256) {
             if (fl == 1) k_gconv3w<1, 4, 2><<<grid, 512, 0, s>>>(p);
             else if (fl == 8) k_gconv3w<8, 4, 2><<<grid, 512, 0, s>>>(p);
diff --git a/hplflownet_amd/csrc/gconv_common.h b/hplflownet_amd/csrc/gconv_common.h
--- a/hplflownet_amd/csrc/gconv_common.h
+++ b/hplflownet_amd/csrc/gconv_common.h
@@ -1,5 +1,6 @@
 #pragma once
 #include "common.h"
+#include "presplit_layout.h"
 
 namespace hpl_gc {
 
@@ -73,6 +74,8 @@
     const unsigned *a_guard; unsigned *y_guard; int *guard_trips;
     int guard_partials;
     int epi_fast;
+    const void *a_planes; int64_t a_pl_ld; int64_t a_pl_rows;
+    int presplit;
 };
 
 __device__ __forceinline__ int64_t src_row(const GParams &p, int f, int64_t m) {
@@ -149,6 +152,12 @@
 
 
 int fill_params(const hpl_gconv_desc *d, GParams &p, const char *who);
+int fill_planes(GParams &p, const void *a_planes, int64_t ld_bytes, int64_t rows, const char *who);
+int presplit_mode();
+inline bool presplit_maybe(int64_t M, int C, int F, int N) {
+    (void)M; (void)F;
+    return C % 4 == 0 && N > 128;
+}
 bool plan_split3(GParams &p, hpl_gconv_info &o);
 void launch_split3(const GParams &p, const hpl_gconv_info &o, hipStream_t s);
 bool split3_enabled();
diff --git a/hplflownet_amd/csrc/presplit_layout.h b/hplflownet_amd/csrc/presplit_layout.h
--- /dev/null
+++ b/hplflownet_amd/csrc/presplit_layout.h
@@ -0,0 +1,29 @@
+#pragma once
+#include <stdint.h>
+
+#if defined(__HIPCC__) || defined(__CUDACC__)
+#define HPL_LAYOUT_FN __host__ __device__ __forceinline__
+#else
+#define HPL_LAYOUT_FN inline
+#endif
+
+namespace hpl_gc {
+
+constexpr int PRESPLIT_UNIT = 128;
+HPL_LAYOUT_FN int64_t presplit_ld(int C) { return (int64_t)((C + 31) / 32) * PRESPLIT_UNIT; }
+HPL_LAYOUT_FN int64_t presplit_bytes(int64_t rows, int C) { return (rows + 1) * presplit_ld(C); }
+HPL_LAYOUT_FN int64_t presplit_offset(int64_t ld, int64_t row, int unit, int pl, int kb) {
+    return row * ld + (int64_t)unit * PRESPLIT_UNIT + pl * 64 + kb * 16;
+}
+HPL_LAYOUT_FN void presplit_locate(int64_t ld, int64_t off, int64_t &row, int &unit, int &pl, int &kb) {
+    row = off / ld;
+    const int in_row = (int)(off - row * ld);
+    unit = in_row / PRESPLIT_UNIT;
+    pl = (in_row % PRESPLIT_UNIT) / 64;
+    kb = (in_row % 64) / 16;
+}
+HPL_LAYOUT_FN int64_t presplit_col_offset(int64_t ld, int64_t row, int c, int pl) {
+    return presplit_offset(ld, row, c >> 5, pl, (c >> 3) & 3);
+}
+
+}
diff --git a/hplflownet_amd/ops.py b/hplflownet_amd/ops.py
--- a/hplflownet_amd/ops.py
+++ b/hplflownet_amd/ops.py
@@ -1117,6 +1117,21 @@
     check(_lib.load().hpl_amax_rows(p_, ld, r if rows is None else rows, c if cols is None else cols, ptr(out), ptr(guard), stream()),
           'hpl_amax_rows')
     return out, guard
+
+
+def _planes_buffer(nbytes, device):
+    raw = torch.empty(nbytes + 128, dtype=torch.uint8, device=device)
+    return raw[(-raw.data_ptr()) % 128:][:nbytes]
+
+
+def presplit2h(X, scale, rows=None, cols=None):
+    p_, ld, r, c = _mat(X, 'presplit2h input')
+    r, c = (r if rows is None else rows), (c if cols is None else cols)
+    lib = _lib.load()
+    pld = lib.hpl_presplit_ld(c)
+    out = _planes_buffer(lib.hpl_presplit_bytes(r, c), X.device)
+    check(lib.hpl_presplit2h(p_, ld, r, c, ptr(scale), ptr(out), stream()), 'hpl_presplit2h')
+    return out.view(r + 1, pld)
 
 
 def _mat(x, what, dev=True):
@@ -1216,10 +1231,15 @@
 
 def gconv_raw(A, nbr, M, C, F, Wt, N, bias=None, act=ACT_NONE, res=None, res_mod=0, out=None,
               scat=None, scat_c=0, naive=False, slope=LEAKY_RATE, row_perm=None, split_k=True, reg_stride=0, tiles=None,
-              out2=None, rows2=0, Wt3=None, y_amax=None, guard=True, y_guard=None, guard_trips=None):
+              out2=None, rows2=0, Wt3=None, y_amax=None, guard=True, y_guard=None, guard_trips=None, presplit=False):
     d, out, st, _keep = _gconv_desc(A, nbr, M, C, F, Wt, N, bias, act, res, res_mod, out, scat, scat_c, slope, row_perm, split_k,
                                     reg_stride, tiles, out2, rows2, Wt3, y_amax, guard, y_guard, guard_trips)
     lib = _lib.load()
+    if presplit and not naive and d.a_amax and d.wt3_planes == 2 and C % 4 == 0:
+        planes = _planes_buffer(lib.hpl_presplit_bytes(d.rows_a, C), A.device)
+        check(lib.hpl_presplit2h(d.A, d.lda, d.rows_a, C, d.a_amax, ptr(planes), st), 'hpl_presplit2h')
+        check(lib.hpl_gconv_forward_presplit(ctypes.byref(d), ptr(planes), lib.hpl_presplit_ld(C), d.rows_a, st), 'hpl_gconv_forward_presplit')
+        return out
     rc = (lib.hpl_gconv_forward_naive if naive else lib.hpl_gconv_forward)(ctypes.byref(d), st)
     if rc != 0:
         check(rc, 'hpl_gconv_forward')
@@ -1232,11 +1252,16 @@
 
 def gconv_launch_info(A, nbr, M, C, F, Wt, N, bias=None, act=ACT_NONE, res=None, res_mod=0, out=None,
                       scat=None, scat_c=0, slope=LEAKY_RATE, row_perm=None, split_k=True, reg_stride=0, tiles=None,
-                      out2=None, rows2=0, Wt3=None, y_amax=None, guard=True, y_guard=None, guard_trips=None):
+                      out2=None, rows2=0, Wt3=None, y_amax=None, guard=True, y_guard=None, guard_trips=None, presplit=False):
     d = _gconv_desc(A, nbr, M, C, F, Wt, N, bias, act, res, res_mod, out, scat, scat_c, slope, row_perm, split_k,
                     reg_stride, tiles, out2, rows2, Wt3, y_amax, guard, y_guard, guard_trips, query=True)[0]
     info = _lib.GConvInfo()
-    check(_lib.load().hpl_gconv_launch_info(ctypes.byref(d), ctypes.byref(info)), 'hpl_gconv_launch_info')
+    lib = _lib.load()
+    if presplit and d.a_amax and d.wt3_planes == 2 and C % 4 == 0:
+        check(lib.hpl_gconv_launch_info_presplit(ctypes.byref(d), _QUERY_PTR, lib.hpl_presplit_ld(C), d.rows_a, ctypes.byref(info)),
+              'hpl_gconv_launch_info_presplit')
+    else:
+        check(lib.hpl_gconv_launch_info(ctypes.byref(d), ctypes.byref(info)), 'hpl_gconv_launch_info')
     return _info_dict(info)
 
 
diff --git a/include/hpl_bcl.h b/include/hpl_bcl.h
--- a/include/hpl_bcl.h
+++ b/include/hpl_bcl.h
@@ -160,6 +160,7 @@
 #define HPL_FAMILY_FP32 0
 #define HPL_FAMILY_PAIRS 2
 #define HPL_FAMILY_TRIPLES 3
+#define HPL_FAMILY_PAIRS_PRESPLIT 4
 #define HPL_FINISH_NONE 0
 #define HPL_FINISH_SCALAR 1
 #define HPL_FINISH_VEC4 2
@@ -181,6 +182,14 @@
     int64_t grid;
 } hpl_gconv_info;
 int hpl_gconv_launch_info(const hpl_gconv_desc *desc , hpl_gconv_info *info );
+
+int64_t hpl_presplit_ld(int32_t C);
+int64_t hpl_presplit_bytes(int64_t rows, int32_t C);
+int hpl_presplit2h(const float *X, int64_t ld, int64_t rows, int32_t C, const float *amax, void *planes, hplStream stream);
+int hpl_gconv_forward_presplit(const hpl_gconv_desc *desc , const void *planes, int64_t ld_bytes, int64_t rows,
+                               hplStream stream);
+int hpl_gconv_launch_info_presplit(const hpl_gconv_desc *desc , const void *planes, int64_t ld_bytes, int64_t rows,
+                                   hpl_gconv_info *info );
 
 #define HPL_WBIAS_NONE 0
 #define HPL_WBIAS_KERNEL 1
```

Result: slower. 478.6 point-pairs/s (-4.4%).
